# lthero-big/A-watermark-for-Diffusion-Models

Hardware: AMD Instinct MI355X
Metric: watermarked images/sec (embed+extract, 512x512 SD2.1) + lossless bit-accuracy (higher is better)
Workload: dtype f16; 1 GPU; e2e: gsw_embed -> 50-step DDIM sampling (CFG 7.5, 2B-row UNet) -> 50-step DDIM inversion -> fused last step + 256-bit vote; SD2.1-base-shaped UNet (865.9 M params, synthetic weights; convolutions on the hand-written MFMA implicit GEMM), image stages per image: VAE decode -> uint8 -> ToTensor -> VAE encode (timed; synthetic VAE, inversion consumes the latent); batch_per_gpu=64, global_batch=64, message_bits=256, ddim_steps=50, parallelism=dp1 (images sharded, UNet replicated, no data-path collective)

## Files before the change

a-watermark-for-diffusion-models_amd/_native.py:

```python
from __future__ import annotations

import ctypes as C
import os

_HERE = os.path.dirname(os.path.abspath(__file__))
LIB_PATH = os.environ.get("GSWM_LIB", os.path.join(_HERE, "libgswm.so"))

GSW_F32, GSW_F16, GSW_BF16, GSW_F64 = 0, 1, 2, 3
GSW_OK, GSW_ERR_BAD_ARG, GSW_ERR_UNSUPPORTED, GSW_ERR_RAGGED, GSW_ERR_HIP, GSW_WARN_NO_RECORDS = 0, 1, 2, 3, 4, 5
GSW_EMBED_EXACT_F64, GSW_EMBED_FAST_F32 = 0, 1
GSW_MM_GN_ONLY = 1
GSW_FLAG_SATURATED, GSW_FLAG_NAN = 1, 2
GSW_MSG_INLINE_MAX = 256
GSW_IMG_U8_HWC, GSW_IMG_F16_CHW, GSW_IMG_F32_CHW = 0, 1, 2
GSW_PW_BRIGHTNESS, GSW_PW_CONTRAST, GSW_PW_INVERT, GSW_PW_GRAY, GSW_PW_HFLIP, GSW_PW_VFLIP, GSW_PW_NOISE = range(7)
GSW_RESAMPLE_LANCZOS, GSW_RESAMPLE_BILINEAR = 1, 2
GSW_TRACE_SOFT, GSW_TRACE_HARD = 0, 1

_u8p = C.POINTER(C.c_uint8)


class GswMmExtras(C.Structure):
    _fields_ = [("colstats_dev", C.c_void_p), ("colstats_capacity", C.c_int64), ("rowstats_dev", C.c_void_p), ("rowstats_capacity", C.c_int64),
                ("workspace_dev", C.c_void_p), ("workspace_bytes", C.c_int64), ("max_splits", C.c_int),
                ("colstats_rows_per_block", C.c_int), ("colstats_blocks", C.c_int), ("rowstats_slots", C.c_int), ("splits", C.c_int), ("flags", C.c_int)]


_PROTOTYPES = {
    "gsw_version": (C.c_int, []),
    "gsw_build_flags": (C.c_int, []),
    "gsw_strerror": (C.c_char_p, [C.c_int]),
    "gsw_last_hip_error": (C.c_int, []),
    "gsw_keystream": (C.c_int, [C.c_char_p, C.c_char_p, C.c_void_p, C.c_size_t, C.c_void_p]),
    "gsw_embed": (C.c_int, [C.c_char_p, C.c_char_p, C.c_char_p, C.c_int, C.c_void_p, C.c_uint64, C.c_uint64, C.c_void_p,
                            C.c_int, C.c_int, C.c_int64, C.c_uint32, C.c_void_p]),
    "gsw_philox_uniform": (C.c_int, [C.c_uint64, C.c_uint64, C.c_void_p, C.c_int, C.c_int64, C.c_void_p]),
    "gsw_extract": (C.c_int, [C.c_void_p, C.c_int, C.c_char_p, C.c_char_p, C.c_int, C.c_void_p, C.c_void_p, C.c_void_p,
                              C.c_int, C.c_int64, C.c_void_p]),
    "gsw_bit_matches": (C.c_int, [C.c_void_p, C.c_int, C.c_char_p, C.c_int, C.c_void_p, C.c_int, C.c_void_p]),
    "gsw_ddim_step": (C.c_int, [C.c_void_p, C.c_void_p, C.c_void_p, C.c_float, C.c_float, C.c_int, C.c_int64, C.c_void_p]),
    "gsw_ddim_step_cfg": (C.c_int, [C.c_void_p, C.c_void_p, C.c_void_p, C.c_void_p, C.c_float, C.c_float, C.c_float,
                                    C.c_int, C.c_int64, C.c_void_p]),
    "gsw_dpm_step": (C.c_int, [C.c_void_p, C.c_void_p, C.c_void_p, C.c_void_p, C.c_void_p, C.c_void_p, C.c_float, C.c_float, C.c_float,
                               C.c_float, C.c_float, C.c_float, C.c_int, C.c_int64, C.c_void_p]),
    "gsw_ddim_step_extract": (C.c_int, [C.c_void_p, C.c_void_p, C.c_void_p, C.c_float, C.c_float, C.c_int, C.c_char_p,
                                        C.c_char_p, C.c_int, C.c_void_p, C.c_void_p, C.c_void_p, C.c_int, C.c_int64,
                                        C.c_void_p]),
    "gsw_groupnorm_silu": (C.c_int, [C.c_void_p, C.c_void_p, C.c_void_p, C.c_void_p, C.c_void_p, C.c_int, C.c_int, C.c_int, C.c_int,
                                     C.c_float, C.c_int, C.c_int, C.c_void_p]),
    "gsw_geglu": (C.c_int, [C.c_void_p, C.c_void_p, C.c_int64, C.c_int, C.c_int, C.c_void_p]),
    "gsw_conv_pf": (C.c_int, [C.c_void_p, C.c_void_p, C.c_void_p, C.c_void_p, C.c_int, C.c_void_p, C.c_void_p, C.c_int, C.c_int, C.c_int, C.c_int,
                              C.c_int, C.c_int, C.c_int, C.c_int, C.c_int, C.c_void_p]),
    "gsw_groupnorm_pf": (C.c_int, [C.c_void_p, C.c_void_p, C.c_void_p, C.c_void_p, C.c_void_p, C.c_int, C.c_int, C.c_int, C.c_int, C.c_int,
                                   C.c_float, C.c_int, C.c_int, C.c_int, C.c_void_p]),
    "gsw_add_layernorm": (C.c_int, [C.c_void_p, C.c_void_p, C.c_void_p, C.c_void_p, C.c_void_p, C.c_void_p, C.c_int64, C.c_int, C.c_float,
                                    C.c_int, C.c_void_p]),
    "gsw_groupnorm_pf2": (C.c_int, [C.c_void_p, C.c_void_p, C.c_int, C.c_void_p, C.c_void_p, C.c_void_p, C.c_void_p, C.c_int, C.c_int, C.c_int,
                                    C.c_int, C.c_int, C.c_float, C.c_int, C.c_int, C.c_int, C.c_void_p]),
    "gsw_conv3x3_res_pf": (C.c_int, [C.c_void_p, C.c_void_p, C.c_void_p, C.c_void_p, C.c_int, C.c_void_p, C.c_void_p, C.c_int, C.c_int, C.c_int, C.c_int,
                                     C.c_int, C.c_void_p, C.c_int, C.c_void_p, C.c_int, C.c_int, C.c_void_p]),
    "gsw_conv_up2x_pf": (C.c_int, [C.c_void_p, C.c_void_p, C.c_void_p, C.c_void_p, C.c_int, C.c_int, C.c_int, C.c_int, C.c_int, C.c_int, C.c_void_p]),
    "gsw_attention": (C.c_int, [C.c_void_p, C.c_void_p, C.c_void_p, C.c_void_p, C.c_int, C.c_int, C.c_int, C.c_int, C.c_int, C.c_int, C.c_int, C.c_int,
                                C.c_int, C.c_float, C.c_int, C.c_void_p]),
    "gsw_attention_ws": (C.c_int, [C.c_void_p, C.c_void_p, C.c_void_p, C.c_void_p, C.c_int, C.c_int, C.c_int, C.c_int, C.c_int, C.c_int, C.c_int, C.c_int,
                                   C.c_int, C.c_float, C.c_int, C.c_void_p, C.c_int64, C.c_void_p]),
    "gsw_xattn_fused": (C.c_int, [C.c_void_p, C.c_void_p, C.c_void_p, C.c_int64, C.c_void_p, C.c_int64, C.c_void_p, C.c_void_p, C.c_void_p, C.c_float, C.c_int, C.c_int,
                                  C.c_int, C.c_int, C.c_int, C.c_int, C.c_void_p]),
    "gsw_xattn_fused_pre": (C.c_int, [C.c_void_p, C.c_void_p, C.c_void_p, C.c_float, C.c_void_p, C.c_int64, C.c_void_p, C.c_int64, C.c_void_p, C.c_void_p, C.c_void_p,
                                      C.c_float, C.c_int, C.c_int, C.c_int, C.c_int, C.c_int, C.c_int, C.c_void_p]),
    "gsw_gn_colstats_pairs": (C.c_int, [C.c_void_p, C.c_int, C.c_int, C.c_int, C.c_void_p, C.c_int, C.c_int, C.c_int, C.c_int, C.c_void_p]),
    "gsw_gn_proj_tokens": (C.c_int, [C.c_void_p, C.c_void_p, C.c_void_p, C.c_void_p, C.c_float, C.c_int, C.c_void_p, C.c_void_p, C.c_void_p, C.c_float, C.c_int, C.c_int,
                                     C.c_int, C.c_int, C.c_int, C.c_void_p]),
    "gsw_mt19937_seed": (None, [C.c_uint32, C.c_void_p]),
    "gsw_mt19937_uniform": (C.c_int, [C.c_void_p, C.c_int, C.c_void_p, C.c_int64, C.c_void_p, C.c_void_p]),
    "gsw_lanczos_plan": (C.c_int, [C.c_int, C.c_int, C.c_void_p, C.c_void_p, C.c_int]),
    "gsw_resize_lanczos": (C.c_int, [C.c_void_p, C.c_int, C.c_int, C.c_int, C.c_void_p, C.c_int, C.c_int, C.c_int, C.c_void_p, C.c_void_p, C.c_void_p,
                                     C.c_int, C.c_void_p, C.c_void_p, C.c_int, C.c_void_p]),
    "gsw_tensor_to_image": (C.c_int, [C.c_void_p, C.c_int, C.c_int, C.c_int, C.c_int, C.c_int, C.c_void_p, C.c_void_p]),
    "gsw_jpeg_quant_tables": (C.c_int, [C.c_int, C.c_void_p, C.c_void_p]),
    "gsw_jpeg_workspace_bytes": (C.c_size_t, [C.c_int, C.c_int, C.c_int]),
    "gsw_jpeg_roundtrip": (C.c_int, [C.c_void_p, C.c_int, C.c_int, C.c_int, C.c_int, C.c_void_p, C.c_int, C.c_void_p, C.c_void_p]),
    "gsw_gaussian_blur_params": (C.c_int, [C.c_float, C.c_int, C.c_void_p, C.c_void_p, C.c_void_p]),
    "gsw_gaussian_blur": (C.c_int, [C.c_void_p, C.c_int, C.c_int, C.c_int, C.c_float, C.c_void_p, C.c_void_p, C.c_void_p]),
    "gsw_image_pointwise": (C.c_int, [C.c_void_p, C.c_int, C.c_int, C.c_int, C.c_int, C.c_float, C.c_uint64, C.c_uint64, C.c_void_p, C.c_int,
                                      C.c_void_p, C.c_void_p]),
    "gsw_resample_plan": (C.c_int, [C.c_int, C.c_int, C.c_int, C.c_void_p, C.c_void_p, C.c_int]),
    "gsw_affine_nearest": (C.c_int, [C.c_void_p, C.c_int, C.c_int, C.c_int, C.c_void_p, C.c_void_p, C.c_int, C.c_void_p]),
    "gsw_box_mask": (C.c_int, [C.c_void_p, C.c_int, C.c_int, C.c_int, C.c_void_p, C.c_int, C.c_void_p, C.c_int, C.c_void_p]),
    "gsw_crop_resize": (C.c_int, [C.c_void_p, C.c_int, C.c_int, C.c_int, C.c_void_p, C.c_int, C.c_int, C.c_void_p, C.c_int, C.c_int, C.c_int,
                                  C.c_void_p, C.c_void_p, C.c_void_p, C.c_int, C.c_void_p, C.c_void_p, C.c_int, C.c_void_p]),
    "gsw_gemm": (C.c_int, [C.c_void_p, C.c_void_p, C.c_void_p, C.c_void_p, C.c_void_p, C.c_int64, C.c_int, C.c_int, C.c_int, C.c_int, C.c_int,
                           C.c_int, C.c_void_p]),
    "gsw_gemm_qkv": (C.c_int, [C.c_void_p, C.c_void_p, C.c_void_p, C.c_void_p, C.c_void_p, C.c_int64, C.c_int, C.c_int, C.c_int, C.c_int, C.c_int, C.c_void_p]),
    "gsw_ln_rowstats_finish": (C.c_int, [C.c_void_p, C.c_int, C.c_int64, C.c_int, C.c_float, C.c_void_p, C.c_void_p]),
    "gsw_gemm_ln": (C.c_int, [C.c_void_p, C.c_void_p, C.c_void_p, C.c_void_p, C.c_void_p, C.c_void_p, C.c_int64, C.c_int, C.c_int, C.c_int, C.c_int, C.c_int, C.c_void_p]),
    "gsw_gemm_strided": (C.c_int, [C.c_void_p, C.c_int64, C.c_void_p, C.c_int64, C.c_void_p, C.c_void_p, C.c_int64, C.c_void_p, C.c_int64, C.c_int64,
                                   C.c_int, C.c_int, C.c_int, C.c_int, C.c_int, C.c_int, C.c_void_p]),
    "gsw_softmax_rows": (C.c_int, [C.c_void_p, C.c_int64, C.c_int, C.c_int64, C.c_float, C.c_int, C.c_void_p]),
    "gsw_mm_config": (C.c_int, [C.c_int, C.c_int]),
    "gsw_mm_get_config": (C.c_int, [C.POINTER(C.c_int), C.POINTER(C.c_int)]),
    "gsw_groupnorm_pf_cs": (C.c_int, [C.c_void_p, C.c_void_p, C.c_int, C.c_void_p, C.c_int, C.c_int, C.c_int, C.c_void_p, C.c_int, C.c_int, C.c_int,
                                      C.c_void_p, C.c_void_p, C.c_void_p, C.c_void_p, C.c_int, C.c_int, C.c_int, C.c_int, C.c_int, C.c_float, C.c_int, C.c_int,
                                      C.c_int, C.c_void_p]),
    "gsw_groupnorm_pf_fused": (C.c_int, [C.c_void_p, C.c_void_p, C.c_int, C.c_void_p, C.c_void_p, C.c_void_p, C.c_int, C.c_int, C.c_int, C.c_int, C.c_int, C.c_float,
                                         C.c_int, C.c_int, C.c_int, C.c_void_p]),
    "gsw_gather_rows": (C.c_int, [C.c_void_p, C.c_int64, C.c_int64, C.c_void_p, C.c_int, C.c_void_p, C.c_int64, C.c_int, C.c_int64, C.c_void_p]),
    "gsw_nchw_to_pf": (C.c_int, [C.c_void_p, C.c_void_p, C.c_int, C.c_int, C.c_int, C.c_int, C.c_int, C.c_int, C.c_void_p]),
    "gsw_conv3x3_pf_nchw": (C.c_int, [C.c_void_p, C.c_void_p, C.c_void_p, C.c_void_p, C.c_int, C.c_int, C.c_int, C.c_int, C.c_int, C.c_int, C.c_void_p]),
    "gsw_gemm_small_config": (C.c_int, [C.c_int64, C.c_int, C.c_int, C.c_int]),
    "gsw_gemm_small": (C.c_int, [C.c_void_p, C.c_int64, C.c_void_p, C.c_int64, C.c_void_p, C.c_void_p, C.c_int64, C.c_void_p, C.c_int64, C.c_int64, C.c_int, C.c_int,
                                 C.c_int, C.c_int, C.c_int, C.c_void_p, C.c_int, C.c_float, C.c_void_p, C.c_void_p, C.c_void_p, C.c_int64, C.POINTER(C.c_int), C.c_int,
                                 C.c_int, C.c_void_p]),
    "gsw_gemm_ex": (C.c_int, [C.c_void_p, C.c_int64, C.c_void_p, C.c_int64, C.c_void_p, C.c_void_p, C.c_int64, C.c_void_p, C.c_int64, C.c_int64, C.c_int, C.c_int,
                              C.c_int, C.c_int, C.c_int, C.c_int, C.c_void_p, C.c_void_p]),
    "gsw_gemm2_ex": (C.c_int, [C.c_void_p, C.c_int64, C.c_int, C.c_void_p, C.c_int64, C.c_int, C.c_void_p, C.c_int64, C.c_void_p, C.c_void_p, C.c_int64, C.c_void_p,
                               C.c_int64, C.c_int64, C.c_int, C.c_int, C.c_int, C.c_int, C.c_int, C.c_void_p, C.c_void_p]),
    "gsw_gemm_ln_ex": (C.c_int, [C.c_void_p, C.c_void_p, C.c_void_p, C.c_void_p, C.c_void_p, C.c_void_p, C.c_int64, C.c_int, C.c_int, C.c_int, C.c_int, C.c_int,
                                 C.c_void_p, C.c_void_p]),
    "gsw_conv_pf_ex": (C.c_int, [C.c_void_p, C.c_void_p, C.c_void_p, C.c_void_p, C.c_int, C.c_void_p, C.c_void_p, C.c_int, C.c_int, C.c_int, C.c_int,
                                 C.c_int, C.c_int, C.c_int, C.c_int, C.c_int, C.c_void_p, C.c_void_p]),
    "gsw_conv3x3_res_pf_ex": (C.c_int, [C.c_void_p, C.c_void_p, C.c_void_p, C.c_void_p, C.c_int, C.c_void_p, C.c_void_p, C.c_int, C.c_int, C.c_int, C.c_int,
                                        C.c_int, C.c_void_p, C.c_int, C.c_void_p, C.c_int, C.c_int, C.c_void_p, C.c_void_p]),
    "gsw_conv_up2x_pf_ex": (C.c_int, [C.c_void_p, C.c_void_p, C.c_void_p, C.c_void_p, C.c_int, C.c_int, C.c_int, C.c_int, C.c_int, C.c_int, C.c_void_p, C.c_void_p]),
    "gsw_trace_workspace_bytes": (C.c_size_t, [C.c_int, C.c_int64, C.c_int]),
    "gsw_trace_topk": (C.c_int, [C.c_void_p, C.c_int, C.c_int, C.c_int, C.c_int, C.c_void_p, C.c_int64, C.c_int, C.c_void_p, C.c_void_p, C.c_void_p, C.c_void_p]),
    "gsw_sign_pack": (C.c_int, [C.c_void_p, C.c_int, C.c_void_p, C.c_void_p, C.c_int, C.c_int64, C.c_void_p]),
    "gsw_trace_keyed_workspace_bytes": (C.c_size_t, [C.c_int, C.c_int64, C.c_int]),
    "gsw_trace_keyed_topk": (C.c_int, [C.c_void_p, C.c_int, C.c_int64, C.c_void_p, C.c_int64, C.c_int, C.c_int64, C.c_int, C.c_void_p, C.c_void_p, C.c_void_p, C.c_void_p]),
    "gsw_embed_l": (C.c_int, [C.c_char_p, C.c_char_p, C.c_char_p, C.c_int, C.c_void_p, C.c_uint64, C.c_uint64, C.c_void_p,
                              C.c_int, C.c_int, C.c_int64, C.c_uint32, C.c_int, C.c_void_p]),
    "gsw_extract_l": (C.c_int, [C.c_void_p, C.c_int, C.c_char_p, C.c_char_p, C.c_int, C.c_void_p, C.c_void_p, C.c_void_p,
                                C.c_int, C.c_int64, C.c_int, C.c_void_p]),
    "gsw_quant_pack": (C.c_int, [C.c_void_p, C.c_int, C.c_void_p, C.c_void_p, C.c_int, C.c_int64, C.c_int, C.c_void_p]),
}

_lib = None


class GswError(RuntimeError):
    def __init__(self, status: int, what: str):
        super().__init__(f"libgswm: {what} (status {status})")
        self.status = status


def lib() -> C.CDLL:
    global _lib
    if _lib is None:
        if not os.path.exists(LIB_PATH):
            raise ImportError(
                f"{LIB_PATH} is missing: the HIP library has not been built. Run __graft_entry__.build() "
                "(hipcc --offload-arch=gfx950). There is no CPU fallback for the watermark hot path.")
        l = C.CDLL(LIB_PATH)
        for name, (res, args) in _PROTOTYPES.items():
            fn = getattr(l, name)
            fn.restype = res
            fn.argtypes = args
        flags = l.gsw_build_flags()
        if flags != 0 and os.environ.get("GSWM_LIB") is None:
            raise ImportError(f"{LIB_PATH} was compiled with measurement switches (gsw_build_flags() = {flags:#x}): not a production build; rebuild it "
                              "(__graft_entry__.build()) or select the side build explicitly with GSWM_LIB")
        _lib = l
    return _lib


def exported_symbols():
    return sorted(_PROTOTYPES)


def check(status: int):
    if status == GSW_OK:
        return
    what = lib().gsw_strerror(status).decode()
    if status == GSW_ERR_RAGGED:
        raise IndexError("string index out of range")
    if status == GSW_ERR_BAD_ARG:
        raise ValueError(f"libgswm: {what}")
    if status == GSW_ERR_HIP:
        what += f" (hipError_t {lib().gsw_last_hip_error()})"
    raise GswError(status, what)
```

a-watermark-for-diffusion-models_amd/csrc/gswm_mm.hip:

```cpp
#include <hip/hip_runtime.h>
#include <hip/hip_fp16.h>
#include <hip/hip_bf16.h>
#include <stdint.h>
#include <stdlib.h>
#include <algorithm>
#include <atomic>
#include <type_traits>

#include "../../include/gswm.h"
#include "gswm_mm.h"
#include "gswm_mmtypes.h"
#include "gswm_ablate.inc"

static std::atomic<int> g_mm_tile_rows{getenv("GSW_MM_BM") ? atoi(getenv("GSW_MM_BM")) : 0};
static std::atomic<int> g_mm_split_mask{getenv("GSW_MM_SPLIT") ? atoi(getenv("GSW_MM_SPLIT")) : 10 };

namespace {

__device__ unsigned long long* g_mm_trace_buf;
template <typename F>
__device__ __forceinline__ mm_f4 mm_abl_touch(F a, F b, mm_f4 c) { c[0] = fmaf((float)a[0], (float)b[0], c[0]); return c; }
#define MM_BARRIER() do { __builtin_amdgcn_sched_barrier(0); __builtin_amdgcn_s_barrier(); __builtin_amdgcn_sched_barrier(0); } while (0)
#define MM_LDS_BARRIER() do { asm volatile("s_waitcnt lgkmcnt(0)" ::: "memory"); MM_BARRIER(); } while (0)

typedef float mm_f2 __attribute__((ext_vector_type(2)));
__device__ __forceinline__ uint32_t mm_lds_addr(const uint8_t* p) { return (uint32_t)(uintptr_t)(const __attribute__((address_space(3))) uint8_t*)p; }
__device__ __forceinline__ void mm_lds_read5_b64(uint32_t a, uint2 (&o)[5]) {
    uint64_t r0, r1, r2, r3, r4;
    asm volatile("ds_read_b64 %0, %5\n\tds_read_b64 %1, %5 offset:32\n\tds_read_b64 %2, %5 offset:64\n\tds_read_b64 %3, %5 offset:96\n\tds_read_b64 %4, %5 offset:128\n\t"
                 "s_waitcnt lgkmcnt(0)"
                 : "=&v"(r0), "=&v"(r1), "=&v"(r2), "=&v"(r3), "=&v"(r4) : "v"(a) : "memory");
    const uint64_t r[5] = {r0, r1, r2, r3, r4};
#pragma unroll
    for (int i = 0; i < 5; ++i) o[i] = make_uint2((uint32_t)r[i], (uint32_t)(r[i] >> 32));
}
template <uint32_t VOFF>
__device__ __forceinline__ void mm_lds_read_uv(uint32_t a, mm_f4 (&u)[5], mm_f4 (&v)[5]) {
    asm volatile("ds_read_b128 %0, %10\n\tds_read_b128 %1, %10 offset:64\n\tds_read_b128 %2, %10 offset:128\n\tds_read_b128 %3, %10 offset:192\n\tds_read_b128 %4, %10 offset:256\n\t"
                 "ds_read_b128 %5, %10 offset:%11\n\tds_read_b128 %6, %10 offset:%12\n\tds_read_b128 %7, %10 offset:%13\n\tds_read_b128 %8, %10 offset:%14\n\t"
                 "ds_read_b128 %9, %10 offset:%15\n\ts_waitcnt lgkmcnt(0)"
                 : "=&v"(u[0]), "=&v"(u[1]), "=&v"(u[2]), "=&v"(u[3]), "=&v"(u[4]), "=&v"(v[0]), "=&v"(v[1]), "=&v"(v[2]), "=&v"(v[3]), "=&v"(v[4])
                 : "v"(a), "n"(VOFF), "n"(VOFF + 64u), "n"(VOFF + 128u), "n"(VOFF + 192u), "n"(VOFF + 256u) : "memory");
}
template <uint32_t VOFF>
__device__ __forceinline__ void mm_lds_read_uv1(uint32_t a, mm_f4& u, mm_f4& v) {
    asm volatile("ds_read_b128 %0, %2\n\tds_read_b128 %1, %2 offset:%3\n\ts_waitcnt lgkmcnt(0)" : "=&v"(u), "=&v"(v) : "v"(a), "n"(VOFF) : "memory");
}
template <int MT>
__device__ __forceinline__ void mm_lds_read_rows(uint32_t a, mm_f2 (&r)[MT]) {
    if constexpr (MT == 8)
        asm volatile("ds_read_b64 %0, %8\n\tds_read_b64 %1, %8 offset:128\n\tds_read_b64 %2, %8 offset:256\n\tds_read_b64 %3, %8 offset:384\n\t"
                     "ds_read_b64 %4, %8 offset:512\n\tds_read_b64 %5, %8 offset:640\n\tds_read_b64 %6, %8 offset:768\n\tds_read_b64 %7, %8 offset:896\n\ts_waitcnt lgkmcnt(0)"
                     : "=&v"(r[0]), "=&v"(r[1]), "=&v"(r[2]), "=&v"(r[3]), "=&v"(r[4]), "=&v"(r[5]), "=&v"(r[6]), "=&v"(r[7]) : "v"(a) : "memory");
    else if constexpr (MT == 4)
        asm volatile("ds_read_b64 %0, %4\n\tds_read_b64 %1, %4 offset:128\n\tds_read_b64 %2, %4 offset:256\n\tds_read_b64 %3, %4 offset:384\n\ts_waitcnt lgkmcnt(0)"
                     : "=&v"(r[0]), "=&v"(r[1]), "=&v"(r[2]), "=&v"(r[3]) : "v"(a) : "memory");
    else
        asm volatile("ds_read_b64 %0, %2\n\tds_read_b64 %1, %2 offset:128\n\ts_waitcnt lgkmcnt(0)" : "=&v"(r[0]), "=&v"(r[1]) : "v"(a) : "memory");
}

__device__ __forceinline__ uint32_t mm_lane_now() {
    uint32_t l;
    asm volatile("v_mbcnt_lo_u32_b32 %0, -1, 0\n\tv_mbcnt_hi_u32_b32 %0, -1, %0" : "=v"(l));
    return l;
}
template <int CTRL, int ROW_MASK>
__device__ __forceinline__ float mm_dpp_add(float x) {
    return x + __int_as_float(__builtin_amdgcn_update_dpp(0, __float_as_int(x), CTRL, ROW_MASK, 0xf, false));
}

template <typename T, int EPI, bool SPLIT, int MT, bool LNF = false>
__global__ __launch_bounds__(SPLIT ? 768 : 512, SPLIT ? 1 : 2) void gsw_mm_kernel(const MMArgs p) {
    static_assert(!LNF || (!SPLIT && (EPI == 0 || EPI == 2 || EPI == 3)), "LayerNorm-folded epilogues: dense rows, GEGLU, transposed; 8-wave form");
    constexpr bool SWAP = EPI == 3;
    constexpr bool QKV = EPI == 5;
    constexpr bool PART = EPI == 4;
    static_assert(!PART || SPLIT, "split-K partial launches use the producer-wave variant");
    constexpr bool WIDE = MT == 8;
    constexpr int WM = WIDE ? 2 : 4;
    constexpr int NG = 8 / WM;
    constexpr int BM = WM * 16 * MT, BN = NG * 80;
    constexpr int NPR = MT / 2;
    static_assert(MT == 8 || MT == 4 || MT == 2, "wave tile of 128, 64 or 32 rows");
    static_assert(!WIDE || (!SPLIT && EPI != 3 && EPI != 4 && EPI != 5), "the wide tile: 8-wave form, dense rows / PF rows / GEGLU; no split-K, no transposed output, no fused q | k | v");
    constexpr int NPROD = SPLIT ? 4 : 8;
    constexpr int NPA = BM / 8 / NPROD;
    constexpr int NPW = BN / 8 / NPROD;
    constexpr int NEXTRA = BN / 8 - NPROD * NPW;
    constexpr int NDMA = NPA + NPW;
    constexpr uint32_t STAGE = (uint32_t)(BM + BN) * 128u;
    constexpr uint32_t RING = (WIDE ? 2u : 3u) * STAGE;
    constexpr int HC = 80;
    constexpr bool STG = !SPLIT && !SWAP && !QKV && (EPI == 2 || (EPI == 0 && (!LNF || WIDE)));
    constexpr uint32_t PARAM = RING;
    constexpr uint32_t PAR_V = WIDE ? 2048u : 1024u, PAR_ROWS = WIDE ? 4096u : 2048u;
    constexpr int NPCOL = WIDE ? 2 : 1;
    constexpr int NPAR = LNF ? 2 * NPCOL + (BM + 127) / 128 : 1;
    typedef typename MM<T>::frag frag;
    typedef unsigned int mm_u4 __attribute__((ext_vector_type(4)));
    extern __shared__ __attribute__((aligned(16))) uint8_t lds[];

    const uint32_t tid = threadIdx.x, lane = tid & 63u;
    const uint32_t wave = (uint32_t)__builtin_amdgcn_readfirstlane((int)(tid >> 6));
    const uint32_t grp = WIDE ? (wave >> 1) & 3u : (wave >> 2) & 1u, wm = WIDE ? wave & 1u : wave & 3u;
    const uint32_t pid = SPLIT ? (wave & 3u) : wave;
    const bool extra = pid < (uint32_t)NEXTRA;
    const bool stg = STG && p.P >= (WIDE ? 2 : 3) && (LNF || p.bias != nullptr);
    const bool stg7 = stg && wave == 7u;

    const uint32_t lane_rd0 = (lane & 15u) * 128u + ((((lane >> 4)) ^ ((lane >> 1) & 7u)) << 4);
    const uint32_t a_rd0 = wm * (16u * MT) * 128u + lane_rd0, a_rd1 = a_rd0 ^ 64u;
    const uint32_t w_rd0 = (uint32_t)BM * 128u + (grp * (uint32_t)HC) * 128u + lane_rd0, w_rd1 = w_rd0 ^ 64u;
    const uint32_t prow = lane >> 3;
    const uint32_t chunk8 = ((lane & 7u) ^ ((4u * (pid & 1u) + (lane >> 4)) & 7u)) * 8u;

    const uint32_t G = gridDim.x;
    const uint32_t slotx = (blockIdx.x & 7u) * (G >> 3) + (blockIdx.x >> 3);
    const uint32_t ntiles = (uint32_t)p.ntiles;
    const uint32_t nvirt = PART ? ntiles * (uint32_t)p.splits : ntiles;
    const uint32_t nt_mine = nvirt > slotx ? (nvirt - slotx + G - 1u) / G : 0u;
    if (nt_mine == 0u) return;
    const uint32_t part_split = PART ? slotx / ntiles : 0u;
    const int32_t k_lo = PART ? (int32_t)(((int64_t)part_split * p.P) / p.splits) : 0;
    const int32_t P_mine = PART ? (int32_t)(((int64_t)(part_split + 1u) * p.P) / p.splits) - k_lo : p.P;
    const T* Wbase = reinterpret_cast<const T*>(p.w);
    auto decode_tile = [&](uint32_t L, int32_t& tm, int32_t& tn) {
        const uint32_t tiles_m = ntiles / (uint32_t)p.tiles_n, pw = (uint32_t)p.panel;
        const uint32_t full = tiles_m * pw;
        const uint32_t pn = L / full, rem = L - pn * full;
        const uint32_t width = min(pw, (uint32_t)p.tiles_n - pn * pw);
        tm = (int32_t)(rem / width);
        tn = (int32_t)(pn * pw + rem - (rem / width) * width);
    };

    uint32_t pr_it = 0, pr_slot = 0;
    int32_t pr_seg = 0, pr_kc = 0, pr_kh = 0, pr_run = 0, a_step = 0, w_step = 0;
    int32_t pr_arow[NPA], pr_wrow[NPW + 1];
    const T* pa[NPA];
    const T* pw[NPW + 1];
    const bool compact = (p.flags & MM_FLAG_COMPACT) != 0;
    const int32_t HpWp = p.Hp * p.Wp;
    auto opaque = [&](int32_t v) -> int32_t { if constexpr (WIDE) asm volatile("" : "+s"(v)); return v; };
    auto udiv = [&](uint32_t m, uint32_t d, uint32_t mg) -> uint32_t {
        uint32_t q = __umulhi(m, mg);
        if (m - q * d >= d) ++q;
        return q;
    };
    auto pf_row = [&](int32_t m, int32_t& b, int32_t& yy, int32_t& xx) -> int32_t {
        if constexpr (WIDE) {
            const int32_t Wi = opaque(p.Wp - 2), HW = opaque((p.Hp - 2) * (p.Wp - 2));
            const uint32_t mg_hw = 0xFFFFFFFFu / (uint32_t)HW, mg_wi = 0xFFFFFFFFu / (uint32_t)Wi;
            b = (int32_t)udiv((uint32_t)m, (uint32_t)HW, mg_hw);
            const int32_t r = m - b * HW;
            yy = (int32_t)udiv((uint32_t)r, (uint32_t)Wi, mg_wi);
            xx = r - yy * Wi + 1;
            yy += 1;
            return b * HpWp + yy * p.Wp + xx;
        }
        const int32_t Wi = p.Wp - 2, HW = (p.Hp - 2) * Wi;
        b = m / HW;
        const int32_t r = m - b * HW;
        yy = r / Wi;
        xx = r - yy * Wi + 1;
        yy += 1;
        return b * HpWp + yy * p.Wp + xx;
    };
    auto setup_tile = [&](uint32_t it) {
        int32_t tm, tn;
        decode_tile(PART ? slotx % ntiles : it * G + slotx, tm, tn);
        const int32_t m0 = tm * BM, n0 = tn * BN;
#pragma unroll
        for (int i = 0; i < NPA; ++i) {
            const int32_t m = m0 + 8 * (int32_t)(pid + (uint32_t)NPROD * i) + (int32_t)prow;
            const int32_t mc = m < p.M ? m : p.M - 1;
            int32_t b_, y_, x_;
            pr_arow[i] = compact ? pf_row(mc, b_, y_, x_) : mc;
            if (compact && p.stride == 2) pr_arow[i] = b_ * (p.in_Hp * p.in_Wp) + 2 * (y_ - 1) * p.in_Wp + 2 * (x_ - 1);
        }
#pragma unroll
        for (int i = 0; i <= NPW; ++i) {
            const int32_t n = n0 + 8 * (int32_t)(pid + (uint32_t)NPROD * i) + (int32_t)prow;
            pr_wrow[i] = n < p.N ? n : p.N - 1;
        }
    };
    auto begin_run = [&]() {
        const MMSeg& s0 = p.seg[0]; const MMSeg& s1 = p.seg[1]; const MMSeg& s2 = p.seg[2];
        const int32_t s = pr_seg;
        const T* x = reinterpret_cast<const T*>(s == 0 ? s0.x : s == 1 ? s1.x : s2.x);
        const int32_t ld = s == 0 ? s0.ld : s == 1 ? s1.ld : s2.ld;
        const int32_t kb = s == 0 ? s0.kblocks : s == 1 ? s1.kblocks : s2.kblocks;
        const int32_t nt = s == 0 ? s0.ntaps : s == 1 ? s1.ntaps : s2.ntaps;
        const int32_t tw = s == 0 ? s0.tw : s == 1 ? s1.tw : s2.tw;
        const int32_t trow = s == 0 ? s0.tap_row : s == 1 ? s1.tap_row : s2.tap_row;
        const int32_t tbase = s == 0 ? s0.tap_base : s == 1 ? s1.tap_base : s2.tap_base;
        const int32_t wk0 = s == 0 ? s0.wk0 : s == 1 ? s1.wk0 : s2.wk0;
        const int32_t tapoff = tbase + pr_kh * trow;
        const int32_t wk = wk0 + pr_kh * tw * (kb * 64) + pr_kc * 64 + (int32_t)chunk8;
        if (nt == 1) { pr_run = kb; a_step = 64; w_step = 64; }
        else { pr_run = tw; a_step = ld; w_step = kb * 64; }
#pragma unroll
        for (int i = 0; i < NPA; ++i) pa[i] = x + ((int64_t)(pr_arow[i] + tapoff) * ld + pr_kc * 64 + (int32_t)chunk8);
#pragma unroll
        for (int i = 0; i <= NPW; ++i) pw[i] = Wbase + (pr_wrow[i] * p.ldw + wk);
    };
    auto end_run = [&]() {
        const MMSeg& s0 = p.seg[0]; const MMSeg& s1 = p.seg[1]; const MMSeg& s2 = p.seg[2];
        const int32_t s = pr_seg;
        const int32_t kb = s == 0 ? s0.kblocks : s == 1 ? s1.kblocks : s2.kblocks;
        const int32_t nt = s == 0 ? s0.ntaps : s == 1 ? s1.ntaps : s2.ntaps;
        const int32_t tw = s == 0 ? s0.tw : s == 1 ? s1.tw : s2.tw;
        bool seg_done = nt == 1;
        if (!seg_done && ++pr_kh * tw == nt) { pr_kh = 0; seg_done = ++pr_kc == kb; }
        if (seg_done) {
            pr_kc = 0; pr_kh = 0;
            if (++pr_seg == p.nseg) {
                pr_seg = 0;
                if (++pr_it == nt_mine) {
                    pr_run = 0x7FFFFFFF; a_step = 0; w_step = 0;
#pragma unroll
                    for (int i = 0; i < NPA; ++i) pa[i] = Wbase + chunk8;
#pragma unroll
                    for (int i = 0; i <= NPW; ++i) pw[i] = Wbase + chunk8;
                    return;
                }
                setup_tile(pr_it);
            }
        }
        begin_run();
    };
    auto dma_extra = [&]() {
        if (extra) {
            __builtin_amdgcn_global_load_lds((const __attribute__((address_space(1))) void*)pw[NPW],
                                             (__attribute__((address_space(3))) void*)(lds + pr_slot + (uint32_t)BM * 128u + (pid + (uint32_t)NPROD * NPW) * 1024u), 16, 0, 0);
            pw[NPW] += w_step;
        }
    };
    auto dma_piece_a = [&](int i) {
        __builtin_amdgcn_global_load_lds((const __attribute__((address_space(1))) void*)pa[i],
                                         (__attribute__((address_space(3))) void*)(lds + pr_slot + (pid + (uint32_t)NPROD * i) * 1024u), 16, 0, 0);
        pa[i] += a_step;
    };
    auto dma_piece_w = [&](int i) {
        __builtin_amdgcn_global_load_lds((const __attribute__((address_space(1))) void*)pw[i],
                                         (__attribute__((address_space(3))) void*)(lds + pr_slot + (uint32_t)BM * 128u + (pid + (uint32_t)NPROD * i) * 1024u), 16, 0, 0);
        pw[i] += w_step;
    };
    constexpr bool AFF = EPI == 0 || EPI == 2;
    uint32_t vo_a[4] = {0u, 0u, 0u, 0u}, vo_w = 0u, so_a = 0u, so_w = 0u, st_a = 0u, st_w = 0u, w_piece = 0u, a_piece = 0u;
    int32_t seg_rows = -1;
    bool pr_end = false;
    __amdgpu_buffer_rsrc_t rs_a = __builtin_amdgcn_make_buffer_rsrc(const_cast<void*>(p.w), 0, -1, 0x00020000);
    const __amdgpu_buffer_rsrc_t rs_w = __builtin_amdgcn_make_buffer_rsrc(const_cast<void*>(p.w), 0, -1, 0x00020000);
    uint32_t str_a8 = 128u * (uint32_t)p.seg[0].ld, str_w8 = 128u * (uint32_t)p.ldw;
    if constexpr (WIDE) asm volatile("" : "+s"(str_a8), "+s"(str_w8));
    int32_t tile_m8 = 0, tile_n8 = 0;
    auto setup_tile8 = [&](uint32_t it) {
        decode_tile(it * G + slotx, tile_m8, tile_n8);
        seg_rows = -1;
    };
    auto begin_run8 = [&]() {
        const MMSeg& s0 = p.seg[0]; const MMSeg& s1 = p.seg[1]; const MMSeg& s2 = p.seg[2];
        const int32_t sg = pr_seg;
        const T* x = reinterpret_cast<const T*>(sg == 0 ? s0.x : sg == 1 ? s1.x : s2.x);
        const int32_t ld = sg == 0 ? s0.ld : sg == 1 ? s1.ld : s2.ld;
        const int32_t kb = sg == 0 ? s0.kblocks : sg == 1 ? s1.kblocks : s2.kblocks;
        const int32_t nt = sg == 0 ? s0.ntaps : sg == 1 ? s1.ntaps : s2.ntaps;
        const int32_t tw = sg == 0 ? s0.tw : sg == 1 ? s1.tw : s2.tw;
        const int32_t trow = sg == 0 ? s0.tap_row : sg == 1 ? s1.tap_row : s2.tap_row;
        const int32_t tbase = sg == 0 ? s0.tap_base : sg == 1 ? s1.tap_base : s2.tap_base;
        const int32_t wk0 = sg == 0 ? s0.wk0 : sg == 1 ? s1.wk0 : s2.wk0;
        if (seg_rows != sg) {
            seg_rows = sg;
            const uint32_t l8 = mm_lane_now();

            const uint32_t prow = l8 >> 3;
            const uint32_t chunk8 = ((l8 & 7u) ^ ((4u * (pid & 1u) + (l8 >> 4)) & 7u)) * 8u;
            rs_a = __builtin_amdgcn_make_buffer_rsrc(const_cast<T*>(x + (int64_t)tbase * ld), 0, -1, 0x00020000);
            const int32_t m0 = tile_m8 * BM;
            if constexpr (AFF) {
                vo_a[0] = ((uint32_t)(m0 + 8 * (int32_t)pid + (int32_t)prow) * (uint32_t)ld + chunk8) * 2u;
            } else {
#pragma unroll
                for (int i = 0; i < NPA; ++i) {
                    const int32_t m = m0 + 8 * (int32_t)(pid + (uint32_t)NPROD * i) + (int32_t)prow;
                    const int32_t mc = m < p.M ? m : p.M - 1;
                    int32_t b_, y_, x_, row = mc;
                    if (compact) {
                        row = pf_row(mc, b_, y_, x_);
                        if (p.stride == 2) row = b_ * (p.in_Hp * p.in_Wp) + 2 * (y_ - 1) * p.in_Wp + 2 * (x_ - 1);
                    }
                    vo_a[i] = ((uint32_t)row * (uint32_t)ld + chunk8) * 2u;
                }
            }
        }
        so_a = (uint32_t)(pr_kh * trow * ld + pr_kc * 64) * 2u;
        so_w = (uint32_t)(tile_n8 * BN * p.ldw + wk0 + pr_kh * tw * (kb * 64) + pr_kc * 64) * 2u;
        if (nt == 1) { pr_run = kb; st_a = 128u; st_w = 128u; }
        else { pr_run = tw; st_a = (uint32_t)ld * 2u; st_w = (uint32_t)(kb * 64) * 2u; }
    };
    auto end_run8 = [&]() {
        const MMSeg& s0 = p.seg[0]; const MMSeg& s1 = p.seg[1]; const MMSeg& s2 = p.seg[2];
        const int32_t sg = pr_seg;
        const int32_t kb = sg == 0 ? s0.kblocks : sg == 1 ? s1.kblocks : s2.kblocks;
        const int32_t nt = sg == 0 ? s0.ntaps : sg == 1 ? s1.ntaps : s2.ntaps;
        const int32_t tw = sg == 0 ? s0.tw : sg == 1 ? s1.tw : s2.tw;
        bool seg_done = nt == 1;
        if (!seg_done && ++pr_kh * tw == nt) { pr_kh = 0; seg_done = ++pr_kc == kb; }
        if (seg_done) {
            pr_kc = 0; pr_kh = 0;
            if (++pr_seg == p.nseg) {
                pr_seg = 0;
                if (++pr_it == nt_mine) {
                    pr_run = 0x7FFFFFFF; st_a = 0u; st_w = 0u;
                    so_a = 0u; so_w = 0u;
                    return;
                }
                setup_tile8(pr_it);
            }
        }
        begin_run8();
    };
    auto dma_piece8 = [&](int j) {
        if (j < NPA) {
            if constexpr (AFF) {
                if (j == 0) a_piece = so_a;
                MM_ABL_DMA_A(__builtin_amdgcn_raw_ptr_buffer_load_lds(rs_a, (__attribute__((address_space(3))) void*)(lds + pr_slot + (pid + (uint32_t)NPROD * j) * 1024u), 16, (int)vo_a[0], (int)a_piece, 0, 0));
                a_piece += str_a8;
            } else {
                MM_ABL_DMA_A(__builtin_amdgcn_raw_ptr_buffer_load_lds(rs_a, (__attribute__((address_space(3))) void*)(lds + pr_slot + (pid + (uint32_t)NPROD * j) * 1024u), 16, (int)vo_a[j], (int)so_a, 0, 0));
            }
        } else {
            if (j == NPA) w_piece = so_w;
            MM_ABL_DMA_W(__builtin_amdgcn_raw_ptr_buffer_load_lds(rs_w, (__attribute__((address_space(3))) void*)(lds + pr_slot + (uint32_t)BM * 128u + (pid + (uint32_t)NPROD * (j - NPA)) * 1024u), 16,
                                                                  (int)vo_w, (int)w_piece, 0, 0));
            w_piece += str_w8;
        }
        if (j == NDMA - 1) {
            so_a += st_a; so_w += st_w;
            pr_slot = pr_slot + STAGE == RING ? 0u : pr_slot + STAGE;
            pr_end = --pr_run == 0;
        }
    };
    auto dma_h1 = [&]() {
#pragma unroll
        for (int i = 0; i < NPA / 2; ++i) dma_piece_a(i);
        dma_piece_w(0);
    };
    auto dma_h2 = [&]() {
#pragma unroll
        for (int i = NPA / 2; i < NPA; ++i) dma_piece_a(i);
        dma_piece_w(1);
        pr_slot = pr_slot + STAGE == RING ? 0u : pr_slot + STAGE;
    };
    if constexpr (SPLIT) {
        if (wave >= 8u) {
            int32_t pr_left = 0x7FFFFFFF;
            auto dma_stage = [&]() {
#pragma unroll
                for (int i = 0; i < NPA; ++i) MM_ABL_DMA_A(dma_piece_a(i));
#pragma unroll
                for (int i = 0; i < NPW; ++i) MM_ABL_DMA_W(dma_piece_w(i));
                pr_slot = pr_slot + STAGE == RING ? 0u : pr_slot + STAGE;
                if constexpr (PART) {
                    if (--pr_left == 0) {
                        pr_run = 0x7FFFFFFF; a_step = 0; w_step = 0;
#pragma unroll
                        for (int i = 0; i < NPA; ++i) pa[i] = Wbase + chunk8;
#pragma unroll
                        for (int i = 0; i <= NPW; ++i) pw[i] = Wbase + chunk8;
                        return;
                    }
                }
                if (--pr_run == 0) end_run();
            };
            constexpr int NWAIT = MM_ABL_NPA(NPA) + MM_ABL_NPW(NPW);
            setup_tile(0);
            if constexpr (PART) {
                const MMSeg& s0 = p.seg[0]; const MMSeg& s1 = p.seg[1];
                int32_t st = k_lo;
                const int32_t len0 = s0.kblocks * s0.ntaps, len1 = s1.kblocks * s1.ntaps;
                if (p.nseg > 1 && st >= len0) { st -= len0; pr_seg = 1; if (p.nseg > 2 && st >= len1) { st -= len1; pr_seg = 2; } }
                const int32_t nt = pr_seg == 0 ? s0.ntaps : 1, tw = pr_seg == 0 ? s0.tw : 1;
                int32_t skip = st;
                if (nt != 1) { pr_kc = st / nt; const int32_t r = st - pr_kc * nt; pr_kh = r / tw; skip = r - pr_kh * tw; }
                begin_run();
#pragma unroll
                for (int i = 0; i < NPA; ++i) pa[i] += (int64_t)skip * a_step;
#pragma unroll
                for (int i = 0; i <= NPW; ++i) pw[i] += (int64_t)skip * w_step;
                pr_run -= skip;
                pr_left = P_mine;
            } else {
                begin_run();
            }
            dma_stage();
            dma_stage();
            asm volatile("s_waitcnt vmcnt(%0)" :: "n"(NWAIT) : "memory");
            MM_BARRIER();
            const uint32_t total = nt_mine * (uint32_t)P_mine;
            MM_TRACE_DECL();
            for (uint32_t sidx = 0; sidx < total; ++sidx) {
                dma_stage();
                MM_STAMP(0);
                asm volatile("s_waitcnt vmcnt(%0)" :: "n"(NWAIT) : "memory");
                MM_STAMP(1);
                MM_BARRIER();
                MM_STAMP(2);
            }
            MM_TRACE_DUMP();
            asm volatile("s_waitcnt vmcnt(0)" ::: "memory");
            return;
        }
    } else if constexpr (WIDE) {
        {
            const uint32_t l8 = mm_lane_now();

            vo_w = (((8u * pid + (l8 >> 3)) * (uint32_t)p.ldw) + ((l8 & 7u) ^ ((4u * (pid & 1u) + (l8 >> 4)) & 7u)) * 8u) * 2u;
        }
        setup_tile8(0);
        begin_run8();
#pragma unroll
        for (int j = 0; j < NDMA; ++j) dma_piece8(j);
        if (pr_end) { end_run8(); pr_end = false; }
#pragma unroll
        for (int j = 0; j < NDMA; ++j) dma_piece8(j);
        __builtin_amdgcn_s_waitcnt(0x0F70);
    } else {
        static_assert(SPLIT || ((NPA == 4 || NPA == 2) && NPW == 2), "the half-stage split assumes 4 (2) + 2 (+1) pieces per wave");
        setup_tile(0);
        begin_run();
        for (int i = 0; i < 2; ++i) { dma_h1(); dma_extra(); dma_h2(); if (--pr_run == 0) end_run(); }
        dma_h1();
        asm volatile("s_waitcnt vmcnt(%0)" :: "n"(NDMA + NPA / 2 + 1) : "memory");
    }
    MM_BARRIER();

    const uint16_t* bias = reinterpret_cast<const uint16_t*>(p.bias);
    const uint16_t* rowbias = reinterpret_cast<const uint16_t*>(p.rowbias);
    const uint16_t* resid = reinterpret_cast<const uint16_t*>(p.resid);
    uint16_t* Y = reinterpret_cast<uint16_t*>(p.y);
    mm_f4 acc[5][MT];
#pragma unroll
    for (int a = 0; a < 5; ++a)
#pragma unroll
        for (int b = 0; b < MT; ++b) acc[a][b] = mm_f4{0.f, 0.f, 0.f, 0.f};
    uint32_t c_it = 0, rd_slot = 0;
    MM_TRACE_DECL();

    auto read_frags = [&](frag (&xf)[MT], frag (&wf)[5], uint32_t slot, uint32_t khalf) {
        const uint8_t* ap = lds + ((khalf ? a_rd1 : a_rd0) + slot);
        const uint8_t* wp = lds + ((khalf ? w_rd1 : w_rd0) + slot);
#pragma unroll
        for (int im = 0; im < MT; ++im) xf[im] = *reinterpret_cast<const frag*>(ap + im * 2048);
#pragma unroll
        for (int in = 0; in < 5; ++in) wf[in] = *reinterpret_cast<const frag*>(wp + in * 2048);
    };

    auto dma_params = [&]() {
        int32_t tm, tn;
        decode_tile(c_it * G + slotx, tm, tn);
        const int32_t m0 = tm * BM, n0 = tn * BN;
        const uint32_t lane_p = WIDE ? mm_lane_now() : (threadIdx.x & 63u);
        const uint32_t lane = lane_p;
        auto piece = [&](const void* base, uint32_t lane_bytes, uint32_t byte_off) {
            if constexpr (WIDE) {
                const __amdgpu_buffer_rsrc_t rs = __builtin_amdgcn_make_buffer_rsrc(const_cast<void*>(base), 0, -1, 0x00020000);
                __builtin_amdgcn_raw_ptr_buffer_load_lds(rs, (__attribute__((address_space(3))) void*)(lds + PARAM + byte_off), 16, (int)lane_bytes, 0, 0, 0);
            } else {
                __builtin_amdgcn_global_load_lds((const __attribute__((address_space(1))) void*)(reinterpret_cast<const uint8_t*>(base) + lane_bytes),
                                                 (__attribute__((address_space(3))) void*)(lds + PARAM + byte_off), 16, 0, 0);
            }
        };
        if constexpr (LNF) {
#pragma unroll
            for (int k = 0; k < NPCOL; ++k) {
                const uint32_t nc = (uint32_t)min(n0 + 256 * k + 4 * (int32_t)lane, p.N - 4) * 4u;
                piece(p.ln_u, nc, (uint32_t)k * 1024u);
                piece(p.ln_v, nc, PAR_V + (uint32_t)k * 1024u);
            }
#pragma unroll
            for (int k = 0; k < (BM + 127) / 128; ++k) piece(p.ln_stat, (uint32_t)min(m0 + 128 * k + 2 * (int32_t)lane, p.M - 2) * 8u, PAR_ROWS + (uint32_t)k * 1024u);
        } else {
            piece(p.bias, (uint32_t)min(n0 + 8 * (int32_t)lane, p.N - 8) * 2u, 0u);
        }
    };

    auto epilogue = [&]() {
        int32_t tile_m, tile_n;
        decode_tile(PART ? slotx % ntiles : c_it * G + slotx, tile_m, tile_n);
        const int32_t m0 = tile_m * BM, n0 = tile_n * BN;
        const uint32_t lane_e = WIDE ? mm_lane_now() : (threadIdx.x & 63u);

        const uint32_t lane = lane_e;
        const uint32_t q = lane >> 4, li = lane & 15u;
        uint32_t zero_hi = 0u;
        if constexpr (WIDE) asm volatile("v_mov_b32 %0, 0" : "=v"(zero_hi));
        auto zx = [&](uint32_t v) -> int64_t { return WIDE ? (int64_t)(((uint64_t)zero_hi << 32) | (uint64_t)v) : (int64_t)v; };
        MM_STAMP(13);
        auto out_row = [&](int32_t m, int32_t& img, bool& brd, bool& lv) -> int64_t {
            lv = m < p.M; brd = false; img = 0;
            int64_t orow_ = m;
            const int32_t mc = lv ? m : 0;
            if (p.mode == MM_MODE_PF || p.mode == MM_MODE_UP2X) {
                int32_t b, yy, xx;
                if (compact) {
                    orow_ = pf_row(mc, b, yy, xx);
                } else {
                    const int32_t d1 = opaque(HpWp), d2 = opaque(p.Wp);
                    b = mc / d1;
                    const int32_t r = mc - b * HpWp;
                    yy = r / d2; xx = r - yy * p.Wp;
                    brd = (yy == 0) | (yy == p.Hp - 1) | (xx == 0) | (xx == p.Wp - 1);
                }
                img = b;
                if (p.mode == MM_MODE_UP2X) {
                    const int32_t dy = (p.up - 1) >> 1, dx = (p.up - 1) & 1;
                    orow_ = ((int64_t)b * (2 * p.Hp - 2) + (2 * (yy - 1) + dy + 1)) * (2 * p.Wp - 2) + (2 * (xx - 1) + dx + 1);
                    lv = lv && !brd;
                }
            } else if (p.mode == MM_MODE_TOK2PF) {
                const int32_t d1 = opaque(p.S), d2 = opaque(p.Wimg);
                const int32_t b = mc / d1, ii = mc - b * p.S;
                const int32_t yy = ii / d2, xx = ii - yy * p.Wimg;
                img = b;
                orow_ = (int64_t)b * HpWp + (int64_t)(yy + 1) * p.Wp + (xx + 1);
            }
            return orow_;
        };
        if constexpr (WIDE && EPI == 1) {
            if (resid) {
                const __amdgpu_buffer_rsrc_t rs_r = __builtin_amdgcn_make_buffer_rsrc(const_cast<uint16_t*>(resid), 0, -1, 0x00020000);
#pragma unroll
                for (int k = 0; k < 4; ++k) {
                    const int32_t m = m0 + (int32_t)(wm * (16u * MT) + (uint32_t)k * 32u + (lane >> 1));
                    int32_t img_; bool brd_, lv_ = m < p.M;
                    int64_t row_ = m;
                    if constexpr (EPI == 1) row_ = out_row(m, img_, brd_, lv_);
                    const int64_t col_ = (int64_t)n0 + grp * (uint32_t)HC + (lane & 1u) * 64u;
                    if (lv_ && col_ < p.N)
                        __builtin_amdgcn_raw_ptr_buffer_load_lds(rs_r, (__attribute__((address_space(3))) void*)(lds + RING + 6144u), 4, (int)(uint32_t)((row_ * p.ldr + col_) * 2), 0, 0, 0);
                }
            }
        }
        const bool vtile = QKV && n0 >= p.n_rows;
        const bool transposed = SWAP || vtile;
        if constexpr (PART) {
            uint32_t sx = slotx * 8u + wave;
            asm volatile("" : "+s"(sx));
            float* slab = p.ws + (size_t)sx * (size_t)(5 * MT * 64 * 4);
            const uint32_t loff = lane * 4u;
#pragma unroll
            for (int in = 0; in < 5; ++in)
#pragma unroll
                for (int im = 0; im < MT; ++im)
                    if (m0 + (int32_t)(wm * (16u * MT)) + im * 16 < p.M)
                        *reinterpret_cast<mm_f4*>(slab + (uint32_t)((in * MT + im) * 256) + loff) = acc[in][im];
            ++c_it;
            return;
        }
        float ln_r[SWAP ? 4 * MT : MT], ln_n[SWAP ? 4 * MT : MT];
        mm_f4 ln_u4[5], ln_v4[5];
        if constexpr (LNF) {
            const float2* st = reinterpret_cast<const float2*>(p.ln_stat);
            if constexpr (!SWAP) {
                if constexpr (STG) {
                    if (!stg) {
                        MM_BARRIER();
                        if (wave == 7u) { dma_params(); asm volatile("s_waitcnt vmcnt(0)" ::: "memory"); }
                        MM_BARRIER();
                    }
                    if constexpr (!(WIDE && EPI == 0)) {
                        mm_f2 rw[MT];
                        mm_lds_read_rows<MT>(mm_lds_addr(lds + PARAM + PAR_ROWS) + (wm * (16u * MT) + li) * 8u, rw);
#pragma unroll
                        for (int im = 0; im < MT; ++im) { ln_r[im] = rw[im][0]; ln_n[im] = rw[im][1]; }
                    }
                    if constexpr (!WIDE) mm_lds_read_uv<PAR_V>(mm_lds_addr(lds + PARAM) + (grp * HC + q * 4u) * 4u, ln_u4, ln_v4);
                } else {
#pragma unroll
                for (int im = 0; im < MT; ++im) {
                    const int32_t m = m0 + (int32_t)(wm * (16u * MT) + (uint32_t)im * 16u + li);
                    const float2 v = st[m < p.M ? m : p.M - 1];
                    ln_r[im] = v.x; ln_n[im] = v.y;
                }
#pragma unroll
                for (int in = 0; in < 5; ++in) {
                    const int32_t nb = n0 + (int32_t)(grp * HC + (uint32_t)in * 16u + q * 4u);
                    const int32_t nc = nb < p.N ? nb : 0;
                    ln_u4[in] = *reinterpret_cast<const mm_f4*>(p.ln_u + nc);
                    ln_v4[in] = *reinterpret_cast<const mm_f4*>(p.ln_v + nc);
                }
                }
            } else {
#pragma unroll
                for (int im = 0; im < MT; ++im) {
                    const int32_t m = m0 + (int32_t)(wm * (16u * MT) + (uint32_t)im * 16u + q * 4u);
                    const int32_t mc = m + 3 < p.M ? m : 0;
                    const mm_f4 a = *reinterpret_cast<const mm_f4*>(st + mc), b = *reinterpret_cast<const mm_f4*>(st + mc + 2);
                    ln_r[4 * im] = a[0]; ln_n[4 * im] = a[1]; ln_r[4 * im + 1] = a[2]; ln_n[4 * im + 1] = a[3];
                    ln_r[4 * im + 2] = b[0]; ln_n[4 * im + 2] = b[1]; ln_r[4 * im + 3] = b[2]; ln_n[4 * im + 3] = b[3];
                }
#pragma unroll
                for (int in = 0; in < 5; ++in) {
                    const int32_t ncol = n0 + (int32_t)(grp * HC + (uint32_t)in * 16u + li);
                    const int32_t nc = ncol < p.N ? ncol : 0;
                    ln_u4[in] = mm_f4{p.ln_u[nc], 0.f, 0.f, 0.f};
                    ln_v4[in] = mm_f4{p.ln_v[nc], 0.f, 0.f, 0.f};
                }
            }
        }
        auto lnf_rows = [&](int pr) {
            if constexpr (LNF && WIDE && STG && EPI == 0) {
                mm_f2 rw[2];
                mm_lds_read_rows<2>(mm_lds_addr(lds + PARAM + PAR_ROWS) + (wm * (16u * MT) + (uint32_t)(2 * pr) * 16u + li) * 8u, rw);
                ln_r[2 * pr] = rw[0][0]; ln_n[2 * pr] = rw[0][1]; ln_r[2 * pr + 1] = rw[1][0]; ln_n[2 * pr + 1] = rw[1][1];
            }
        };
        auto lnf_cols = [&](int in) {
            if constexpr (LNF && WIDE && STG) mm_lds_read_uv1<PAR_V>(mm_lds_addr(lds + PARAM) + (grp * HC + (uint32_t)in * 16u + q * 4u) * 4u, ln_u4[in], ln_v4[in]);
        };
        auto vals4 = [&](int in, int im, const float (&b)[4], float (&o)[4]) {
            const mm_f4& a = acc[in][im];
            if constexpr (LNF) {
                if constexpr (!SWAP) {
#pragma unroll
                    for (int j = 0; j < 4; ++j) o[j] = fmaf(a[j], ln_r[im], fmaf(ln_n[im], ln_u4[in][j], ln_v4[in][j]));
                } else {
#pragma unroll
                    for (int j = 0; j < 4; ++j) o[j] = fmaf(a[j], ln_r[4 * im + j], fmaf(ln_n[4 * im + j], ln_u4[in][0], ln_v4[in][0]));
                }
            } else {
#pragma unroll
                for (int j = 0; j < 4; ++j) o[j] = a[j] + b[j];
            }
        };
        auto pack4 = [&](int in, int im, const float (&b)[4], uint32_t& lo, uint32_t& hi) {
            if constexpr (LNF) {
                float o[4];
                vals4(in, im, b, o);
                lo = MM<T>::cvt2(o[0], o[1]);
                hi = MM<T>::cvt2(o[2], o[3]);
            } else {
                const mm_f4& a = acc[in][im];
                lo = MM<T>::cvt2(a[0] + b[0], a[1] + b[1]);
                hi = MM<T>::cvt2(a[2] + b[2], a[3] + b[3]);
            }
        };
        uint2 bq_raw[5];
        if constexpr (STG && !LNF) {
#pragma unroll
            for (int in = 0; in < 5; ++in) bq_raw[in] = make_uint2(0, 0);
            if (bias) {
                if (!stg) {
                    MM_BARRIER();
                    if (wave == 7u) { dma_params(); asm volatile("s_waitcnt vmcnt(0)" ::: "memory"); }
                    MM_BARRIER();
                }
                mm_lds_read5_b64(mm_lds_addr(lds + PARAM) + (grp * HC + q * 4u) * 2u, bq_raw);
            }
        } else
#pragma unroll
        for (int in = 0; in < 5; ++in) {
            bq_raw[in] = make_uint2(0, 0);
            const int32_t nb = n0 + (int32_t)(grp * HC + (uint32_t)in * 16u + q * 4u);
            if (!LNF && !transposed && bias && nb < p.N) bq_raw[in] = *reinterpret_cast<const uint2*>(bias + nb);
        }
        auto bias4 = [&](int in, float (&bq)[4]) {
            bq[0] = MM<T>::up((uint16_t)bq_raw[in].x); bq[1] = MM<T>::up((uint16_t)(bq_raw[in].x >> 16));
            bq[2] = MM<T>::up((uint16_t)bq_raw[in].y); bq[3] = MM<T>::up((uint16_t)(bq_raw[in].y >> 16));
        };
        auto swap16 = [&](uint32_t& a, uint32_t& b) {
            const auto r = __builtin_amdgcn_permlane16_swap(a, b, false, false);
            a = r[0]; b = r[1];
        };
        auto swap32 = [&](uint32_t& a, uint32_t& b) {
            const auto r = __builtin_amdgcn_permlane32_swap(a, b, false, false);
            a = r[0]; b = r[1];
        };
        if (EPI == 0 || (QKV && !vtile)) {
            uint16_t* yrow[NPR];
            const uint16_t* rrow[NPR];
            bool live[NPR];
            const int32_t colb = n0 + (int32_t)(grp * HC + (q >> 1) * 8u);
            auto row_setup = [&](int pr) {
                const int32_t m = m0 + (int32_t)(wm * (16u * MT) + (uint32_t)(2 * pr + (int)(q & 1u)) * 16u + li);
                live[pr] = m < p.M;
                const int64_t mm = live[pr] ? m : 0;
                yrow[pr] = Y + mm * p.ldy + colb;
                rrow[pr] = resid ? resid + mm * p.ldr + colb : nullptr;
            };
            const bool rstat = EPI == 0 && p.rowstats != nullptr;
            float rs_s[NPR], rs_q[NPR];
#pragma unroll
            for (int pr = 0; pr < NPR; ++pr) { rs_s[pr] = __uint_as_float(zero_hi); rs_q[pr] = __uint_as_float(zero_hi); }
            constexpr int RSD = SPLIT ? 2 : (WIDE ? 2 : 5);
            uint4 rs[5][NPR];
            auto load_rs1 = [&](int in, int pr) {
                rs[in][pr] = make_uint4(zero_hi, zero_hi, zero_hi, zero_hi);
                if (colb + in * 16 < p.N) rs[in][pr] = *reinterpret_cast<const uint4*>(rrow[pr] + in * 16);
            };
            auto load_rs = [&](int in) {
#pragma unroll
                for (int pr = 0; pr < NPR; ++pr) load_rs1(in, pr);
            };
            auto block = [&](int in, int pr, const float (&bq)[4]) {
                uint32_t a0, a1, b0, b1;
                pack4(in, 2 * pr, bq, a0, a1);
                pack4(in, 2 * pr + 1, bq, b0, b1);
                swap16(a0, b0);
                swap16(a1, b1);
                uint32_t w4[4] = {a0, a1, b0, b1};
                if (resid) {
                    const uint32_t rsw[4] = {rs[in][pr].x, rs[in][pr].y, rs[in][pr].z, rs[in][pr].w};
#pragma unroll
                    for (int k = 0; k < 4; ++k) w4[k] = MM<T>::add2(w4[k], rsw[k]);
                }
                if constexpr (WIDE) { if (in == 0 && pr == 0) { MM_STAMP(7); if (!resid) __builtin_amdgcn_s_waitcnt(0x0F70); MM_STAMP(8); } }
                if (live[pr] && colb + in * 16 < p.N) {
                    *reinterpret_cast<uint4*>(yrow[pr] + in * 16) = make_uint4(w4[0], w4[1], w4[2], w4[3]);
                    if (rstat) {
#pragma unroll
                        for (int k = 0; k < 4; ++k) MM<T>::stat2(w4[k], rs_s[pr], rs_q[pr]);
                    }
                }
            };
            auto flush_stat = [&](int pr) {
                uint32_t a = __float_as_uint(rs_s[pr]), b = __float_as_uint(rs_q[pr]);
                swap32(a, b);
                const float t = __uint_as_float(a) + __uint_as_float(b);
                const int32_t m = m0 + (int32_t)(wm * (16u * MT) + (uint32_t)(2 * pr + (int)(q & 1u)) * 16u + li);
                if (m < p.M) p.rowstats[((int64_t)m * (NG * p.tiles_n) + NG * tile_n + (int32_t)grp) * 2 + zx(lane >> 5)] = t;
            };
            if constexpr (WIDE) {
                auto body = [&](auto res_tag, auto stat_tag) {
                    constexpr bool RES = decltype(res_tag)::value, STAT = decltype(stat_tag)::value;
                    constexpr int RD = LNF ? 10 : 8;
                    const uint32_t lrow = (q & 1u) * 16u + li, lcol = grp * (uint32_t)HC + (q >> 1) * 8u;
                    const uint32_t y_voff = (lrow * (uint32_t)p.ldy + lcol) * 2u;
                    const uint32_t y_s0 = (uint32_t)(((int64_t)(m0 + (int32_t)(wm * (16u * MT))) * p.ldy + n0) * 2);
                    mm_u4 rq[4 * 5];
                    const __amdgpu_buffer_rsrc_t rs_q = __builtin_amdgcn_make_buffer_rsrc(const_cast<uint16_t*>(RES ? resid : Y), 0, -1, 0x00020000);
                    uint32_t r_voff = 0u, r_s0 = 0u;
                    auto rq_issue = [&](int b) {
                        const int pr = b / 5, in = b % 5;
                        rq[b] = __builtin_amdgcn_raw_buffer_load_b128(rs_q, (int)r_voff, (int)(r_s0 + (uint32_t)(pr * 32) * (uint32_t)p.ldr * 2u + (uint32_t)(in * 32)), 0);
                    };
                    if constexpr (RES) {
                        r_voff = (lrow * (uint32_t)p.ldr + lcol) * 2u;
                        r_s0 = (uint32_t)(((int64_t)(m0 + (int32_t)(wm * (16u * MT))) * p.ldr + n0) * 2);
#pragma unroll
                        for (int b = 0; b < RD; ++b) rq_issue(b);
                    }
#pragma unroll
                    for (int pr = 0; pr < NPR; ++pr) {
                        lnf_rows(pr);
                        float ss = __uint_as_float(zero_hi), sq = __uint_as_float(zero_hi);
#pragma unroll
                        for (int in = 0; in < 5; ++in) {
                            const int b = pr * 5 + in;
                            float bq[4];
                            bias4(in, bq);
                            lnf_cols(in);
                            if constexpr (RES) { if (b + RD < 20) rq_issue(b + RD); }
                            uint32_t a0, a1, b0, b1;
                            pack4(in, 2 * pr, bq, a0, a1);
                            pack4(in, 2 * pr + 1, bq, b0, b1);
                            swap16(a0, b0);
                            swap16(a1, b1);
                            mm_u4 w4 = {a0, a1, b0, b1};
                            if constexpr (RES) {
#pragma unroll
                                for (int k = 0; k < 4; ++k) w4[k] = MM<T>::add2(w4[k], rq[b][k]);
                            }
                            if (b == 0) {
                                MM_STAMP(7);
                                if constexpr (!RES) __builtin_amdgcn_s_waitcnt(0x0F70);
                                MM_STAMP(8);
                            }
                            *reinterpret_cast<mm_u4*>(reinterpret_cast<uint8_t*>(Y) + (size_t)(y_s0 + (uint32_t)(pr * 32) * (uint32_t)p.ldy * 2u + (uint32_t)(in * 32)) + (size_t)y_voff) = w4;
                            if constexpr (STAT) {
#pragma unroll
                                for (int k = 0; k < 4; ++k) MM<T>::stat2(w4[k], ss, sq);
                            }
                            __builtin_amdgcn_sched_barrier(0);
                        }
                        if constexpr (STAT) {
                            uint32_t a = __float_as_uint(ss), bb = __float_as_uint(sq);
                            swap32(a, bb);
                            const float t = __uint_as_float(a) + __uint_as_float(bb);
                            const int32_t m = m0 + (int32_t)(wm * (16u * MT) + (uint32_t)(2 * pr + (int)(q & 1u)) * 16u + li);
                            p.rowstats[((int64_t)m * (NG * p.tiles_n) + NG * tile_n + (int32_t)grp) * 2 + zx(lane >> 5)] = t;
                        }
                        __builtin_amdgcn_sched_barrier(0);
                    }
                };
                if (resid) { if (rstat) body(std::true_type{}, std::true_type{}); else body(std::true_type{}, std::false_type{}); }
                else { if (rstat) body(std::false_type{}, std::true_type{}); else body(std::false_type{}, std::false_type{}); }
            } else {
#pragma unroll
                for (int pr = 0; pr < NPR; ++pr) row_setup(pr);
                if (resid) {
#pragma unroll
                    for (int in = 0; in < RSD; ++in) load_rs(in);
                }
#pragma unroll
                for (int in = 0; in < 5; ++in) {
                    float bq[4];
                    bias4(in, bq);
                    if (resid && in + RSD < 5) load_rs(in + RSD);
#pragma unroll
                    for (int pr = 0; pr < NPR; ++pr) block(in, pr, bq);
                }
                if (rstat) {
#pragma unroll
                    for (int pr = 0; pr < NPR; ++pr) flush_stat(pr);
                }
            }
        } else if (EPI == 1) {
            using orow_t = std::conditional_t<WIDE, int32_t, int64_t>;
            orow_t orow[NPR];
            int32_t img_b[NPR];
            bool live[NPR], border[NPR];
#pragma unroll
            for (int pr = 0; pr < NPR; ++pr) {
                const int32_t m = m0 + (int32_t)(wm * (16u * MT) + (uint32_t)(2 * pr + (int)(q & 1u)) * 16u + li);
                orow[pr] = (orow_t)out_row(m, img_b[pr], border[pr], live[pr]);
            }
            const bool cstat = p.colstats != nullptr;
            MM_STAMP(14);
            constexpr int PD = WIDE ? 6 : 1;
            uint4 prev[PD + 1];
            auto fetch = [&](int in, int pr, int sl) {
                const int64_t col = (int64_t)n0 + grp * (uint32_t)HC + (uint32_t)in * 16u + (q >> 1) * 8u;
                const bool okl = live[pr] && col < p.N && !border[pr];
                if (resid) prev[sl] = *reinterpret_cast<const uint4*>(resid + (okl ? (int64_t)orow[pr] * p.ldr + col : (int64_t)0));
                else prev[sl] = *reinterpret_cast<const uint4*>(rowbias + (okl ? (int64_t)img_b[pr] * p.ldrb + col : (int64_t)0));
            };
            if constexpr (WIDE) {
                if (rowbias || resid) {
#pragma unroll
                    for (int j0 = 0; j0 < PD; ++j0) fetch(j0 / NPR, j0 % NPR, j0);
                }
            }
#pragma unroll
            for (int in = 0; in < 5; ++in) {
                float bq[4];
                bias4(in, bq);
                const int64_t col = (int64_t)n0 + grp * (uint32_t)HC + (uint32_t)in * 16u + (q >> 1) * 8u;
                float cs_s[4] = {0.f, 0.f, 0.f, 0.f}, cs_q[4] = {0.f, 0.f, 0.f, 0.f};
#pragma unroll
                for (int pr = 0; pr < NPR; ++pr) {
                    constexpr int NB = 5 * NPR;
                    const int j = in * NPR + pr;
                    if constexpr (WIDE) { if ((rowbias || resid) && j + PD < NB) fetch((j + PD) / NPR, (j + PD) % NPR, (j + PD) % (PD + 1)); }
                    uint32_t a0, a1, b0, b1;
                    pack4(in, 2 * pr, bq, a0, a1);
                    pack4(in, 2 * pr + 1, bq, b0, b1);
                    swap16(a0, b0);
                    swap16(a1, b1);
                    if constexpr (WIDE) { if (j == 0 && !(rowbias || resid)) __builtin_amdgcn_s_waitcnt(0x0F70); }
                    if constexpr (WIDE) {
                        uint32_t w4[4] = {a0, a1, b0, b1};
                        if (rowbias || resid) {
                            uint4 rb = make_uint4(0, 0, 0, 0), rs = make_uint4(0, 0, 0, 0);
                            if (resid) { rs = prev[j % (PD + 1)]; if (rowbias) rb = *reinterpret_cast<const uint4*>(rowbias + (int64_t)img_b[pr] * p.ldrb + (col < p.N ? col : 0)); }
                            else rb = prev[j % (PD + 1)];
                            const uint32_t rbw[4] = {rb.x, rb.y, rb.z, rb.w}, rsw[4] = {rs.x, rs.y, rs.z, rs.w};
#pragma unroll
                            for (int k = 0; k < 4; ++k) {
                                if (rowbias) w4[k] = MM<T>::add2(w4[k], rbw[k]);
                                if (resid) w4[k] = MM<T>::add2(w4[k], rsw[k]);
                            }
                        }
                        if (border[pr]) { w4[0] = w4[1] = w4[2] = w4[3] = 0u; }
                        if (live[pr] && col < p.N) {
                            *reinterpret_cast<uint4*>(Y + (int64_t)orow[pr] * p.ldy + col) = make_uint4(w4[0], w4[1], w4[2], w4[3]);
                            if (cstat && !border[pr]) {
#pragma unroll
                                for (int k = 0; k < 4; ++k) MM<T>::stat2(w4[k], cs_s[k], cs_q[k]);
                            }
                        }
                        continue;
                    }
                    if (!live[pr] || col >= p.N) continue;
                    uint32_t w4[4] = {a0, a1, b0, b1};
                    if (border[pr]) { w4[0] = w4[1] = w4[2] = w4[3] = 0u; }
                    else if (rowbias || resid) {
                        uint4 rb = make_uint4(0, 0, 0, 0), rs = make_uint4(0, 0, 0, 0);
                        if (rowbias) rb = *reinterpret_cast<const uint4*>(rowbias + (int64_t)img_b[pr] * p.ldrb + col);
                        if (resid) rs = *reinterpret_cast<const uint4*>(resid + (int64_t)orow[pr] * p.ldr + col);
                        const uint32_t rbw[4] = {rb.x, rb.y, rb.z, rb.w}, rsw[4] = {rs.x, rs.y, rs.z, rs.w};
#pragma unroll
                        for (int k = 0; k < 4; ++k) {
                            if (rowbias) w4[k] = MM<T>::add2(w4[k], rbw[k]);
                            if (resid) w4[k] = MM<T>::add2(w4[k], rsw[k]);
                        }
                    }
                    *reinterpret_cast<uint4*>(Y + (int64_t)orow[pr] * p.ldy + col) = make_uint4(w4[0], w4[1], w4[2], w4[3]);
                    if (cstat && !border[pr]) {
#pragma unroll
                        for (int k = 0; k < 4; ++k) MM<T>::stat2(w4[k], cs_s[k], cs_q[k]);
                    }
                }
                if (cstat) {
                    float rec[4];
#pragma unroll
                    for (int k = 0; k < 4; ++k) {
                        uint32_t a = __float_as_uint(cs_s[k]), b = __float_as_uint(cs_q[k]);
                        swap16(a, b);
                        float t = __uint_as_float(a) + __uint_as_float(b);
                        t = mm_dpp_add<0x111, 0xf>(t);
                        t = mm_dpp_add<0x112, 0xf>(t);
                        t = mm_dpp_add<0x114, 0xf>(t);
                        t = mm_dpp_add<0x118, 0xf>(t);
                        rec[k] = t;
                    }
                    if (li == 15u && col < p.N) {
                        float* dst = p.colstats + (((int64_t)tile_m * WM + wm) * 2 + (q & 1u)) * (int64_t)(p.N >> 1) + (col >> 1);
                        *reinterpret_cast<mm_f4*>(dst) = mm_f4{rec[0], rec[1], rec[2], rec[3]};
                    }
                }
                MM_STAMP(8 + in);
            }
            if constexpr (WIDE) {
                if (rowbias || resid) {
#pragma unroll
                    for (int k = 0; k <= PD; ++k) asm volatile("" :: "v"(prev[k].x));
                }
            }
        } else if (EPI == 2) {
            const uint32_t qv = q & 1u;
            uint32_t D[5][NPR][2];
            auto gate_block = [&](int in) {
                float bq[4];
                bias4(in, bq);
                lnf_cols(in);
                uint32_t Wv[MT];
#pragma unroll
                for (int im = 0; im < MT; ++im) {
                    uint32_t A, Bp;
                    pack4(in, im, bq, A, Bp);
                    swap32(A, Bp);
                    const uint32_t G = MM<T>::cvt2(mm_gelu(MM<T>::up_lo(Bp)), mm_gelu(MM<T>::up_hi(Bp)));
                    Wv[im] = MM<T>::mul2(A, G);
                }
#pragma unroll
                for (int pr = 0; pr < NPR; ++pr) {
                    uint32_t a = Wv[2 * pr], b = Wv[2 * pr + 1];
                    swap32(a, b);
                    D[in][pr][0] = a;
                    D[in][pr][1] = b;
                }
            };
            const int64_t obase = (int64_t)tile_n * (BN / 2) + grp * 40u;
            auto store_pair = [&](int ip) {
#pragma unroll
                for (int pr = 0; pr < NPR; ++pr) {
                    uint32_t a0 = D[2 * ip][pr][0], a1 = D[2 * ip][pr][1], b0 = D[2 * ip + 1][pr][0], b1 = D[2 * ip + 1][pr][1];
                    swap16(a0, b0);
                    swap16(a1, b1);
                    const int32_t m = m0 + (int32_t)(wm * (16u * MT) + (uint32_t)(2 * pr + (int)(q >> 1)) * 16u + li);
                    if (m < p.M)
                        *reinterpret_cast<uint4*>(Y + (int64_t)m * p.ldy + obase + zx((uint32_t)(2 * ip + (int)(q & 1u)) * 8u)) = make_uint4(a0, a1, b0, b1);
                }
            };
            auto store_last = [&]() {
#pragma unroll
                for (int pr = 0; pr < NPR; ++pr) {
                    const int32_t m = m0 + (int32_t)(wm * (16u * MT) + (uint32_t)(2 * pr + (int)(lane >> 5)) * 16u + li);
                    if (m < p.M)
                        *reinterpret_cast<uint2*>(Y + (int64_t)m * p.ldy + obase + zx(32u + qv * 4u)) = make_uint2(D[4][pr][0], D[4][pr][1]);
                }
            };
            if constexpr (WIDE) {
                gate_block(0); gate_block(1);
                MM_STAMP(7);
                __builtin_amdgcn_s_waitcnt(0x0F70);
                MM_STAMP(8);
                store_pair(0);
                __builtin_amdgcn_sched_barrier(0);
                gate_block(2); gate_block(3); store_pair(1);
                __builtin_amdgcn_sched_barrier(0);
                gate_block(4); store_last();
            } else {
#pragma unroll
                for (int in = 0; in < 5; ++in) gate_block(in);
                store_pair(0); store_pair(1);
                store_last();
            }
        } else {
            const int32_t nbase = QKV ? p.n_rows : 0, Nt = p.N - nbase;
            uint16_t* Yt = QKV ? reinterpret_cast<uint16_t*>(p.y2) : Y;
#pragma unroll
            for (int in = 0; in < 5; ++in) {
                const int32_t ncol = n0 + (int32_t)(grp * HC + (uint32_t)in * 16u + li);
                const int32_t nrow = ncol - nbase;
                const bool nok = ncol < p.N;
                const float bv = !LNF && bias && nok ? MM<T>::up(bias[ncol]) : 0.f;
                const float bq[4] = {bv, bv, bv, bv};
#pragma unroll
                for (int pr = 0; pr < NPR; ++pr) {
                    uint32_t a0, a1, b0, b1;
                    pack4(in, 2 * pr, bq, a0, a1);
                    pack4(in, 2 * pr + 1, bq, b0, b1);
                    swap16(a0, b0);
                    swap16(a1, b1);
                    const int32_t m = m0 + (int32_t)(wm * (16u * MT) + (uint32_t)(2 * pr + (int)(q & 1u)) * 16u + (q >> 1) * 8u);
                    if (m >= p.M || !nok) continue;
                    const int32_t b = m / p.S, sidx = m - b * p.S;
                    *reinterpret_cast<uint4*>(Yt + ((int64_t)b * Nt + nrow) * p.S + sidx) = make_uint4(a0, a1, b0, b1);
                }
            }
        }
#pragma unroll
        for (int a = 0; a < 5; ++a)
#pragma unroll
            for (int b = 0; b < MT; ++b) acc[a][b] = mm_f4{0.f, 0.f, 0.f, 0.f};
        ++c_it;
    };

    auto mfma20 = [&](auto swap_tag, frag (&xc)[MT], frag (&wc)[5]) {
        constexpr bool SW = decltype(swap_tag)::value;
#pragma unroll
        for (int in = 0; in < 5; ++in)
#pragma unroll
            for (int im = 0; im < MT; ++im)
                acc[in][im] = SW ? MM_ABL_MMA(xc[im], wc[in], acc[in][im]) : MM_ABL_MMA(wc[in], xc[im], acc[in][im]);
    };
    auto pin_order = [&]() {
        constexpr int NM = 5 * MT, NR = MT + 5;
        if constexpr (SPLIT) {
            constexpr int per = MT == 4 ? 2 : 1;
#pragma unroll
            for (int i = 0; i < NR; ++i) {
                __builtin_amdgcn_sched_group_barrier(0x008, per, 0);
                __builtin_amdgcn_sched_group_barrier(0x100, 1, 0);
            }
            __builtin_amdgcn_sched_group_barrier(0x008, NM - per * NR, 0);
        } else {
            constexpr int NV = NPA / 2 + 1;
            constexpr int per = MT == 4 ? 3 : 1;
#pragma unroll
            for (int i = 0; i < NV; ++i) {
                __builtin_amdgcn_sched_group_barrier(0x008, per, 0);
                __builtin_amdgcn_sched_group_barrier(0x020, 1, 0);
            }
#pragma unroll
            for (int i = 0; i < NR; ++i) {
                __builtin_amdgcn_sched_group_barrier(0x008, 1, 0);
                __builtin_amdgcn_sched_group_barrier(0x100, 1, 0);
            }
            __builtin_amdgcn_sched_group_barrier(0x008, NM - per * NV - NR, 0);
        }
    };
    auto step = [&](auto swap_tag, frag (&xX)[MT], frag (&wX)[5], frag (&xY)[MT], frag (&wY)[5], const int32_t step_i) {
        const uint32_t nx_slot = rd_slot + STAGE == RING ? 0u : rd_slot + STAGE;
        MM_STAMP(0);
        if constexpr (!SPLIT) { dma_extra(); dma_h2(); }
        MM_ABL_READ(read_frags(xY, wY, rd_slot, 1u));
        mfma20(swap_tag, xX, wX);
        pin_order();
        if constexpr (!SPLIT) { if (--pr_run == 0) end_run(); }
        MM_STAMP(1);
        if constexpr (STG) {
            if (stg7 && step_i == 1) asm volatile("s_waitcnt vmcnt(%0)" :: "n"(NDMA + NPAR) : "memory");
            else asm volatile("s_waitcnt vmcnt(%0)" :: "n"(NDMA) : "memory");
        } else if constexpr (!SPLIT) asm volatile("s_waitcnt vmcnt(%0)" :: "n"(NDMA) : "memory");
        MM_STAMP(2);
        asm volatile("s_waitcnt lgkmcnt(0)" ::: "memory");
        MM_BARRIER();
        MM_STAMP(3);
        if constexpr (STG) {
            if (stg7 && step_i == 0) dma_params();
        }
        if constexpr (!SPLIT) dma_h1();
        MM_ABL_READ(read_frags(xX, wX, nx_slot, 0u));
        mfma20(swap_tag, xY, wY);
        pin_order();
        MM_STAMP(4);
        __builtin_amdgcn_sched_barrier(0);
        MM_STAMP(5);
        rd_slot = nx_slot;
    };

    if constexpr (WIDE) {
        auto rd_at = [&](uint32_t base, int blk) -> frag { return *reinterpret_cast<const frag*>(lds + base + blk * 2048); };
        frag wA[5], wB[5], xr[4];
        auto seg = [&](auto odd_tag, auto im0_tag, auto im1_tag, auto dma_tag, frag (&wc)[5], frag (&wn)[5], const uint32_t slot_c, const uint32_t slot_n) {
            constexpr bool ODD = decltype(odd_tag)::value;
            constexpr int IM0 = decltype(im0_tag)::value, IM1 = decltype(im1_tag)::value, DMA = decltype(dma_tag)::value;
            constexpr uint32_t kh_c = ODD ? 1u : 0u, kh_n = ODD ? 0u : 1u;
            uint32_t lrd = lane_rd0;
            asm volatile("" : "+v"(lrd));
            const uint32_t a_c = (lrd ^ (kh_c * 64u)) + (wm * (16u * MT) * 128u + slot_c);
            const uint32_t a_n = (lrd ^ (kh_n * 64u)) + (wm * (16u * MT) * 128u + slot_n);
            const uint32_t w_n = (lrd ^ (kh_n * 64u)) + ((uint32_t)BM * 128u + grp * (uint32_t)HC * 128u + slot_n);
#pragma unroll
            for (int im = IM0; im < IM1; ++im) {
                if (im + 3 < 8) { MM_ABL_READ(xr[(im + 3) & 3] = rd_at(a_c, im + 3)); }
                else if (DMA != 2) { MM_ABL_READ(xr[(im + 3) & 3] = rd_at(a_n, im - 5)); }
                if (DMA != 2 && im == 5) { MM_ABL_READ(wn[0] = rd_at(w_n, 0)); MM_ABL_READ(wn[1] = rd_at(w_n, 1)); MM_ABL_READ(wn[2] = rd_at(w_n, 2)); }
                if (DMA != 2 && im == 6) { MM_ABL_READ(wn[3] = rd_at(w_n, 3)); MM_ABL_READ(wn[4] = rd_at(w_n, 4)); }
                if (DMA == 2 && ODD && im >= 5) { dma_piece8(3 * (im - 5)); dma_piece8(3 * (im - 5) + 1); dma_piece8(3 * (im - 5) + 2); }
                if (DMA == 1 && ODD && im >= 5) dma_piece8(im - 5);
                if (DMA == 1 && !ODD && im < 6) dma_piece8(3 + im);
#pragma unroll
                for (int in = 0; in < 5; ++in) acc[in][im] = MM_ABL_MMA(wc[in], xr[im & 3], acc[in][im]);
                __builtin_amdgcn_sched_barrier(0);
            }
        };
        auto run_end = [&]() { if (pr_end) { end_run8(); pr_end = false; } };
        using I0 = std::integral_constant<int, 0>; using I1 = std::integral_constant<int, 1>; using I2 = std::integral_constant<int, 2>;
        using I5 = std::integral_constant<int, 5>; using I8 = std::integral_constant<int, 8>;
        for (uint32_t it = 0; it < nt_mine; ++it) {
            uint32_t nx_slot = rd_slot + STAGE == RING ? 0u : rd_slot + STAGE;
            MM_STAMP(6);
            {
                uint32_t lrd = lane_rd0;
                asm volatile("" : "+v"(lrd));
                const uint32_t a0_ = lrd + (wm * (16u * MT) * 128u + rd_slot), w0_ = lrd + ((uint32_t)BM * 128u + grp * (uint32_t)HC * 128u + rd_slot);
#pragma unroll
                for (int in = 0; in < 5; ++in) { MM_ABL_READ(wA[in] = rd_at(w0_, in)); }
#pragma unroll
                for (int im = 0; im < 3; ++im) { MM_ABL_READ(xr[im] = rd_at(a0_, im)); }
            }
            seg(std::false_type{}, I0{}, I8{}, I0{}, wA, wB, rd_slot, rd_slot);
            seg(std::true_type{}, I0{}, I5{}, I0{}, wB, wA, rd_slot, nx_slot);
            MM_STAMP(0);
            asm volatile("s_waitcnt lgkmcnt(0)" ::: "memory");
            MM_BARRIER();
            MM_STAMP(1);
            run_end();
            if constexpr (STG) { if (stg7) dma_params(); }
            for (int32_t i = 1; i < P_mine; ++i) {
                seg(std::true_type{}, I5{}, I8{}, I1{}, wB, wA, rd_slot, nx_slot);
                rd_slot = nx_slot;
                nx_slot = rd_slot + STAGE == RING ? 0u : rd_slot + STAGE;
                seg(std::false_type{}, I0{}, I8{}, I1{}, wA, wB, rd_slot, rd_slot);
                seg(std::true_type{}, I0{}, I5{}, I0{}, wB, wA, rd_slot, nx_slot);
                MM_STAMP(2);
                asm volatile("s_waitcnt vmcnt(0)" ::: "memory");
                MM_STAMP(3);
                asm volatile("s_waitcnt lgkmcnt(0)" ::: "memory");
                MM_BARRIER();
                MM_STAMP(4);
                run_end();
            }
            seg(std::true_type{}, I5{}, I8{}, I2{}, wB, wA, rd_slot, nx_slot);
            MM_STAMP(5);
            rd_slot = nx_slot;
            epilogue();
        }
        MM_STAMP(6);
        MM_TRACE_DUMP();
        asm volatile("s_waitcnt vmcnt(0)" ::: "memory");
        return;
    }
    frag xa[MT], wa[5], xb[MT], wb[5];
    read_frags(xa, wa, 0u, 0u);
    asm volatile("s_waitcnt lgkmcnt(0)" ::: "memory");
    for (uint32_t it = 0; it < nt_mine; ++it) {
        if constexpr (QKV) {
            int32_t tm_, tn_;
            decode_tile(it * G + slotx, tm_, tn_);
            if (tn_ * BN >= p.n_rows) { for (int32_t i = 0; i < P_mine; ++i) step(std::true_type{}, xa, wa, xb, wb, i); }
            else { for (int32_t i = 0; i < P_mine; ++i) step(std::false_type{}, xa, wa, xb, wb, i); }
        } else {
            for (int32_t i = 0; i < P_mine; ++i) step(std::integral_constant<bool, SWAP>{}, xa, wa, xb, wb, i);
        }
        epilogue();
        MM_STAMP(6);
    }
    MM_TRACE_DUMP();
    asm volatile("s_waitcnt vmcnt(0)" ::: "memory");
}


template <typename T>
__global__ __launch_bounds__(256) void gsw_mm_reduce_kernel(const MMArgs p, const int MT) {
    const int32_t BM = 64 * MT, upt = 8 * 5 * MT * 64;
    const int64_t total = (int64_t)p.ntiles * upt;
    const size_t split_stride = (size_t)total * 4;
    const uint16_t* bias = reinterpret_cast<const uint16_t*>(p.bias);
    const uint16_t* rowbias = reinterpret_cast<const uint16_t*>(p.rowbias);
    const uint16_t* resid = reinterpret_cast<const uint16_t*>(p.resid);
    uint16_t* Y = reinterpret_cast<uint16_t*>(p.y);
    const bool compact = (p.flags & MM_FLAG_COMPACT) != 0;
    const int32_t HpWp = p.Hp * p.Wp;
    const uint32_t tiles_m = (uint32_t)p.ntiles / (uint32_t)p.tiles_n;
    for (int64_t u = (int64_t)blockIdx.x * 256 + threadIdx.x; u < total; u += (int64_t)gridDim.x * 256) {
        const uint32_t lane = (uint32_t)u & 63u;
        uint32_t r = (uint32_t)(u >> 6);
        const uint32_t accidx = r % (uint32_t)(5 * MT); r /= (uint32_t)(5 * MT);
        const uint32_t wave = r & 7u, L = r >> 3;
        const uint32_t in = accidx / (uint32_t)MT, im = accidx - in * (uint32_t)MT;
        const uint32_t wm = wave & 3u, grp = wave >> 2, q = lane >> 4, li = lane & 15u;
        const uint32_t pw = (uint32_t)p.panel, full = tiles_m * pw, pn = L / full, rem = L - pn * full;
        const uint32_t width = min(pw, (uint32_t)p.tiles_n - pn * pw);
        const int32_t tile_m = (int32_t)(rem / width), tile_n = (int32_t)(pn * pw + rem - (rem / width) * width);
        const int32_t m = tile_m * BM + (int32_t)(wm * (uint32_t)(16 * MT) + im * 16u + li);
        const int32_t n = tile_n * 160 + (int32_t)(grp * 80u + in * 16u + q * 4u);
        const bool geglu = p.mode == MM_MODE_GEGLU;
        if (m >= p.M || n >= p.N || (geglu && q >= 2u)) continue;
        mm_f4 a = mm_f4{0.f, 0.f, 0.f, 0.f}, g = mm_f4{0.f, 0.f, 0.f, 0.f};
        const float* src = p.ws + (size_t)u * 4;
        int s = 0;
        for (; s + 8 <= p.splits; s += 8) {
            mm_f4 t[8], tg[8];
#pragma unroll
            for (int j = 0; j < 8; ++j) t[j] = *reinterpret_cast<const mm_f4*>(src + (size_t)(s + j) * split_stride);
            if (geglu) {
#pragma unroll
                for (int j = 0; j < 8; ++j) tg[j] = *reinterpret_cast<const mm_f4*>(src + (size_t)(s + j) * split_stride + 32 * 4);
            }
#pragma unroll
            for (int j = 0; j < 8; ++j) a += t[j];
            if (geglu) {
#pragma unroll
                for (int j = 0; j < 8; ++j) g += tg[j];
            }
        }
        for (; s + 2 <= p.splits; s += 2) {
            const mm_f4 t0 = *reinterpret_cast<const mm_f4*>(src + (size_t)s * split_stride), t1 = *reinterpret_cast<const mm_f4*>(src + (size_t)(s + 1) * split_stride);
            mm_f4 g0 = mm_f4{0.f, 0.f, 0.f, 0.f}, g1 = g0;
            if (geglu) { g0 = *reinterpret_cast<const mm_f4*>(src + (size_t)s * split_stride + 32 * 4); g1 = *reinterpret_cast<const mm_f4*>(src + (size_t)(s + 1) * split_stride + 32 * 4); }
            a += t0; a += t1;
            if (geglu) { g += g0; g += g1; }
        }
        for (; s < p.splits; ++s) {
            a += *reinterpret_cast<const mm_f4*>(src + (size_t)s * split_stride);
            if (geglu) g += *reinterpret_cast<const mm_f4*>(src + (size_t)s * split_stride + 32 * 4);
        }
        float b4[4] = {0.f, 0.f, 0.f, 0.f};
        if (bias) { for (int j = 0; j < 4; ++j) b4[j] = MM<T>::up(bias[n + j]); }
        uint16_t h[4];
        for (int j = 0; j < 4; ++j) h[j] = MM<T>::cvt(a[j] + b4[j]);
        if (geglu) {
            for (int j = 0; j < 4; ++j) {
                const float gb = bias ? MM<T>::up(bias[n + 8 + j]) : 0.f;
                const float gg = MM<T>::up(MM<T>::cvt(g[j] + gb));
                const float ge = MM<T>::up(MM<T>::cvt(mm_gelu(gg)));
                h[j] = MM<T>::cvt(MM<T>::up(h[j]) * ge);
            }
            const int64_t ocol = (int64_t)tile_n * 80 + grp * 40u + in * 8u + q * 4u;
            *reinterpret_cast<uint2*>(Y + (int64_t)m * p.ldy + ocol) = make_uint2((uint32_t)h[0] | ((uint32_t)h[1] << 16), (uint32_t)h[2] | ((uint32_t)h[3] << 16));
            continue;
        }
        if (p.mode == MM_MODE_TRANS || (p.mode == MM_MODE_QKV && n >= p.n_rows)) {
            const int32_t nbase = p.mode == MM_MODE_QKV ? p.n_rows : 0;
            uint16_t* Yt = p.mode == MM_MODE_QKV ? reinterpret_cast<uint16_t*>(p.y2) : Y;
            const int32_t b = m / p.S, sidx = m - b * p.S;
            for (int j = 0; j < 4; ++j) Yt[((int64_t)b * (p.N - nbase) + (n - nbase) + j) * p.S + sidx] = h[j];
            continue;
        }
        int64_t orow = m;
        int32_t img = 0;
        bool border = false;
        if (p.mode == MM_MODE_PF || p.mode == MM_MODE_UP2X) {
            int32_t b, yy, xx;
            if (compact) {
                const int32_t Wi = p.Wp - 2, HW = (p.Hp - 2) * Wi;
                b = m / HW;
                const int32_t rr = m - b * HW;
                yy = rr / Wi; xx = rr - yy * Wi + 1; yy += 1;
                orow = (int64_t)b * HpWp + yy * p.Wp + xx;
            } else {
                b = m / HpWp;
                const int32_t rr = m - b * HpWp;
                yy = rr / p.Wp; xx = rr - yy * p.Wp;
                border = (yy == 0) | (yy == p.Hp - 1) | (xx == 0) | (xx == p.Wp - 1);
            }
            img = b;
            if (p.mode == MM_MODE_UP2X) {
                if (border) continue;
                const int32_t dy = (p.up - 1) >> 1, dx = (p.up - 1) & 1;
                orow = ((int64_t)b * (2 * p.Hp - 2) + (2 * (yy - 1) + dy + 1)) * (2 * p.Wp - 2) + (2 * (xx - 1) + dx + 1);
            }
        } else if (p.mode == MM_MODE_TOK2PF) {
            const int32_t b = m / p.S, ii = m - b * p.S;
            const int32_t yy = ii / p.Wimg, xx = ii - yy * p.Wimg;
            img = b;
            orow = (int64_t)b * HpWp + (int64_t)(yy + 1) * p.Wp + (xx + 1);
        }
        if (border) { h[0] = h[1] = h[2] = h[3] = 0; }
        else if (rowbias || resid) {
            for (int j = 0; j < 4; ++j) {
                float f = MM<T>::up(h[j]);
                if (p.mode == MM_MODE_DENSE && !rowbias) f += MM<T>::up(resid[orow * p.ldr + n + j]);
                else f = f + (rowbias ? MM<T>::up(rowbias[(int64_t)img * p.ldrb + n + j]) : 0.f) + (resid ? MM<T>::up(resid[orow * p.ldr + n + j]) : 0.f);
                h[j] = MM<T>::cvt(f);
            }
        }
        *reinterpret_cast<uint2*>(Y + orow * p.ldy + n) = make_uint2((uint32_t)h[0] | ((uint32_t)h[1] << 16), (uint32_t)h[2] | ((uint32_t)h[3] << 16));
    }
}

template <typename T, int EPI, bool SPLIT, int MT, bool LNF = false>
int mm_launch_k(const MMArgs& a, uint32_t grid, hipStream_t st) {
    static bool attr_done = false;
    constexpr bool wide = MT == 8;
    constexpr size_t ldsb = wide ? 2u * 576u * 128u + 6144u + 256u
                                 : 3u * (size_t)(64 * MT + 160) * 128u + (!SPLIT && (EPI == 2 || (EPI == 0 && !LNF)) ? 4096u : 0u);
    if (!attr_done) {
        hipError_t e = hipFuncSetAttribute((const void*)gsw_mm_kernel<T, EPI, SPLIT, MT, LNF>, hipFuncAttributeMaxDynamicSharedMemorySize, 160 * 1024);
        if (e != hipSuccess) return (int)e;
        attr_done = true;
    }
    hipLaunchKernelGGL((gsw_mm_kernel<T, EPI, SPLIT, MT, LNF>), dim3(grid), dim3(SPLIT ? 768 : 512), ldsb, st, a);
    return (int)hipGetLastError();
}
template <typename T, int EPI>
int mm_launch_t(const MMArgs& a, uint32_t grid, int mt, hipStream_t st) {
    if constexpr (EPI == 5) return mt == 4 ? mm_launch_k<T, 5, false, 4>(a, grid, st) : mm_launch_k<T, 5, false, 2>(a, grid, st);
    else {
    if (a.ln_stat) {
        if constexpr (EPI == 0 || EPI == 2) { if (mt == 8) return mm_launch_k<T, EPI, false, 8, true>(a, grid, st); }
        if constexpr (EPI == 0 || EPI == 2 || EPI == 3)
            return mt == 4 ? mm_launch_k<T, EPI, false, 4, true>(a, grid, st) : mm_launch_k<T, EPI, false, 2, true>(a, grid, st);
        else return (int)hipErrorInvalidValue;
    }
    if constexpr (EPI == 0 || EPI == 1 || EPI == 2) { if (mt == 8) return mm_launch_k<T, EPI, false, 8>(a, grid, st); }
    const bool split = (g_mm_split_mask.load(std::memory_order_relaxed) >> EPI) & 1;
    if constexpr (EPI == 0) { if (mt == 4) return mm_launch_k<T, EPI, false, 4>(a, grid, st); }
    else { if (mt == 4) return split ? mm_launch_k<T, EPI, true, 4>(a, grid, st) : mm_launch_k<T, EPI, false, 4>(a, grid, st); }
    return split ? mm_launch_k<T, EPI, true, 2>(a, grid, st) : mm_launch_k<T, EPI, false, 2>(a, grid, st);
    }
}
template <typename T>
int mm_launch_splitk(const MMArgs& a, uint32_t grid, int mt, hipStream_t st) {
    if (mt != 2 && mt != 4) return (int)hipErrorInvalidValue;
    const int e = mt == 4 ? mm_launch_k<T, 4, true, 4>(a, grid, st) : mm_launch_k<T, 4, true, 2>(a, grid, st);
    if (e != 0) return e;
    const int64_t units = (int64_t)a.ntiles * 8 * 5 * mt * 64;
    hipLaunchKernelGGL((gsw_mm_reduce_kernel<T>), dim3((uint32_t)std::min<int64_t>((units + 255) / 256, 2048)), dim3(256), 0, st, a, mt);
    return (int)hipGetLastError();
}
template <typename T>
int mm_launch_e(const MMArgs& a, int epi, uint32_t grid, int mt, hipStream_t st) {
    switch (epi) {
        case 0: return mm_launch_t<T, 0>(a, grid, mt, st);
        case 1: return mm_launch_t<T, 1>(a, grid, mt, st);
        case 2: return mm_launch_t<T, 2>(a, grid, mt, st);
        case 5: return mm_launch_t<T, 5>(a, grid, mt, st);
        default: return mm_launch_t<T, 3>(a, grid, mt, st);
    }
}

}

extern __attribute__((visibility("hidden"))) thread_local int g_last_hip_error;


void gsw_mm_no_extras(GswMmExtras* ex) {
    ex->colstats_dev = nullptr; ex->colstats_capacity = 0;
    ex->rowstats_dev = nullptr; ex->rowstats_capacity = 0;
    ex->workspace_dev = nullptr; ex->workspace_bytes = 0; ex->max_splits = 0;
    ex->colstats_rows_per_block = 0; ex->colstats_blocks = 0; ex->rowstats_slots = 0; ex->splits = 1; ex->flags = 0;
}

int gsw_build_flags(void) { return GSW_MM_BUILD_FLAGS; }

int gsw_mm_config(int tile_rows, int split_mask) {
    if (tile_rows != 0 && tile_rows != 128 && tile_rows != 256 && tile_rows != 512 && tile_rows != -1) return GSW_ERR_BAD_ARG;
    if (split_mask < -1 || split_mask > 15) return GSW_ERR_BAD_ARG;
    if (tile_rows != -1) g_mm_tile_rows.store(tile_rows, std::memory_order_relaxed);
    if (split_mask != -1) g_mm_split_mask.store(split_mask, std::memory_order_relaxed);
    return GSW_OK;
}

int gsw_mm_get_config(int* tile_rows, int* split_mask) {
    if (tile_rows) *tile_rows = g_mm_tile_rows.load(std::memory_order_relaxed);
    if (split_mask) *split_mask = g_mm_split_mask.load(std::memory_order_relaxed);
    return GSW_OK;
}

static int mm_cus() {
    static const int cus = [] {
        const char* e = getenv("GSW_MM_CUS");
        if (!e || !*e) return 256;
        int n = atoi(e);
        if (n <= 0) {
            int dev = 0;
            hipDeviceProp_t pr;
            n = (hipGetDevice(&dev) == hipSuccess && hipGetDeviceProperties(&pr, dev) == hipSuccess) ? pr.multiProcessorCount : 256;
        }
        return n >= 8 ? n / 8 * 8 : 256;
    }();
    return cus;
}
struct MMPlan { int bm; int splits; double t_us; };
static inline double mm_stage_us(int bm, double W, int64_t CU) {
    const double half = 0.5 * (double)CU;
    const double over = W > half ? (W - half) / half : 0.0;
    return bm == 128 ? 0.56 + 0.11 * over : 0.79 + 0.02 * std::min(1.0, W / half) + 0.32 * over;
}
static MMPlan mm_plan(int64_t M, int64_t tiles_n, int32_t P, bool can_split, int max_splits) {
    const int bm_env = g_mm_tile_rows.load(std::memory_order_relaxed);
    const int64_t CU = mm_cus();
    const int64_t nt256 = ((M + 255) / 256) * tiles_n, nt128 = ((M + 127) / 128) * tiles_n;
    auto t_unsplit = [&](int bm) {
        const int64_t nt = bm == 256 ? nt256 : nt128, rounds = (nt + CU - 1) / CU;
        return 2.5 + mm_stage_us(bm, rounds == 1 ? (double)nt : (double)CU, CU) * (double)P * (double)rounds;
    };
    int BM;
    if (bm_env == 128 || bm_env == 256) BM = bm_env;
    else if (M <= 128) BM = 256;
    else if (P >= 40 && nt256 <= CU) BM = t_unsplit(128) < t_unsplit(256) ? 128 : 256;
    else BM = nt256 < (P >= 64 ? CU / 2 : CU) ? 128 : 256;
    MMPlan pl{BM, 1, t_unsplit(BM)};
    if (!can_split) return pl;
    if (max_splits > 1) {
        const int bm_s = bm_env == 256 && M > 128 ? 256 : 128;
        const int64_t nt_f = ((M + bm_s - 1) / bm_s) * tiles_n;
        const int sp = (int)std::min<int64_t>(std::min<int64_t>(max_splits, P), CU / std::max<int64_t>(nt_f, 1));
        if (sp >= 2) { pl.bm = bm_s; pl.splits = sp; }
        return pl;
    }
    if (P < 8) return pl;
    double best = pl.t_us / 1.05;
    for (int bm_c = 128; bm_c <= 256; bm_c += 128) {
        if (bm_c == 256 && (M <= 128 || bm_env == 128)) continue;
        if (bm_c == 128 && bm_env == 256) continue;
        const int64_t nt_c = bm_c == 256 ? nt256 : nt128;
        if (nt_c > CU / 2) continue;
        for (int s_ = 2; s_ <= 32 && s_ * nt_c <= CU && 2 * s_ <= P; ++s_) {
            const double t = 12.5 + mm_stage_us(bm_c, (double)(s_ * nt_c), CU) * (double)((P + s_ - 1) / s_) + 0.014 * (double)(s_ * nt_c * (bm_c / 128));
            if (t < best) { best = t; pl.bm = bm_c; pl.splits = s_; pl.t_us = t; }
        }
    }
    return pl;
}

double gsw_mm_predict_us(int64_t M, int N, int P, const GswMmExtras* ex) {
    const bool have_ws = ex && ex->workspace_bytes > 0 && ex->workspace_dev;
    const int max_splits = ex ? ex->max_splits : 0;
    const MMPlan pl = mm_plan(M, ((int64_t)N + 159) / 160, P, have_ws && max_splits != 1, max_splits);
    const int64_t need = (int64_t)pl.splits * (((M + pl.bm - 1) / pl.bm) * (((int64_t)N + 159) / 160)) * 8 * 5 * (pl.bm / 64) * 64 * 16;
    if (pl.splits >= 2 && need > (ex ? ex->workspace_bytes : 0)) return mm_plan(M, ((int64_t)N + 159) / 160, P, false, 1).t_us;
    return pl.t_us;
}

int gsw_mm_launch(MMArgs& a, int dtype, void* stream, GswMmExtras* ex) {
    GswMmExtras none;
    if (!ex) { gsw_mm_no_extras(&none); ex = &none; }
    else { ex->colstats_rows_per_block = 0; ex->colstats_blocks = 0; ex->rowstats_slots = 0; ex->splits = 1; }
    if (dtype != GSW_F16 && dtype != GSW_BF16) return GSW_ERR_BAD_ARG;
    if (ex->colstats_capacity < 0 || ex->rowstats_capacity < 0 || ex->workspace_bytes < 0 || ex->max_splits < 0 || ex->max_splits > 64
        || ((uintptr_t)ex->colstats_dev & 15) || ((uintptr_t)ex->rowstats_dev & 7) || ((uintptr_t)ex->workspace_dev & 15)
        || (ex->flags & ~GSW_MM_GN_ONLY)) return GSW_ERR_BAD_ARG;
    void* const ws_dev = ex->workspace_bytes > 0 ? ex->workspace_dev : nullptr;
    const int64_t ws_bytes = ws_dev ? ex->workspace_bytes : 0;
    const int max_splits = ex->max_splits;
    if (a.N % 8 || (a.mode == MM_MODE_GEGLU && a.N % 160) || a.M <= 0 || a.P <= 0) return GSW_ERR_UNSUPPORTED;
    if (a.mode == MM_MODE_QKV && (a.n_rows <= 0 || a.n_rows % 160 || a.n_rows >= a.N || !a.y2)) return GSW_ERR_UNSUPPORTED;
    constexpr int BN = 160;
    const int64_t tiles_n = (a.N + BN - 1) / BN;
    {
        static const int panel_env = getenv("GSW_MM_PANEL") ? atoi(getenv("GSW_MM_PANEL")) : 0;
        a.panel = 8;
        if (tiles_n > 8 && tiles_n <= 32 && tiles_n * BN * (int64_t)a.P * 64 * 2 <= (2 << 20)) a.panel = (int32_t)tiles_n;
        if (panel_env > 0) a.panel = panel_env;
    }
    const MMPlan plan = mm_plan(a.M, tiles_n, a.P, ws_dev && max_splits != 1 && !a.ln_stat, max_splits);
    const int BM = plan.splits >= 2 ? mm_plan(a.M, tiles_n, a.P, false, 1).bm : plan.bm;
    hipStream_t st = (hipStream_t)stream;
    a.splits = 1; a.ws = nullptr;
    if ((a.mode == MM_MODE_DENSE || a.mode == MM_MODE_GEGLU) && ((uintptr_t)a.bias & 15u)) return GSW_ERR_BAD_ARG;
    float* const cs_req = ex->colstats_capacity > 0 ? ex->colstats_dev : nullptr;
    const int64_t cs_cap = cs_req ? ex->colstats_capacity : 0;
    float* const rs_req = ex->rowstats_capacity > 0 ? ex->rowstats_dev : nullptr;
    const int64_t rs_cap = rs_req ? ex->rowstats_capacity : 0;
    a.colstats = nullptr;
    a.rowstats = nullptr;
    if (a.ln_stat && (a.mode != MM_MODE_DENSE && a.mode != MM_MODE_GEGLU && a.mode != MM_MODE_TRANS)) return GSW_ERR_UNSUPPORTED;
    if (a.ln_stat && a.rowbias) return GSW_ERR_UNSUPPORTED;
    if (plan.splits >= 2) {
        const int bm_s = plan.bm, splits = plan.splits;
        const int64_t nt = (((int64_t)a.M + bm_s - 1) / bm_s) * tiles_n;
        const int64_t need = (int64_t)splits * nt * 8 * 5 * (bm_s / 64) * 64 * 16;
        if (need <= ws_bytes) {
            a.tiles_n = (int32_t)tiles_n;
            a.ntiles = (int32_t)nt;
            a.splits = splits; a.ws = (float*)ws_dev;
            ex->splits = splits;
            const uint32_t grid = (uint32_t)((nt * splits + 7) / 8 * 8);
            const int e = dtype == GSW_F16 ? mm_launch_splitk<_Float16>(a, grid, bm_s / 64, st) : mm_launch_splitk<__bf16>(a, grid, bm_s / 64, st);
            if (e != 0) { g_last_hip_error = e; return GSW_ERR_HIP; }
            return GSW_OK;
        }
    }
    bool wide = false;
    {
        static const int wide_mask = getenv("GSW_MM_WIDE") ? atoi(getenv("GSW_MM_WIDE")) : 7;
        const int epi_k = a.mode == MM_MODE_GEGLU ? 2 : (a.mode == MM_MODE_DENSE && !a.rowbias) ? 0 : 1;
        const int wide_env = (wide_mask >> epi_k) & 1;
        const int bm_cfg = g_mm_tile_rows.load(std::memory_order_relaxed);
        const bool mode_ok = a.mode == MM_MODE_DENSE || a.mode == MM_MODE_PF || a.mode == MM_MODE_TOK2PF || a.mode == MM_MODE_UP2X || a.mode == MM_MODE_GEGLU;
        const int64_t tn_w = (a.N + 319) / 320, tm_w = ((int64_t)a.M + 255) / 256;
        int64_t rows_in = a.M;
        if (a.mode == MM_MODE_PF || a.mode == MM_MODE_UP2X) {
            const int64_t per_img = (a.flags & MM_FLAG_COMPACT) ? (int64_t)std::max(1, (a.Hp - 2) * (a.Wp - 2)) : (int64_t)a.Hp * a.Wp;
            rows_in = ((int64_t)a.M / per_img + 1) * (int64_t)a.in_Hp * a.in_Wp + 2 * (int64_t)a.in_Wp + 4;
        }
        int64_t ld_max = 0;
        for (int i = 0; i < a.nseg; ++i) ld_max = std::max<int64_t>(ld_max, a.seg[i].ld);
        int64_t rows_out = a.M;
        if (a.mode == MM_MODE_PF || a.mode == MM_MODE_TOK2PF) rows_out = ((int64_t)a.M / std::max<int64_t>(1, (a.mode == MM_MODE_TOK2PF ? a.S : ((a.flags & MM_FLAG_COMPACT) ? (int64_t)(a.Hp - 2) * (a.Wp - 2) : (int64_t)a.Hp * a.Wp))) + 1) * (int64_t)a.Hp * a.Wp;
        if (a.mode == MM_MODE_UP2X) rows_out = rows_in * 4 + 8;
        const bool res_ok = !a.resid || rows_out * (int64_t)a.ldr * 2 < ((int64_t)1 << 32) - (1 << 20);
        const bool y_ok = !(a.mode == MM_MODE_DENSE && !a.rowbias) || (int64_t)a.M * a.ldy * 2 < ((int64_t)1 << 32) - (1 << 20);
        const bool legal = mode_ok && res_ok && y_ok && a.N >= 320 && a.N % 320 == 0 && (!(a.mode == MM_MODE_GEGLU || (a.mode == MM_MODE_DENSE && !a.rowbias)) || a.M % 256 == 0) && rows_in * ld_max * 2 < ((int64_t)1 << 32) - (1 << 20) && (int64_t)a.N * a.ldw * 2 < ((int64_t)1 << 32) - (1 << 20);
        static const int pmin_dense = getenv("GSW_MM_WIDE_PMIN") ? atoi(getenv("GSW_MM_WIDE_PMIN")) : 5;
        static const int pmin_pf = getenv("GSW_MM_WIDE_PMIN_PF") ? atoi(getenv("GSW_MM_WIDE_PMIN_PF")) : 64;
        static const int pmin_res = getenv("GSW_MM_WIDE_PMIN_RES") ? atoi(getenv("GSW_MM_WIDE_PMIN_RES")) : 8;
        const int p_min = epi_k == 1 ? pmin_pf : (a.resid ? std::max(pmin_dense, pmin_res) : pmin_dense);
        const int64_t cus = mm_cus();
        const int64_t t_w = tm_w * tn_w, t_n = (((int64_t)a.M + 255) / 256) * tiles_n;
        const double cost_w = 1.77 * (double)((t_w + cus - 1) / cus), cost_n = (double)((t_n + cus - 1) / cus);
        const bool fits = t_w >= cus && cost_w <= 0.995 * cost_n && a.P >= p_min && a.M >= 2048;
        const bool aff_multi = epi_k != 1 && a.nseg > 1;
        if (aff_multi && legal && bm_cfg == 512) return GSW_ERR_UNSUPPORTED;
        wide = legal && !aff_multi && (bm_cfg == 512 || (bm_cfg == 0 && wide_env != 0 && fits));
    }
    const int BMt = wide ? 256 : BM, BNt = wide ? 320 : BN;
    const int64_t tiles_nt = (a.N + BNt - 1) / BNt;
    const int64_t tiles_m = ((int64_t)a.M + BMt - 1) / BMt;
    if (tiles_m * tiles_nt > 0x7FFFFFFF) return GSW_ERR_UNSUPPORTED;
    a.tiles_n = (int32_t)tiles_nt;
    a.ntiles = (int32_t)(tiles_m * tiles_nt);
    if (wide) {
        a.panel = 4;
        if (tiles_nt > 4 && tiles_nt <= 16 && tiles_nt * 320 * (int64_t)a.P * 64 * 2 <= (2 << 20)) a.panel = (int32_t)tiles_nt;
    }
    const uint32_t grid = (uint32_t)std::min<int64_t>(mm_cus(), (a.ntiles + 7) / 8 * 8);
    const int ngrp = wide ? 4 : 2, wmv = wide ? 2 : 4;
    if (rs_req && a.mode == MM_MODE_DENSE && !a.rowbias && !a.ln_stat && (int64_t)a.M * ngrp * tiles_nt * 2 <= rs_cap) {
        a.rowstats = rs_req;
        ex->rowstats_slots = (int)(ngrp * tiles_nt);
    }
    if (cs_req && (a.mode == MM_MODE_TOK2PF || ((a.mode == MM_MODE_PF || a.mode == MM_MODE_UP2X) && (a.flags & MM_FLAG_COMPACT)))
        && tiles_m * wmv * (int64_t)a.N <= cs_cap) {
        a.colstats = cs_req;
        ex->colstats_rows_per_block = BMt / wmv; ex->colstats_blocks = (int)(tiles_m * wmv);
    }
    const int epi = a.mode == MM_MODE_QKV ? 5 : a.mode == MM_MODE_TRANS ? 3 : a.mode == MM_MODE_GEGLU ? 2 : (a.mode == MM_MODE_DENSE && !a.rowbias) ? 0 : 1;
    const int e = dtype == GSW_F16 ? mm_launch_e<_Float16>(a, epi, grid, wide ? 8 : BM / 64, st) : mm_launch_e<__bf16>(a, epi, grid, wide ? 8 : BM / 64, st);
    if (e != 0) { g_last_hip_error = e; return GSW_ERR_HIP; }
    return GSW_OK;
}

int gsw_gemm_strided(const void* x_dev, int64_t ldx, const void* w_dev, int64_t ldw, const void* bias_dev, const void* resid_dev, int64_t ldr,
                     void* y_dev, int64_t ldy, int64_t M, int K, int N, int mode, int S, int Wimg, int dtype, void* stream) {
    return gsw_gemm_ex(x_dev, ldx, w_dev, ldw, bias_dev, resid_dev, ldr, y_dev, ldy, M, K, N, mode, S, Wimg, dtype, nullptr, stream);
}

static int mm_gemm_dense(const void* x0_dev, int64_t ld0, int K0, const void* x1_dev, int64_t ld1, int K1, const void* w_dev, int64_t ldw, const void* bias_dev,
                         const void* resid_dev, int64_t ldr, void* y_dev, int64_t ldy, int64_t M, int N, int mode, int S, int Wimg, int dtype, GswMmExtras* ex, void* stream) {
    const bool two = x1_dev != nullptr;
    const int64_t K = (int64_t)K0 + K1;
    if (!x0_dev || !w_dev || !y_dev || M <= 0 || K0 <= 0 || (two && K1 <= 0) || N <= 0) return GSW_ERR_BAD_ARG;
    if (mode != GSW_GEMM_PLAIN && mode != GSW_GEMM_GEGLU && mode != GSW_GEMM_TRANS && mode != GSW_GEMM_TOK2PF) return GSW_ERR_BAD_ARG;
    if (two && mode != GSW_GEMM_PLAIN && mode != GSW_GEMM_TOK2PF) return GSW_ERR_UNSUPPORTED;
    if (K0 % 64 || K1 % 64 || N % 8 || (mode == GSW_GEMM_GEGLU && N % 160) || M > 0x7FFFFF00 || ld0 < K0 || ldw < K || (ld0 & 7) || (ldw & 7) || (ldy & 7) || (ldr & 7)
        || M * ld0 >= ((int64_t)1 << 40) || (int64_t)N * ldw >= ((int64_t)1 << 31) || ld0 >= ((int64_t)1 << 31) || ldy >= ((int64_t)1 << 31) || ldr >= ((int64_t)1 << 31))
        return GSW_ERR_UNSUPPORTED;
    if (two && (ld1 < K1 || (ld1 & 7) || M * ld1 >= ((int64_t)1 << 40) || ld1 >= ((int64_t)1 << 31))) return GSW_ERR_UNSUPPORTED;
    if (mode == GSW_GEMM_GEGLU && resid_dev) return GSW_ERR_UNSUPPORTED;
    if ((mode == GSW_GEMM_PLAIN || mode == GSW_GEMM_GEGLU) && ((uintptr_t)bias_dev & 15u)) return GSW_ERR_BAD_ARG;
    if (mode == GSW_GEMM_TRANS && (resid_dev || S <= 0 || (S & 7) || M % S)) return GSW_ERR_UNSUPPORTED;
    if (mode == GSW_GEMM_TOK2PF && (S <= 0 || Wimg <= 0 || S % Wimg || M % S)) return GSW_ERR_BAD_ARG;
    const int64_t ncols = mode == GSW_GEMM_GEGLU ? N / 2 : N;
    if (mode != GSW_GEMM_TRANS && (ldy < ncols || (resid_dev && ldr < ncols))) return GSW_ERR_BAD_ARG;
    MMArgs a;
    for (int i = 0; i < 3; ++i) a.seg[i] = MMSeg{x0_dev, (int32_t)ld0, K0 / 64, 1, 1, 0, 0, 0};
    a.nseg = 1;
    if (two) { a.seg[1] = MMSeg{x1_dev, (int32_t)ld1, K1 / 64, 1, 1, 0, 0, K0}; a.nseg = 2; }
    a.P = (int32_t)(K / 64);
    a.w = w_dev; a.ldw = (int32_t)ldw;
    a.M = (int32_t)M; a.N = N;
    a.bias = bias_dev; a.rowbias = nullptr; a.resid = resid_dev; a.y = y_dev; a.colstats = nullptr; a.y2 = nullptr; a.n_rows = 0;
    a.ln_stat = nullptr; a.ln_u = nullptr; a.ln_v = nullptr;
    a.ldy = (int32_t)ldy; a.ldr = (int32_t)ldr; a.ldrb = N;
    a.Hp = 1; a.Wp = 1; a.in_Hp = 1; a.in_Wp = 1; a.stride = 1; a.S = S > 0 ? S : 1; a.Wimg = Wimg > 0 ? Wimg : 1; a.up = 0; a.flags = MM_FLAG_NONE;
    a.mode = MM_MODE_DENSE;
    if (mode == GSW_GEMM_GEGLU) a.mode = MM_MODE_GEGLU;
    else if (mode == GSW_GEMM_TRANS) a.mode = MM_MODE_TRANS;
    else if (mode == GSW_GEMM_TOK2PF) { a.mode = MM_MODE_TOK2PF; a.Wp = Wimg + 2; a.Hp = S / Wimg + 2; }
    return gsw_mm_launch(a, dtype, stream, ex);
}

int gsw_gemm_ex(const void* x_dev, int64_t ldx, const void* w_dev, int64_t ldw, const void* bias_dev, const void* resid_dev, int64_t ldr, void* y_dev, int64_t ldy,
                int64_t M, int K, int N, int mode, int S, int Wimg, int dtype, GswMmExtras* ex, void* stream) {
    return mm_gemm_dense(x_dev, ldx, K, nullptr, 0, 0, w_dev, ldw, bias_dev, resid_dev, ldr, y_dev, ldy, M, N, mode, S, Wimg, dtype, ex, stream);
}

int gsw_gemm2_ex(const void* x0_dev, int64_t ld0, int K0, const void* x1_dev, int64_t ld1, int K1, const void* w_dev, int64_t ldw, const void* bias_dev,
                 const void* resid_dev, int64_t ldr, void* y_dev, int64_t ldy, int64_t M, int N, int mode, int S, int Wimg, int dtype, GswMmExtras* ex, void* stream) {
    if (!x1_dev) return GSW_ERR_BAD_ARG;
    return mm_gemm_dense(x0_dev, ld0, K0, x1_dev, ld1, K1, w_dev, ldw, bias_dev, resid_dev, ldr, y_dev, ldy, M, N, mode, S, Wimg, dtype, ex, stream);
}

int gsw_gemm_qkv(const void* x_dev, const void* w_dev, const void* bias_dev, void* rows_dev, void* trans_dev, int64_t M, int K, int N_rows, int N,
                 int S, int dtype, void* stream) {
    if (!x_dev || !w_dev || !rows_dev || !trans_dev || M <= 0 || K <= 0 || N <= 0 || N_rows <= 0 || N_rows >= N || S <= 0) return GSW_ERR_BAD_ARG;
    if (K % 64 || N % 8 || N_rows % 160 || (S & 7) || M % S || M > 0x7FFFFF00 || M * (int64_t)K >= ((int64_t)1 << 40) || (int64_t)N * K >= ((int64_t)1 << 31)) return GSW_ERR_UNSUPPORTED;
    MMArgs a;
    for (int i = 0; i < 3; ++i) a.seg[i] = MMSeg{x_dev, K, K / 64, 1, 1, 0, 0, 0};
    a.nseg = 1; a.P = K / 64;
    a.w = w_dev; a.ldw = K;
    a.M = (int32_t)M; a.N = N;
    a.bias = bias_dev; a.rowbias = nullptr; a.resid = nullptr; a.y = rows_dev; a.colstats = nullptr; a.y2 = trans_dev; a.n_rows = N_rows;
    a.ln_stat = nullptr; a.ln_u = nullptr; a.ln_v = nullptr;
    a.ldy = N_rows; a.ldr = N_rows; a.ldrb = N;
    a.Hp = 1; a.Wp = 1; a.in_Hp = 1; a.in_Wp = 1; a.stride = 1; a.S = S; a.Wimg = 1; a.up = 0; a.flags = MM_FLAG_NONE;
    a.mode = MM_MODE_QKV;
    return gsw_mm_launch(a, dtype, stream, nullptr);
}

__global__ __launch_bounds__(256) void gsw_ln_rowstats_finish_kernel(const float2* __restrict__ rec, int32_t slots, int64_t M, float inv_c, float eps, float2* __restrict__ out) {
    const int64_t m = (int64_t)blockIdx.x * 256 + threadIdx.x;
    if (m >= M) return;
    float s = 0.f, q = 0.f;
    for (int32_t k = 0; k < slots; ++k) { const float2 v = rec[m * slots + k]; s += v.x; q += v.y; }
    const float mean = s * inv_c;
    const float var = fmaxf(q * inv_c - mean * mean, 0.f);
    const float rstd = rsqrtf(var + eps);
    out[m] = make_float2(rstd, -rstd * mean);
}

int gsw_ln_rowstats_finish(const float* records_dev, int slots, int64_t M, int C, float eps, float* stat_dev, void* stream) {
    if (!records_dev || !stat_dev || slots <= 0 || M <= 0 || C <= 0) return GSW_ERR_BAD_ARG;
    hipLaunchKernelGGL(gsw_ln_rowstats_finish_kernel, dim3((uint32_t)((M + 255) / 256)), dim3(256), 0, (hipStream_t)stream, reinterpret_cast<const float2*>(records_dev), slots, M,
                       1.0f / (float)C, eps, reinterpret_cast<float2*>(stat_dev));
    hipError_t e = hipGetLastError();
    if (e != hipSuccess) { g_last_hip_error = (int)e; return GSW_ERR_HIP; }
    return GSW_OK;
}

int gsw_gemm_ln(const void* x_dev, const float* ln_stat_dev, const void* w_dev, const float* u_dev, const float* v_dev, void* y_dev, int64_t M, int K, int N,
                int mode, int S, int dtype, void* stream) {
    return gsw_gemm_ln_ex(x_dev, ln_stat_dev, w_dev, u_dev, v_dev, y_dev, M, K, N, mode, S, dtype, nullptr, stream);
}

int gsw_gemm_ln_ex(const void* x_dev, const float* ln_stat_dev, const void* w_dev, const float* u_dev, const float* v_dev, void* y_dev, int64_t M, int K, int N,
                   int mode, int S, int dtype, GswMmExtras* ex, void* stream) {
    if (!x_dev || !ln_stat_dev || !w_dev || !u_dev || !v_dev || !y_dev || M <= 0 || K <= 0 || N <= 0) return GSW_ERR_BAD_ARG;
    if (mode != GSW_GEMM_PLAIN && mode != GSW_GEMM_GEGLU && mode != GSW_GEMM_TRANS) return GSW_ERR_BAD_ARG;
    if (K % 64 || N % 8 || (mode == GSW_GEMM_GEGLU && N % 160) || (M & 7) || M > 0x7FFFFF00 || M * (int64_t)K >= ((int64_t)1 << 40) || (int64_t)N * K >= ((int64_t)1 << 31)) return GSW_ERR_UNSUPPORTED;
    if (mode == GSW_GEMM_TRANS && (S <= 0 || (S & 7) || M % S)) return GSW_ERR_UNSUPPORTED;
    if (((uintptr_t)u_dev | (uintptr_t)v_dev | (uintptr_t)ln_stat_dev) & 15) return GSW_ERR_BAD_ARG;
    MMArgs a;
    for (int i = 0; i < 3; ++i) a.seg[i] = MMSeg{x_dev, K, K / 64, 1, 1, 0, 0, 0};
    a.nseg = 1; a.P = K / 64;
    a.w = w_dev; a.ldw = K;
    a.M = (int32_t)M; a.N = N;
    a.bias = nullptr; a.rowbias = nullptr; a.resid = nullptr; a.y = y_dev; a.colstats = nullptr; a.y2 = nullptr; a.n_rows = 0;
    a.ln_stat = ln_stat_dev; a.ln_u = u_dev; a.ln_v = v_dev;
    const int ncols = mode == GSW_GEMM_GEGLU ? N / 2 : N;
    a.ldy = ncols; a.ldr = ncols; a.ldrb = N;
    a.Hp = 1; a.Wp = 1; a.in_Hp = 1; a.in_Wp = 1; a.stride = 1; a.S = S > 0 ? S : 1; a.Wimg = 1; a.up = 0; a.flags = MM_FLAG_NONE;
    a.mode = mode == GSW_GEMM_GEGLU ? MM_MODE_GEGLU : mode == GSW_GEMM_TRANS ? MM_MODE_TRANS : MM_MODE_DENSE;
    return gsw_mm_launch(a, dtype, stream, ex);
}

int gsw_gemm(const void* x_dev, const void* w_dev, const void* bias_dev, const void* resid_dev, void* y_dev, int64_t M, int K, int N,
             int mode, int S, int Wimg, int dtype, void* stream) {
    return gsw_gemm_strided(x_dev, K, w_dev, K, bias_dev, resid_dev, N, y_dev, mode == GSW_GEMM_GEGLU ? N / 2 : N, M, K, N, mode, S, Wimg, dtype, stream);
}
```

a-watermark-for-diffusion-models_amd/graph.py:

```python
from __future__ import annotations

import os
import warnings
from collections import OrderedDict
from typing import Dict, Optional, Tuple

import torch


def _env_mode() -> str:
    return os.environ.get("GSW_GRAPH", "auto").lower()


AUTO_MAX_ROWS = 32
CHECK_EVERY = 32
_WEIGHTS_EPOCH = [0]


def weights_changed() -> None:
    _WEIGHTS_EPOCH[0] += 1

MAX_ENTRIES = 8


def _switches():
    from . import pf, unet as U, xattn as X, _native as N
    import ctypes as C
    tr, sm = C.c_int(0), C.c_int(0)
    N.lib().gsw_mm_get_config(C.byref(tr), C.byref(sm))
    return (U.FUSED_KERNELS, U.USE_PF, U.UPSAMPLE_SUBPIXEL, U.CACHE_CONTEXT_KV, U.FUSED_QK, U.FUSED_QKV, U.OWN_ATTENTION, U.OWN_GEMM, U.TEMB_TABLE,
            U.CONV_OUT_DIRECT_MAX_PIXELS, U.CFG_SHARED_PREFIX, pf.FUSE_GN_STATS, pf.GN_FUSED_MAX_WGS, pf.GN_FUSED_MAX_PIXELS, pf.FOLD_LN, pf.FOLD_LN_MIN_ROWS, pf.SPLITK_MAX,
            pf.SPLITK_BYTES, pf.SMALL_GEMM_MAX_ROWS, pf.ATTN_KEY_SPLIT, U.FOLD_FF_OUT, X.ENABLED, X.PRE_ENABLED, X.GNPROJ_ENABLED,
            tr.value, sm.value)


class _Entry:
    __slots__ = ("graph", "x_s", "t_s", "ctx_s", "out", "ctx_id", "replays", "ws")


def _ctx_identity(ctx: torch.Tensor):
    base = ctx._base if ctx._base is not None else ctx
    return (base, ctx._version, ctx.storage_offset(), tuple(ctx.shape), tuple(ctx.stride()))


def _same_ctx(a, b) -> bool:
    return a[0] is b[0] and a[1:] == b[1:]


class GraphedEpsModel:

    def __init__(self, model, mode: Optional[str] = None, max_rows: int = AUTO_MAX_ROWS, clone_output: bool = True):
        self.model = model
        m = (mode or _env_mode()).lower()
        self.mode = {"1": "always", "0": "never", "on": "always", "off": "never"}.get(m, m)
        if self.mode not in ("auto", "always", "never"):
            raise ValueError(f"GSW_GRAPH / mode must be auto | always | never (got {m!r})")
        self.max_rows = max_rows
        self.clone_output = clone_output
        self.capture_fallbacks: Dict[str, int] = {}
        self._entries: "OrderedDict[Tuple, _Entry]" = OrderedDict()
        self._weights_key = None
        self._epoch = _WEIGHTS_EPOCH[0]
        if hasattr(model, "register_load_state_dict_post_hook"):
            model.register_load_state_dict_post_hook(lambda _m, _keys: weights_changed())
        self._failed: Dict[Tuple, str] = {}
        self.stats = {"captures": 0, "replays": 0, "eager": 0, "context_refreshes": 0}

    def __getattr__(self, name):
        return getattr(self.__dict__["model"], name)

    def _wants_graph(self, x: torch.Tensor) -> bool:
        if self.mode == "never" or not x.is_cuda:
            return False
        if torch.cuda.is_current_stream_capturing():
            return False
        return self.mode == "always" or x.shape[0] <= self.max_rows

    def _params_key(self):
        return tuple((p.data_ptr(), p._version) for p in self.model.parameters())

    def reset(self):
        self._entries.clear()
        self._failed.clear()

    def _capture(self, key, x, t, ctx, kw) -> Optional[_Entry]:
        e = _Entry()
        e.x_s = torch.empty_like(x, memory_format=torch.contiguous_format).copy_(x)
        e.t_s = torch.empty_like(t).copy_(t)
        e.ctx_s = torch.empty(ctx.shape, dtype=ctx.dtype, device=ctx.device).copy_(ctx)
        e.ctx_id, e.replays = _ctx_identity(ctx), 0
        from . import pf
        e.ws = torch.empty(pf.SPLITK_BYTES, dtype=torch.uint8, device=x.device)
        from . import unet as U
        fb_before = dict(U.FALLBACKS)
        try:
            side = torch.cuda.Stream(device=x.device)
            side.wait_stream(torch.cuda.current_stream(x.device))
            with torch.cuda.stream(side), torch.no_grad(), pf.splitk_workspace(e.ws):
                self.model(e.x_s, e.t_s, e.ctx_s, **kw)
                self.model(e.x_s, e.t_s, e.ctx_s, **kw)
            torch.cuda.current_stream(x.device).wait_stream(side)
            g = torch.cuda.CUDAGraph()
            with torch.no_grad(), pf.splitk_workspace(e.ws), torch.cuda.graph(g):
                e.out = self.model(e.x_s, e.t_s, e.ctx_s, **kw)
            e.graph = g
            for k_, v_ in U.FALLBACKS.items():
                if v_ != fb_before.get(k_, 0):
                    self.capture_fallbacks[k_] = self.capture_fallbacks.get(k_, 0) + 1
        except Exception as exc:
            self._failed[key] = f"{type(exc).__name__}: {exc}"
            warnings.warn(f"gswm graph: capture of the eps model for {key} failed ({self._failed[key]}); running it eagerly", RuntimeWarning, stacklevel=3)
            return None
        self.stats["captures"] += 1
        return e

    @torch.no_grad()
    def __call__(self, x: torch.Tensor, t: torch.Tensor, ctx: torch.Tensor, cfg_dup: bool = False) -> torch.Tensor:
        kw = {"cfg_dup": True} if cfg_dup else {}
        if not self._wants_graph(ctx if cfg_dup else x):
            self.stats["eager"] += 1
            return self.model(x, t, ctx, **kw)
        if not torch.is_tensor(t):
            t = torch.as_tensor(t, device=x.device)
        key = (tuple(x.shape), x.dtype, str(x.device), tuple(t.shape), t.dtype, tuple(ctx.shape), ctx.dtype, bool(cfg_dup), _switches())
        if key in self._failed:
            self.stats["eager"] += 1
            return self.model(x, t, ctx, **kw)
        e = self._entries.get(key)
        cid = _ctx_identity(ctx)
        if e is None or not _same_ctx(cid, e.ctx_id) or e.replays % CHECK_EVERY == 0 or self._epoch != _WEIGHTS_EPOCH[0]:
            self._epoch = _WEIGHTS_EPOCH[0]
            wk = self._params_key()
            if wk != self._weights_key:
                self._entries.clear()
                self._weights_key = wk
                e = None
        if e is None:
            e = self._capture(key, x, t, ctx, kw)
            if e is None:
                self.stats["eager"] += 1
                return self.model(x, t, ctx, **kw)
            self._entries[key] = e
            while len(self._entries) > MAX_ENTRIES:
                self._entries.popitem(last=False)
        elif not _same_ctx(cid, e.ctx_id):
            e.ctx_s.copy_(ctx)
            e.ctx_id = cid
            self.model.prepare_context(e.ctx_s)
            self.stats["context_refreshes"] += 1
        e.x_s.copy_(x)
        e.t_s.copy_(t)
        e.graph.replay()
        e.replays += 1
        self.stats["replays"] += 1
        self._entries.move_to_end(key)
        return e.out.clone() if self.clone_output else e.out


def graphed(model, mode: Optional[str] = None, clone_output: bool = True):
    return model if isinstance(model, GraphedEpsModel) else GraphedEpsModel(model, mode, clone_output=clone_output)
```

a-watermark-for-diffusion-models_amd/vae.py:

```python
from __future__ import annotations

import os
import warnings
from typing import Sequence

import torch
import torch.nn as nn
import torch.nn.functional as F

from . import checkpoint, pf

SCALING_FACTOR = 0.18215

USE_PF = True
FALLBACKS = {}


STRICT = os.environ.get("GSW_STRICT_KERNELS", "1") != "0"


def _fell_off(what: str, x: torch.Tensor) -> None:
    if USE_PF and pf.half_gpu(x):
        why = f"{what}: input {tuple(x.shape)} {x.dtype} is off the padded-flat path (fp16 / bf16; H, W multiples of 8; mid-block tokens % 8; channel counts multiples of 64)"
        if STRICT:
            raise RuntimeError("gswm vae (strict kernels): " + why + " -- pass --strict_kernels 0 to allow the library kernels")
        if why not in FALLBACKS:
            warnings.warn("gswm vae: " + why + " -- running the plain torch modules", RuntimeWarning, stacklevel=3)
        FALLBACKS[why] = FALLBACKS.get(why, 0) + 1


def _pw(conv: nn.Conv2d, cin_pad: int = 0, cout_pad: int = 0):

    def build():
        w, b = conv.weight.detach(), conv.bias.detach()
        if cin_pad and w.shape[1] < cin_pad:
            w = torch.cat([w, w.new_zeros(w.shape[0], cin_pad - w.shape[1], *w.shape[2:])], dim=1)
        if cout_pad and w.shape[0] < cout_pad:
            w = torch.cat([w, w.new_zeros(cout_pad - w.shape[0], *w.shape[1:])], dim=0)
            b = torch.cat([b, b.new_zeros(cout_pad - b.shape[0])])
        return pf.pack_conv_weight(w), b.contiguous()

    return pf.cached(conv, "_gsw_packed", (conv.weight, conv.bias), build)


def _pw_out_folded(conv_out: nn.Conv2d, post: nn.Conv2d):

    def build():
        wp = post.weight.detach().float()[:, :, 0, 0]
        w = torch.einsum("oc,cikl->oikl", wp, conv_out.weight.detach().float())
        b = wp @ conv_out.bias.detach().float() + post.bias.detach().float()
        w = torch.cat([w, w.new_zeros(64 - w.shape[0], *w.shape[1:])], dim=0).to(conv_out.weight.dtype)
        b = torch.cat([b, b.new_zeros(64 - b.shape[0])]).to(conv_out.weight.dtype)
        return pf.pack_conv_weight(w), b.contiguous()

    return pf.cached(conv_out, "_gsw_folded", (conv_out.weight, conv_out.bias, post.weight, post.bias), build)


def _pw_in_folded(conv_in: nn.Conv2d, pre: nn.Conv2d):

    def build():
        wi = conv_in.weight.detach().float()
        wp, bp = pre.weight.detach().float()[:, :, 0, 0], pre.bias.detach().float()
        w = torch.einsum("oikl,ic->ockl", wi, wp)
        w1 = torch.einsum("oikl,i->okl", wi, bp)[:, None]
        w = torch.cat([w, w1, w.new_zeros(w.shape[0], 64 - w.shape[1] - 1, *w.shape[2:])], dim=1).to(conv_in.weight.dtype)
        return pf.pack_conv_weight(w), conv_in.bias.detach().contiguous()

    return pf.cached(conv_in, "_gsw_folded", (conv_in.weight, conv_in.bias, pre.weight, pre.bias), build)


def _pf_ok(x: torch.Tensor) -> bool:
    return USE_PF and pf.half_gpu(x) and x.shape[-1] % 8 == 0 and x.shape[-2] % 8 == 0


def _convs_fit_pf(module: nn.Module) -> bool:
    ok = getattr(module, "_gsw_pf_ok", None)
    if ok is None:
        ok = all((n == "conv_in" or m.in_channels % 64 == 0) and (n == "conv_out" or m.out_channels % 64 == 0)
                 for n, m in module.named_modules() if isinstance(m, nn.Conv2d))
        module._gsw_pf_ok = ok
    return ok


def _to_pf64(x: torch.Tensor, ones_channel: bool = False):
    B, C, H, W = x.shape
    p = pf.PF.zeros(B, H, W, 64, x.dtype, x.device)
    p.interior[..., :C].copy_(x.permute(0, 2, 3, 1))
    if ones_channel:
        p.interior[..., C].fill_(1.0)
    return p


class VaeResnet(nn.Module):
    def __init__(self, cin, cout, groups=32, eps=1e-6):
        super().__init__()
        self.norm1 = nn.GroupNorm(groups, cin, eps=eps)
        self.conv1 = nn.Conv2d(cin, cout, 3, padding=1)
        self.norm2 = nn.GroupNorm(groups, cout, eps=eps)
        self.conv2 = nn.Conv2d(cout, cout, 3, padding=1)
        self.conv_shortcut = nn.Conv2d(cin, cout, 1) if cin != cout else None

    def forward(self, x):
        h = self.conv1(F.silu(self.norm1(x)))
        h = self.conv2(F.silu(self.norm2(h)))
        return (x if self.conv_shortcut is None else self.conv_shortcut(x)) + h

    def forward_pf(self, x):
        h = pf.conv_pf(pf.gn_pf(x, self.norm1), *_pw(self.conv1))
        h = pf.gn_pf(h, self.norm2)
        sc = x if self.conv_shortcut is None else pf.conv_pf(x, *_pw(self.conv_shortcut), ksize=1)
        return pf.conv_pf(h, *_pw(self.conv2), resid=sc)


class VaeAttention(nn.Module):
    def __init__(self, ch, groups=32, eps=1e-6):
        super().__init__()
        self.group_norm = nn.GroupNorm(groups, ch, eps=eps)
        self.to_q = nn.Linear(ch, ch)
        self.to_k = nn.Linear(ch, ch)
        self.to_v = nn.Linear(ch, ch)
        self.to_out = nn.ModuleList([nn.Linear(ch, ch)])

    def forward(self, x):
        b, c, h, w = x.shape
        y = self.group_norm(x).reshape(b, c, h * w).transpose(1, 2)
        q, k, v = self.to_q(y)[:, None], self.to_k(y)[:, None], self.to_v(y)[:, None]
        o = F.scaled_dot_product_attention(q, k, v)[:, 0]
        return x + self.to_out[0](o).transpose(1, 2).reshape(b, c, h, w)

    def forward_pf(self, x):
        y = pf.gn_pf(x, self.group_norm, act=False, tokens=True)
        C, S = x.C, x.H * x.W
        if C % 64 or S % 8:
            raise RuntimeError(f"VaeAttention: {C} channels x {S} tokens is off the hand-written path (channels % 64, tokens % 8)")
        wqk, bqk = pf.cached(self, "_gsw_wqk", (self.to_q.weight, self.to_k.weight, self.to_q.bias, self.to_k.bias),
                          lambda: (torch.cat([self.to_q.weight.detach(), self.to_k.weight.detach()]).contiguous(),
                                   torch.cat([self.to_q.bias.detach(), self.to_k.bias.detach()]).contiguous()))
        qk = pf.gemm(y, wqk, bqk)
        vt = pf.gemm(y, self.to_v.weight.detach(), self.to_v.bias.detach(), mode="trans", tokens=S)
        o = pf.attention_single_head(qk[..., :C], qk[..., C:], vt)
        pf.gemm(o, self.to_out[0].weight.detach(), self.to_out[0].bias.detach(), resid=x.rows, mode="tok2pf", tokens=S, width=x.W, out=x.rows, stats_for=x)
        return x


class VaeMid(nn.Module):
    def __init__(self, ch):
        super().__init__()
        self.resnets = nn.ModuleList([VaeResnet(ch, ch), VaeResnet(ch, ch)])
        self.attentions = nn.ModuleList([VaeAttention(ch)])

    def forward(self, x):
        return self.resnets[1](self.attentions[0](self.resnets[0](x)))

    def forward_pf(self, x):
        return self.resnets[1].forward_pf(self.attentions[0].forward_pf(self.resnets[0].forward_pf(x)))


class _Down(nn.Module):
    def __init__(self, ch):
        super().__init__()
        self.conv = nn.Conv2d(ch, ch, 3, stride=2, padding=0)

    def forward(self, x):
        return self.conv(F.pad(x, (0, 1, 0, 1)))

    def forward_pf(self, x):
        return pf.conv_pf(x, *_pw(self.conv), stride=2, pad_after_only=True)


class _Up(nn.Module):
    def __init__(self, ch):
        super().__init__()
        self.conv = nn.Conv2d(ch, ch, 3, padding=1)

    def forward(self, x):
        return self.conv(F.interpolate(x, scale_factor=2.0, mode="nearest"))

    def forward_pf(self, x):
        if pf.conv_up2x_fusable(x, self.conv.out_channels):
            w4 = pf.cached(self, "_gsw_up4", (self.conv.weight,), lambda: pf.pack_upsample_weight(self.conv.weight))
            return pf.conv_up2x_pf(x, w4, self.conv.bias)
        up = pf.PF.zeros(x.B, 2 * x.H, 2 * x.W, x.C, x.buf.dtype, x.buf.device)
        xi, g = x.interior, up.grid
        for dy in (0, 1):
            for dx in (0, 1):
                g[:, 1 + dy:1 + dy + 2 * x.H:2, 1 + dx:1 + dx + 2 * x.W:2, :].copy_(xi)
        return pf.conv_pf(up, *_pw(self.conv))


class _EncBlock(nn.Module):
    def __init__(self, cin, cout, down):
        super().__init__()
        self.resnets = nn.ModuleList([VaeResnet(cin, cout), VaeResnet(cout, cout)])
        self.downsamplers = nn.ModuleList([_Down(cout)]) if down else None

    def forward(self, x):
        for r in self.resnets:
            x = r(x)
        return x if self.downsamplers is None else self.downsamplers[0](x)

    def forward_pf(self, x):
        for r in self.resnets:
            x = r.forward_pf(x)
        return x if self.downsamplers is None else self.downsamplers[0].forward_pf(x)


class _DecBlock(nn.Module):
    def __init__(self, cin, cout, up):
        super().__init__()
        self.resnets = nn.ModuleList([VaeResnet(cin if i == 0 else cout, cout) for i in range(3)])
        self.upsamplers = nn.ModuleList([_Up(cout)]) if up else None

    def forward(self, x):
        for r in self.resnets:
            x = r(x)
        return x if self.upsamplers is None else self.upsamplers[0](x)

    def forward_pf(self, x):
        for r in self.resnets:
            x = r.forward_pf(x)
        return x if self.upsamplers is None else self.upsamplers[0].forward_pf(x)


class Encoder(nn.Module):
    def __init__(self, chs: Sequence[int], latent=4):
        super().__init__()
        self.conv_in = nn.Conv2d(3, chs[0], 3, padding=1)
        self.down_blocks = nn.ModuleList([_EncBlock(chs[max(i - 1, 0)], c, i < len(chs) - 1) for i, c in enumerate(chs)])
        self.mid_block = VaeMid(chs[-1])
        self.conv_norm_out = nn.GroupNorm(32, chs[-1], eps=1e-6)
        self.conv_out = nn.Conv2d(chs[-1], 2 * latent, 3, padding=1)

    def forward(self, x, post: nn.Conv2d = None):
        if _pf_ok(x) and self._pf_shapes_ok() and self._pf_tokens_ok(x):
            return self.forward_pf(x, post)
        _fell_off("Encoder", x)
        x = self.conv_in(x)
        for b in self.down_blocks:
            x = b(x)
        x = self.conv_out(F.silu(self.conv_norm_out(self.mid_block(x))))
        return x if post is None else post(x)

    def _pf_shapes_ok(self):
        return _convs_fit_pf(self)

    def _pf_tokens_ok(self, x):
        f = 1 << (len(self.down_blocks) - 1)
        return ((x.shape[-2] // f) * (x.shape[-1] // f)) % 8 == 0

    def forward_pf(self, x, post: nn.Conv2d = None):
        h = pf.conv_pf(_to_pf64(x), *_pw(self.conv_in, cin_pad=64))
        for b in self.down_blocks:
            h = b.forward_pf(h)
        h = pf.gn_pf(self.mid_block.forward_pf(h), self.conv_norm_out)
        y = pf.conv_pf(h, *(_pw(self.conv_out, cout_pad=64) if post is None else _pw_out_folded(self.conv_out, post)))
        return y.interior[..., : self.conv_out.out_channels].permute(0, 3, 1, 2).contiguous()


class Decoder(nn.Module):
    def __init__(self, chs: Sequence[int], latent=4):
        super().__init__()
        rev = list(reversed(chs))
        self.conv_in = nn.Conv2d(latent, rev[0], 3, padding=1)
        self.mid_block = VaeMid(rev[0])
        self.up_blocks = nn.ModuleList([_DecBlock(rev[max(i - 1, 0)], c, i < len(rev) - 1) for i, c in enumerate(rev)])
        self.conv_norm_out = nn.GroupNorm(32, rev[-1], eps=1e-6)
        self.conv_out = nn.Conv2d(rev[-1], 3, 3, padding=1)

    def forward(self, z, pre: nn.Conv2d = None):
        if _pf_ok(z) and self._pf_shapes_ok():
            return self.forward_pf(z, pre)
        _fell_off("Decoder", z)
        x = self.mid_block(self.conv_in(z if pre is None else pre(z)))
        for b in self.up_blocks:
            x = b(x)
        return self.conv_out(F.silu(self.conv_norm_out(x)))

    def _pf_shapes_ok(self):
        return _convs_fit_pf(self)

    def forward_pf(self, z, pre: nn.Conv2d = None):
        h0 = pf.conv_pf(_to_pf64(z), *_pw(self.conv_in, cin_pad=64)) if pre is None else pf.conv_pf(_to_pf64(z, ones_channel=True), *_pw_in_folded(self.conv_in, pre))
        h = self.mid_block.forward_pf(h0)
        for b in self.up_blocks:
            h = b.forward_pf(h)
        y = pf.conv_pf(pf.gn_pf(h, self.conv_norm_out), *_pw(self.conv_out, cout_pad=64))
        return y.interior[..., : self.conv_out.out_channels].permute(0, 3, 1, 2).contiguous()


class AutoencoderKL(nn.Module):
    def __init__(self, block_out_channels: Sequence[int] = (128, 256, 512, 512), latent_channels: int = 4):
        super().__init__()
        self.encoder = Encoder(block_out_channels, latent_channels)
        self.decoder = Decoder(block_out_channels, latent_channels)
        self.quant_conv = nn.Conv2d(2 * latent_channels, 2 * latent_channels, 1)
        self.post_quant_conv = nn.Conv2d(latent_channels, latent_channels, 1)
        self.latent_channels = latent_channels

    def encode_mean(self, x: torch.Tensor) -> torch.Tensor:
        return self.encoder(x, post=self.quant_conv)[:, : self.latent_channels]

    def decode(self, z: torch.Tensor) -> torch.Tensor:
        return self.decoder(z, pre=self.post_quant_conv)


@torch.no_grad()
def img_to_latents(x: torch.Tensor, vae: AutoencoderKL) -> torch.Tensor:
    return (vae.encode_mean(2.0 * x - 1.0) * SCALING_FACTOR).contiguous()


@torch.no_grad()
def normalised_img_to_latents(xn: torch.Tensor, vae: AutoencoderKL) -> torch.Tensor:
    return (vae.encode_mean(xn) * SCALING_FACTOR).contiguous()


@torch.no_grad()
def latents_to_img(latents: torch.Tensor, vae: AutoencoderKL) -> torch.Tensor:
    return (vae.decode(latents / SCALING_FACTOR) / 2 + 0.5).clamp(0, 1)


def synthetic_init_(model: nn.Module, seed: int = 0) -> nn.Module:
    g = torch.Generator().manual_seed(seed)
    with torch.no_grad():
        for name, p in model.named_parameters():
            if p.dim() >= 2:
                std = (1.0 / p[0].numel()) ** 0.5
                if name.endswith(("conv2.weight", "to_out.0.weight")):
                    std *= 0.3
                p.copy_(torch.randn(p.shape, generator=g) * std)
            else:
                p.fill_(1.0 if name.endswith("weight") and "norm" in name else 0.0)
    return model


def load_diffusers_state_dict(model: nn.Module, weight_dir: str) -> nn.Module:
    sd = checkpoint.load_component_state_dict(weight_dir, "vae")
    ren = {"query": "to_q", "key": "to_k", "value": "to_v", "proj_attn": "to_out.0"}
    fixed = {}
    for k, v in sd.items():
        for old, new in ren.items():
            k = k.replace(f"attentions.0.{old}.", f"attentions.0.{new}.")
        if k.endswith(("to_q.weight", "to_k.weight", "to_v.weight", "to_out.0.weight")) and v.dim() == 4:
            v = v[:, :, 0, 0]
        fixed[k] = v
    missing, unexpected = model.load_state_dict(fixed, strict=False)
    if missing or unexpected:
        raise RuntimeError(f"VAE state dict mismatch: missing {missing[:5]}, unexpected {unexpected[:5]}")
    return model
```

include/gswm.h:

```cpp
#ifndef GSWM_H
#define GSWM_H

#include <stddef.h>
#include <stdint.h>

#ifdef __cplusplus
extern "C" {
#endif

#if defined(__GNUC__)
#pragma GCC visibility push(default)
#endif

#define GSW_VERSION 500

#define GSW_MSG_INLINE_MAX 256

typedef enum gsw_dtype {
    GSW_F32 = 0,
    GSW_F16 = 1,
    GSW_BF16 = 2,
    GSW_F64 = 3
} gsw_dtype;

typedef enum gsw_status {
    GSW_OK = 0,
    GSW_ERR_BAD_ARG = 1,
    GSW_ERR_UNSUPPORTED = 2,
    GSW_ERR_RAGGED = 3,
    GSW_ERR_HIP = 4,
    GSW_WARN_NO_RECORDS = 5
} gsw_status;

#define GSW_EMBED_EXACT_F64 0u
#define GSW_EMBED_FAST_F32 1u

#define GSW_FLAG_SATURATED 1u
#define GSW_FLAG_NAN 2u

int gsw_version(void);
int gsw_build_flags(void);
const char* gsw_strerror(int status);
int gsw_last_hip_error(void);

int gsw_keystream(const uint8_t key[32], const uint8_t nonce16[16], uint8_t* out_dev, size_t nbytes, void* stream);

int gsw_embed(const uint8_t key[32], const uint8_t nonce16[16], const uint8_t* msg, int msg_bytes,
              const double* u_dev, uint64_t seed, uint64_t image_index0, void* out_dev, int out_dtype, int B,
              int64_t n_elems, uint32_t flags, void* stream);

int gsw_philox_uniform(uint64_t seed, uint64_t image_index0, double* u_dev, int B, int64_t n_elems, void* stream);

int gsw_extract(const void* z_dev, int z_dtype, const uint8_t key[32], const uint8_t nonce16[16], int msg_bits,
                uint8_t* bits_dev, uint32_t* counts_dev, uint32_t* flags_dev, int B, int64_t n_elems, void* stream);

int gsw_bit_matches(const uint8_t* bits_dev, int msg_bits, const uint8_t* ref_msg, int ref_bits,
                    uint32_t* matches_dev, int B, void* stream);

int gsw_ddim_step(const void* x_dev, const void* model_out_dev, void* out_dev, float a, float b, int dtype,
                  int64_t n, void* stream);

int gsw_ddim_step_cfg(const void* x_dev, const void* e_uncond_dev, const void* e_text_dev, void* out_dev, float a,
                      float b, float guidance, int dtype, int64_t n, void* stream);

int gsw_dpm_step(const void* x_dev, const void* e_uncond_dev, const void* e_text_dev ,
                 const void* m_prev_dev , void* x_out_dev, void* m_out_dev, float P, float Q, float A,
                 float B, float C, float guidance, int dtype, int64_t n, void* stream);

int gsw_ddim_step_extract(const void* x_dev, const void* model_out_dev, void* z_out_dev, float a, float b, int dtype,
                          const uint8_t key[32], const uint8_t nonce16[16], int msg_bits, uint8_t* bits_dev,
                          uint32_t* counts_dev, uint32_t* flags_dev, int B, int64_t n_elems, void* stream);

int gsw_groupnorm_silu(const void* x_dev, const void* pre_bias_dev, const void* gamma_dev, const void* beta_dev, void* out_dev, int B, int C,
                       int HW, int groups, float eps, int act, int dtype, void* stream);
int gsw_geglu(const void* in_dev, void* out_dev, int64_t rows, int inner, int dtype, void* stream);

int gsw_conv_pf(const void* x_dev, const void* w_dev, const void* bias_dev, const void* rowbias_dev, int ld_rowbias, const void* resid_dev, void* y_dev,
                int B, int H, int W, int C, int N, int ksize, int stride, int ldx, int dtype, void* stream);

int gsw_groupnorm_pf(const void* x_dev, const void* gamma_dev, const void* beta_dev, void* out_dev, float* workspace_dev, int B, int H, int W,
                     int C, int groups, float eps, int act, int out_tokens, int dtype, void* stream);

int gsw_groupnorm_pf2(const void* x_dev, const void* x2_dev, int Ca, const void* gamma_dev, const void* beta_dev, void* out_dev, float* workspace_dev,
                      int B, int H, int W, int C, int groups, float eps, int act, int out_tokens, int dtype, void* stream);

#define GSW_MM_GN_ONLY 1
typedef struct GswMmExtras {
    float* colstats_dev;
    int64_t colstats_capacity;
    float* rowstats_dev;
    int64_t rowstats_capacity;
    void* workspace_dev;
    int64_t workspace_bytes;
    int max_splits;
    int colstats_rows_per_block, colstats_blocks, rowstats_slots, splits;
    int flags;
} GswMmExtras;

int gsw_gemm_ex(const void* x_dev, int64_t ldx, const void* w_dev, int64_t ldw, const void* bias_dev, const void* resid_dev, int64_t ldr, void* y_dev, int64_t ldy,
                int64_t M, int K, int N, int mode, int S, int Wimg, int dtype, GswMmExtras* ex, void* stream);
int gsw_gemm2_ex(const void* x0_dev, int64_t ld0, int K0, const void* x1_dev, int64_t ld1, int K1, const void* w_dev, int64_t ldw, const void* bias_dev,
                 const void* resid_dev, int64_t ldr, void* y_dev, int64_t ldy, int64_t M, int N, int mode, int S, int Wimg, int dtype, GswMmExtras* ex, void* stream);
int gsw_gemm_ln_ex(const void* x_dev, const float* ln_stat_dev, const void* w_dev, const float* u_dev, const float* v_dev, void* y_dev, int64_t M, int K, int N,
                   int mode, int S, int dtype, GswMmExtras* ex, void* stream);
int gsw_conv_pf_ex(const void* x_dev, const void* w_dev, const void* bias_dev, const void* rowbias_dev, int ld_rowbias, const void* resid_dev, void* y_dev,
                   int B, int H, int W, int C, int N, int ksize, int stride, int ldx, int dtype, GswMmExtras* ex, void* stream);
int gsw_conv3x3_res_pf_ex(const void* x_dev, const void* w_dev, const void* bias_dev, const void* rowbias_dev, int ld_rowbias, const void* resid_dev, void* y_dev,
                          int B, int H, int W, int C, int N, const void* x1_dev, int C1, const void* x2_dev, int C2, int dtype, GswMmExtras* ex, void* stream);
int gsw_conv_up2x_pf_ex(const void* x_dev, const void* w4_dev, const void* bias_dev, void* y_dev, int B, int H, int W, int C, int N, int dtype, GswMmExtras* ex,
                        void* stream);

int gsw_groupnorm_pf_cs(const void* x_dev, const void* x2_dev, int Ca, const float* cs1_dev, int cs1_rows, int cs1_npar, int cs1_blocks,
                        const float* cs2_dev, int cs2_rows, int cs2_npar, int cs2_blocks, const void* gamma_dev, const void* beta_dev, void* out_dev,
                        float* workspace_dev, int B, int H, int W, int C, int groups, float eps, int act, int out_tokens, int dtype, void* stream);

int gsw_conv3x3_res_pf(const void* x_dev, const void* w_dev, const void* bias_dev, const void* rowbias_dev, int ld_rowbias, const void* resid_dev, void* y_dev,
                       int B, int H, int W, int C, int N, const void* x1_dev, int C1, const void* x2_dev, int C2, int dtype, void* stream);

int gsw_add_layernorm(const void* x_dev, const void* delta_dev, const void* gamma_dev, const void* beta_dev, void* xnew_dev, void* y_dev,
                      int64_t rows, int C, float eps, int dtype, void* stream);


#define GSW_GEMM_PLAIN 0
#define GSW_GEMM_GEGLU 1
#define GSW_GEMM_TRANS 2
#define GSW_GEMM_TOK2PF 3
int gsw_gemm(const void* x_dev, const void* w_dev, const void* bias_dev, const void* resid_dev, void* y_dev, int64_t M, int K, int N,
             int mode, int S, int Wimg, int dtype, void* stream);
int gsw_gemm_qkv(const void* x_dev, const void* w_dev, const void* bias_dev, void* rows_dev, void* trans_dev, int64_t M, int K, int N_rows, int N,
                 int S, int dtype, void* stream);

int gsw_ln_rowstats_finish(const float* records_dev, int slots, int64_t M, int C, float eps, float* stat_dev, void* stream);
int gsw_gemm_ln(const void* x_dev, const float* ln_stat_dev, const void* w_dev, const float* u_dev, const float* v_dev, void* y_dev, int64_t M, int K, int N,
                int mode, int S, int dtype, void* stream);

int gsw_gemm_strided(const void* x_dev, int64_t ldx, const void* w_dev, int64_t ldw, const void* bias_dev, const void* resid_dev, int64_t ldr,
                     void* y_dev, int64_t ldy, int64_t M, int K, int N, int mode, int S, int Wimg, int dtype, void* stream);

int gsw_mm_config(int tile_rows, int split_mask);
int gsw_mm_get_config(int* tile_rows, int* split_mask);

int gsw_softmax_rows(void* x_dev, int64_t rows, int cols, int64_t ld, float scale, int dtype, void* stream);

int gsw_groupnorm_pf_fused(const void* x_dev, const void* x2_dev, int Ca, const void* gamma_dev, const void* beta_dev, void* out_dev, int B, int H, int W,
                           int C, int groups, float eps, int act, int out_tokens, int dtype, void* stream);
int gsw_gather_rows(const void* table_dev, int64_t ld_bytes, int64_t nrows, const int64_t* index_dev, int index_stride, void* out_dev, int64_t out_ld_bytes,
                    int B, int64_t row_bytes, void* stream);
int gsw_nchw_to_pf(const void* x_dev, void* y_dev, int B, int Cin, int H, int W, int Cp, int dtype, void* stream);
int gsw_conv3x3_pf_nchw(const void* x_dev, const void* w_dev, const void* bias_dev, void* y_dev, int B, int H, int W, int C, int Nout, int dtype, void* stream);

int gsw_gemm_small_config(int64_t M, int K, int N, int mode);
int gsw_gemm_small(const void* x_dev, int64_t ldx, const void* w_dev, int64_t ldw, const void* bias_dev, const void* resid_dev, int64_t ldr, void* y_dev, int64_t ldy,
                   int64_t M, int K, int N, int mode, int S, int Wimg, const float* ln_records_dev, int ln_slots, float ln_eps, const float* ln_u_dev,
                   const float* ln_v_dev, float* rowstats_dev, int64_t rowstats_capacity, int* rowstats_slots, int config, int dtype, void* stream);

int gsw_conv_up2x_pf(const void* x_dev, const void* w4_dev, const void* bias_dev, void* y_dev, int B, int H, int W, int C, int N, int dtype,
                     void* stream);

int gsw_attention(const void* q_dev, const void* k_dev, const void* vt_dev, void* out_dev, int B, int H, int head_dim, int Sq, int Sk,
                  int Sk_valid, int ldq, int ldk, int ldo, float scale, int dtype, void* stream);
int gsw_attention_ws(const void* q_dev, const void* k_dev, const void* vt_dev, void* out_dev, int B, int H, int head_dim, int Sq, int Sk,
                     int Sk_valid, int ldq, int ldk, int ldo, float scale, int dtype, void* workspace_dev, int64_t workspace_bytes, void* stream);
int gsw_xattn_fused(const void* x_dev, const float* ln_stat_dev, const void* blob_dev, int64_t blob_stride_bytes, const float* v_dev, int64_t v_stride_floats,
                    const int32_t* ctx_index_dev, void* out_dev, float* out_stat_dev, float out_eps, int x_images, int out_images, int tokens, int C, int heads,
                    int dtype, void* stream);
int gsw_xattn_fused_pre(const void* resid_dev, const void* o_dev, const void* w_frag_dev, float ln_eps, const void* blob_dev, int64_t blob_stride_bytes,
                        const float* v_dev, int64_t v_stride_floats, const int32_t* ctx_index_dev, void* out_dev, float* out_stat_dev, float out_eps, int x_images,
                        int out_images, int tokens, int C, int heads, int dtype, void* stream);

int gsw_gn_colstats_pairs(const float* cs_dev, int cs_rows, int cs_npar, int cs_blocks, float* pairsum_dev, int B, int H, int W, int C, void* stream);
int gsw_gn_proj_tokens(const void* x_pf_dev, const float* pairsum_dev, const void* gamma_dev, const void* beta_dev, float gn_eps, int groups, const void* w_frag_dev,
                       void* out_dev, float* out_stat_dev, float out_eps, int B, int H, int W, int C, int dtype, void* stream);

void gsw_mt19937_seed(uint32_t seed, uint32_t key[624]);
int gsw_mt19937_uniform(const uint32_t key[624], int pos, double* u_dev, int64_t n, uint32_t* state_out_dev, void* stream);

typedef enum gsw_image_mode {
    GSW_IMG_U8_HWC = 0,
    GSW_IMG_F16_CHW = 1,
    GSW_IMG_F32_CHW = 2
} gsw_image_mode;

int gsw_lanczos_plan(int in_size, int out_size, int32_t* bounds, int32_t* kk, int kk_capacity);

int gsw_resize_lanczos(const uint8_t* in_dev, int B, int Hin, int Win, void* out_dev, int Hout, int Wout, int out_mode, uint8_t* tmp_dev,
                       const int32_t* hbounds_dev, const int32_t* hkk_dev, int hksize, const int32_t* vbounds_dev, const int32_t* vkk_dev,
                       int vksize, void* stream);

int gsw_tensor_to_image(const void* in_dev, int dtype, int B, int H, int W, int denormalise, uint8_t* out_dev, void* stream);

int gsw_jpeg_quant_tables(int quality, uint8_t luma[64], uint8_t chroma[64]);
size_t gsw_jpeg_workspace_bytes(int B, int H, int W);
int gsw_jpeg_roundtrip(const uint8_t* rgb_dev, int B, int H, int W, int quality, void* out_dev, int out_mode, uint8_t* workspace_dev,
                       void* stream);

int gsw_gaussian_blur_params(float radius, int passes, int* box_radius, uint32_t* ww, uint32_t* fw);
int gsw_gaussian_blur(const uint8_t* rgb_dev, int B, int H, int W, float radius, uint8_t* out_dev, uint8_t* tmp_dev, void* stream);

typedef enum gsw_pointwise_op {
    GSW_PW_BRIGHTNESS = 0,
    GSW_PW_CONTRAST = 1,
    GSW_PW_INVERT = 2,
    GSW_PW_GRAY = 3,
    GSW_PW_HFLIP = 4,
    GSW_PW_VFLIP = 5,
    GSW_PW_NOISE = 6
} gsw_pointwise_op;
int gsw_image_pointwise(const uint8_t* rgb_dev, int B, int H, int W, int op, float strength, uint64_t seed, uint64_t image_index0,
                        void* out_dev, int out_mode, uint64_t* workspace_dev, void* stream);


typedef enum gsw_resample_filter {
    GSW_RESAMPLE_LANCZOS = 1,
    GSW_RESAMPLE_BILINEAR = 2
} gsw_resample_filter;

int gsw_resample_plan(int filter, int in_size, int out_size, int32_t* bounds, int32_t* kk, int kk_capacity);

int gsw_affine_nearest(const uint8_t* in_dev, int B, int H, int W, const int32_t* coeffs_dev, void* out_dev, int out_mode, void* stream);

int gsw_box_mask(const uint8_t* in_dev, int B, int H, int W, const int32_t* boxes_dev, int keep_inside, void* out_dev, int out_mode, void* stream);

int gsw_crop_resize(const uint8_t* in_dev, int B, int H, int W, const int32_t* origins_dev, int crop_h, int crop_w, void* out_dev, int Hout,
                    int Wout, int out_mode, uint8_t* tmp_dev, const int32_t* hbounds_dev, const int32_t* hkk_dev, int hksize,
                    const int32_t* vbounds_dev, const int32_t* vkk_dev, int vksize, void* stream);

#define GSW_TRACE_SOFT 0
#define GSW_TRACE_HARD 1
size_t gsw_trace_workspace_bytes(int B, int64_t n_users, int k);
int gsw_trace_topk(const uint32_t* counts_dev, int B, int msg_bits, int copies, int mode, const uint8_t* registry_dev, int64_t n_users, int k,
                   int32_t* idx_dev, int32_t* score_dev, void* workspace_dev, void* stream);

int gsw_sign_pack(const void* z_dev, int z_dtype, uint8_t* signs_dev, uint32_t* flags_dev, int B, int64_t n_elems, void* stream);

size_t gsw_trace_keyed_workspace_bytes(int B, int64_t n_records, int k);
int gsw_trace_keyed_topk(const uint8_t* signs_dev, int B, int64_t n_bits, const uint8_t* records_dev, int64_t record_stride, int msg_bytes,
                         int64_t n_records, int k, int32_t* idx_dev, int32_t* score_dev, void* workspace_dev, void* stream);

int gsw_embed_l(const uint8_t key[32], const uint8_t nonce16[16], const uint8_t* msg, int msg_bytes, const double* u_dev, uint64_t seed,
                uint64_t image_index0, void* out_dev, int out_dtype, int B, int64_t n_elems, uint32_t flags, int l, void* stream);
int gsw_extract_l(const void* z_dev, int z_dtype, const uint8_t key[32], const uint8_t nonce16[16], int msg_bits, uint8_t* bits_dev,
                  uint32_t* counts_dev, uint32_t* flags_dev, int B, int64_t n_elems, int l, void* stream);
int gsw_quant_pack(const void* z_dev, int z_dtype, uint8_t* packed_dev, uint32_t* flags_dev, int B, int64_t n_elems, int l, void* stream);

#if defined(__GNUC__)
#pragma GCC visibility pop
#endif

#ifdef __cplusplus
}
#endif
#endif
```

Baseline: 7.963 images/s.

## Add 128-column tile variant for PF-row conv GEMM epilogue with auto selection

Templates the MFMA GEMM kernel on the number of 16-column cells per wave group, adding a 128-column tile (NCB=4) for the PF-row epilogue. The tile width is chosen per launch by whichever of 128 or 160 pads N less, so convolutions with N=128, 256 or 512 channels stop wasting MMA work on padding columns. Planning, panel sizing and the wide-tile checks are refactored into helpers, and a policy query API plus a config knob are exposed. The VAE conv1 call also switches to gn_only. The narrower tile lowers arithmetic intensity per tile and changes the scheduling-barrier ratios, which could hurt MFMA overlap.

```diff
diff --git a/a-watermark-for-diffusion-models_amd/_native.py b/a-watermark-for-diffusion-models_amd/_native.py
--- a/a-watermark-for-diffusion-models_amd/_native.py
+++ b/a-watermark-for-diffusion-models_amd/_native.py
@@ -10,6 +10,7 @@
 GSW_OK, GSW_ERR_BAD_ARG, GSW_ERR_UNSUPPORTED, GSW_ERR_RAGGED, GSW_ERR_HIP, GSW_WARN_NO_RECORDS = 0, 1, 2, 3, 4, 5
 GSW_EMBED_EXACT_F64, GSW_EMBED_FAST_F32 = 0, 1
 GSW_MM_GN_ONLY = 1
+GSW_MM_POLICY_CONV, GSW_MM_POLICY_QKV = 4, 5
 GSW_FLAG_SATURATED, GSW_FLAG_NAN = 1, 2
 GSW_MSG_INLINE_MAX = 256
 GSW_IMG_U8_HWC, GSW_IMG_F16_CHW, GSW_IMG_F32_CHW = 0, 1, 2
@@ -99,6 +100,8 @@
     "gsw_softmax_rows": (C.c_int, [C.c_void_p, C.c_int64, C.c_int, C.c_int64, C.c_float, C.c_int, C.c_void_p]),
     "gsw_mm_config": (C.c_int, [C.c_int, C.c_int]),
     "gsw_mm_get_config": (C.c_int, [C.POINTER(C.c_int), C.POINTER(C.c_int)]),
+    "gsw_mm_config_cols": (C.c_int, [C.c_int]),
+    "gsw_mm_tile_policy": (C.c_int, [C.c_int, C.c_int64, C.c_int, C.c_int, C.POINTER(C.c_int), C.POINTER(C.c_int), C.POINTER(C.c_int)]),
     "gsw_groupnorm_pf_cs": (C.c_int, [C.c_void_p, C.c_void_p, C.c_int, C.c_void_p, C.c_int, C.c_int, C.c_int, C.c_void_p, C.c_int, C.c_int, C.c_int,
                                       C.c_void_p, C.c_void_p, C.c_void_p, C.c_void_p, C.c_int, C.c_int, C.c_int, C.c_int, C.c_int, C.c_float, C.c_int, C.c_int,
                                       C.c_int, C.c_void_p]),
diff --git a/a-watermark-for-diffusion-models_amd/csrc/gswm_mm.hip b/a-watermark-for-diffusion-models_amd/csrc/gswm_mm.hip
--- a/a-watermark-for-diffusion-models_amd/csrc/gswm_mm.hip
+++ b/a-watermark-for-diffusion-models_amd/csrc/gswm_mm.hip
@@ -13,6 +13,7 @@
 #include "gswm_ablate.inc"
 
 static std::atomic<int> g_mm_tile_rows{getenv("GSW_MM_BM") ? atoi(getenv("GSW_MM_BM")) : 0};
+static std::atomic<int> g_mm_tile_cols{getenv("GSW_MM_BN") ? atoi(getenv("GSW_MM_BN")) : 0};
 static std::atomic<int> g_mm_split_mask{getenv("GSW_MM_SPLIT") ? atoi(getenv("GSW_MM_SPLIT")) : 10 };
 
 namespace {
@@ -69,7 +70,7 @@
     return x + __int_as_float(__builtin_amdgcn_update_dpp(0, __float_as_int(x), CTRL, ROW_MASK, 0xf, false));
 }
 
-template <typename T, int EPI, bool SPLIT, int MT, bool LNF = false>
+template <typename T, int EPI, bool SPLIT, int MT, bool LNF = false, int NCB = 5>
 __global__ __launch_bounds__(SPLIT ? 768 : 512, SPLIT ? 1 : 2) void gsw_mm_kernel(const MMArgs p) {
     static_assert(!LNF || (!SPLIT && (EPI == 0 || EPI == 2 || EPI == 3)), "LayerNorm-folded epilogues: dense rows, GEGLU, transposed; 8-wave form");
     constexpr bool SWAP = EPI == 3;
@@ -79,7 +80,9 @@
     constexpr bool WIDE = MT == 8;
     constexpr int WM = WIDE ? 2 : 4;
     constexpr int NG = 8 / WM;
-    constexpr int BM = WM * 16 * MT, BN = NG * 80;
+    constexpr int HC = 16 * NCB;
+    constexpr int BM = WM * 16 * MT, BN = NG * HC;
+    static_assert(NCB == 5 || (NCB == 4 && EPI == 1 && MT != 8 && !LNF), "128-column tiles: the PF-row epilogue on the 256- and 128-row tiles only (the staged-parameter helpers read five cells)");
     constexpr int NPR = MT / 2;
     static_assert(MT == 8 || MT == 4 || MT == 2, "wave tile of 128, 64 or 32 rows");
     static_assert(!WIDE || (!SPLIT && EPI != 3 && EPI != 4 && EPI != 5), "the wide tile: 8-wave form, dense rows / PF rows / GEGLU; no split-K, no transposed output, no fused q | k | v");
@@ -90,7 +93,6 @@
     constexpr int NDMA = NPA + NPW;
     constexpr uint32_t STAGE = (uint32_t)(BM + BN) * 128u;
     constexpr uint32_t RING = (WIDE ? 2u : 3u) * STAGE;
-    constexpr int HC = 80;
     constexpr bool STG = !SPLIT && !SWAP && !QKV && (EPI == 2 || (EPI == 0 && (!LNF || WIDE)));
     constexpr uint32_t PARAM = RING;
     constexpr uint32_t PAR_V = WIDE ? 2048u : 1024u, PAR_ROWS = WIDE ? 4096u : 2048u;
@@ -439,21 +441,21 @@
     const uint16_t* rowbias = reinterpret_cast<const uint16_t*>(p.rowbias);
     const uint16_t* resid = reinterpret_cast<const uint16_t*>(p.resid);
     uint16_t* Y = reinterpret_cast<uint16_t*>(p.y);
-    mm_f4 acc[5][MT];
-#pragma unroll
-    for (int a = 0; a < 5; ++a)
+    mm_f4 acc[NCB][MT];
+#pragma unroll
+    for (int a = 0; a < NCB; ++a)
 #pragma unroll
         for (int b = 0; b < MT; ++b) acc[a][b] = mm_f4{0.f, 0.f, 0.f, 0.f};
     uint32_t c_it = 0, rd_slot = 0;
     MM_TRACE_DECL();
 
-    auto read_frags = [&](frag (&xf)[MT], frag (&wf)[5], uint32_t slot, uint32_t khalf) {
+    auto read_frags = [&](frag (&xf)[MT], frag (&wf)[NCB], uint32_t slot, uint32_t khalf) {
         const uint8_t* ap = lds + ((khalf ? a_rd1 : a_rd0) + slot);
         const uint8_t* wp = lds + ((khalf ? w_rd1 : w_rd0) + slot);
 #pragma unroll
         for (int im = 0; im < MT; ++im) xf[im] = *reinterpret_cast<const frag*>(ap + im * 2048);
 #pragma unroll
-        for (int in = 0; in < 5; ++in) wf[in] = *reinterpret_cast<const frag*>(wp + in * 2048);
+        for (int in = 0; in < NCB; ++in) wf[in] = *reinterpret_cast<const frag*>(wp + in * 2048);
     };
 
     auto dma_params = [&]() {
@@ -547,10 +549,10 @@
         if constexpr (PART) {
             uint32_t sx = slotx * 8u + wave;
             asm volatile("" : "+s"(sx));
-            float* slab = p.ws + (size_t)sx * (size_t)(5 * MT * 64 * 4);
+            float* slab = p.ws + (size_t)sx * (size_t)(NCB * MT * 64 * 4);
             const uint32_t loff = lane * 4u;
 #pragma unroll
-            for (int in = 0; in < 5; ++in)
+            for (int in = 0; in < NCB; ++in)
 #pragma unroll
                 for (int im = 0; im < MT; ++im)
                     if (m0 + (int32_t)(wm * (16u * MT)) + im * 16 < p.M)
@@ -584,7 +586,7 @@
                     ln_r[im] = v.x; ln_n[im] = v.y;
                 }
 #pragma unroll
-                for (int in = 0; in < 5; ++in) {
+                for (int in = 0; in < NCB; ++in) {
                     const int32_t nb = n0 + (int32_t)(grp * HC + (uint32_t)in * 16u + q * 4u);
                     const int32_t nc = nb < p.N ? nb : 0;
                     ln_u4[in] = *reinterpret_cast<const mm_f4*>(p.ln_u + nc);
@@ -601,7 +603,7 @@
                     ln_r[4 * im + 2] = b[0]; ln_n[4 * im + 2] = b[1]; ln_r[4 * im + 3] = b[2]; ln_n[4 * im + 3] = b[3];
                 }
 #pragma unroll
-                for (int in = 0; in < 5; ++in) {
+                for (int in = 0; in < NCB; ++in) {
                     const int32_t ncol = n0 + (int32_t)(grp * HC + (uint32_t)in * 16u + li);
                     const int32_t nc = ncol < p.N ? ncol : 0;
                     ln_u4[in] = mm_f4{p.ln_u[nc], 0.f, 0.f, 0.f};
@@ -660,7 +662,7 @@
             }
         } else
 #pragma unroll
-        for (int in = 0; in < 5; ++in) {
+        for (int in = 0; in < NCB; ++in) {
             bq_raw[in] = make_uint2(0, 0);
             const int32_t nb = n0 + (int32_t)(grp * HC + (uint32_t)in * 16u + q * 4u);
             if (!LNF && !transposed && bias && nb < p.N) bq_raw[in] = *reinterpret_cast<const uint2*>(bias + nb);
@@ -693,7 +695,7 @@
             float rs_s[NPR], rs_q[NPR];
 #pragma unroll
             for (int pr = 0; pr < NPR; ++pr) { rs_s[pr] = __uint_as_float(zero_hi); rs_q[pr] = __uint_as_float(zero_hi); }
-            constexpr int RSD = SPLIT ? 2 : (WIDE ? 2 : 5);
+            constexpr int RSD = SPLIT ? 2 : (WIDE ? 2 : NCB);
             uint4 rs[5][NPR];
             auto load_rs1 = [&](int in, int pr) {
                 rs[in][pr] = make_uint4(zero_hi, zero_hi, zero_hi, zero_hi);
@@ -804,10 +806,10 @@
                     for (int in = 0; in < RSD; ++in) load_rs(in);
                 }
 #pragma unroll
-                for (int in = 0; in < 5; ++in) {
+                for (int in = 0; in < NCB; ++in) {
                     float bq[4];
                     bias4(in, bq);
-                    if (resid && in + RSD < 5) load_rs(in + RSD);
+                    if (resid && in + RSD < NCB) load_rs(in + RSD);
 #pragma unroll
                     for (int pr = 0; pr < NPR; ++pr) block(in, pr, bq);
                 }
@@ -843,14 +845,14 @@
                 }
             }
 #pragma unroll
-            for (int in = 0; in < 5; ++in) {
+            for (int in = 0; in < NCB; ++in) {
                 float bq[4];
                 bias4(in, bq);
                 const int64_t col = (int64_t)n0 + grp * (uint32_t)HC + (uint32_t)in * 16u + (q >> 1) * 8u;
                 float cs_s[4] = {0.f, 0.f, 0.f, 0.f}, cs_q[4] = {0.f, 0.f, 0.f, 0.f};
 #pragma unroll
                 for (int pr = 0; pr < NPR; ++pr) {
-                    constexpr int NB = 5 * NPR;
+                    constexpr int NB = NCB * NPR;
                     const int j = in * NPR + pr;
                     if constexpr (WIDE) { if ((rowbias || resid) && j + PD < NB) fetch((j + PD) / NPR, (j + PD) % NPR, (j + PD) % (PD + 1)); }
                     uint32_t a0, a1, b0, b1;
@@ -984,7 +986,7 @@
                 gate_block(4); store_last();
             } else {
 #pragma unroll
-                for (int in = 0; in < 5; ++in) gate_block(in);
+                for (int in = 0; in < NCB; ++in) gate_block(in);
                 store_pair(0); store_pair(1);
                 store_last();
             }
@@ -992,7 +994,7 @@
             const int32_t nbase = QKV ? p.n_rows : 0, Nt = p.N - nbase;
             uint16_t* Yt = QKV ? reinterpret_cast<uint16_t*>(p.y2) : Y;
 #pragma unroll
-            for (int in = 0; in < 5; ++in) {
+            for (int in = 0; in < NCB; ++in) {
                 const int32_t ncol = n0 + (int32_t)(grp * HC + (uint32_t)in * 16u + li);
                 const int32_t nrow = ncol - nbase;
                 const bool nok = ncol < p.N;
@@ -1013,22 +1015,22 @@
             }
         }
 #pragma unroll
-        for (int a = 0; a < 5; ++a)
+        for (int a = 0; a < NCB; ++a)
 #pragma unroll
             for (int b = 0; b < MT; ++b) acc[a][b] = mm_f4{0.f, 0.f, 0.f, 0.f};
         ++c_it;
     };
 
-    auto mfma20 = [&](auto swap_tag, frag (&xc)[MT], frag (&wc)[5]) {
+    auto mfma20 = [&](auto swap_tag, frag (&xc)[MT], frag (&wc)[NCB]) {
         constexpr bool SW = decltype(swap_tag)::value;
 #pragma unroll
-        for (int in = 0; in < 5; ++in)
+        for (int in = 0; in < NCB; ++in)
 #pragma unroll
             for (int im = 0; im < MT; ++im)
                 acc[in][im] = SW ? MM_ABL_MMA(xc[im], wc[in], acc[in][im]) : MM_ABL_MMA(wc[in], xc[im], acc[in][im]);
     };
     auto pin_order = [&]() {
-        constexpr int NM = 5 * MT, NR = MT + 5;
+        constexpr int NM = NCB * MT, NR = MT + NCB;
         if constexpr (SPLIT) {
             constexpr int per = MT == 4 ? 2 : 1;
 #pragma unroll
@@ -1036,10 +1038,10 @@
                 __builtin_amdgcn_sched_group_barrier(0x008, per, 0);
                 __builtin_amdgcn_sched_group_barrier(0x100, 1, 0);
             }
-            __builtin_amdgcn_sched_group_barrier(0x008, NM - per * NR, 0);
+            if constexpr (NM - per * NR > 0) __builtin_amdgcn_sched_group_barrier(0x008, NM - per * NR, 0);
         } else {
             constexpr int NV = NPA / 2 + 1;
-            constexpr int per = MT == 4 ? 3 : 1;
+            constexpr int per = MT == 4 ? (NCB == 5 ? 3 : 2) : 1;
 #pragma unroll
             for (int i = 0; i < NV; ++i) {
                 __builtin_amdgcn_sched_group_barrier(0x008, per, 0);
@@ -1050,10 +1052,11 @@
                 __builtin_amdgcn_sched_group_barrier(0x008, 1, 0);
                 __builtin_amdgcn_sched_group_barrier(0x100, 1, 0);
             }
-            __builtin_amdgcn_sched_group_barrier(0x008, NM - per * NV - NR, 0);
-        }
-    };
-    auto step = [&](auto swap_tag, frag (&xX)[MT], frag (&wX)[5], frag (&xY)[MT], frag (&wY)[5], const int32_t step_i) {
+            static_assert(NM - per * NV - NR >= 0, "a phase has an MFMA for every DMA piece and fragment read");
+            if constexpr (NM - per * NV - NR > 0) __builtin_amdgcn_sched_group_barrier(0x008, NM - per * NV - NR, 0);
+        }
+    };
+    auto step = [&](auto swap_tag, frag (&xX)[MT], frag (&wX)[NCB], frag (&xY)[MT], frag (&wY)[NCB], const int32_t step_i) {
         const uint32_t nx_slot = rd_slot + STAGE == RING ? 0u : rd_slot + STAGE;
         MM_STAMP(0);
         if constexpr (!SPLIT) { dma_extra(); dma_h2(); }
@@ -1156,7 +1159,7 @@
         asm volatile("s_waitcnt vmcnt(0)" ::: "memory");
         return;
     }
-    frag xa[MT], wa[5], xb[MT], wb[5];
+    frag xa[MT], wa[NCB], xb[MT], wb[NCB];
     read_frags(xa, wa, 0u, 0u);
     asm volatile("s_waitcnt lgkmcnt(0)" ::: "memory");
     for (uint32_t it = 0; it < nt_mine; ++it) {
@@ -1295,22 +1298,30 @@
     }
 }
 
-template <typename T, int EPI, bool SPLIT, int MT, bool LNF = false>
+template <typename T, int EPI, bool SPLIT, int MT, bool LNF = false, int NCB = 5>
 int mm_launch_k(const MMArgs& a, uint32_t grid, hipStream_t st) {
     static bool attr_done = false;
     constexpr bool wide = MT == 8;
     constexpr size_t ldsb = wide ? 2u * 576u * 128u + 6144u + 256u
-                                 : 3u * (size_t)(64 * MT + 160) * 128u + (!SPLIT && (EPI == 2 || (EPI == 0 && !LNF)) ? 4096u : 0u);
+                                 : 3u * (size_t)(64 * MT + 32 * NCB) * 128u + (!SPLIT && (EPI == 2 || (EPI == 0 && !LNF)) ? 4096u : 0u);
     if (!attr_done) {
-        hipError_t e = hipFuncSetAttribute((const void*)gsw_mm_kernel<T, EPI, SPLIT, MT, LNF>, hipFuncAttributeMaxDynamicSharedMemorySize, 160 * 1024);
+        hipError_t e = hipFuncSetAttribute((const void*)gsw_mm_kernel<T, EPI, SPLIT, MT, LNF, NCB>, hipFuncAttributeMaxDynamicSharedMemorySize, 160 * 1024);
         if (e != hipSuccess) return (int)e;
         attr_done = true;
     }
-    hipLaunchKernelGGL((gsw_mm_kernel<T, EPI, SPLIT, MT, LNF>), dim3(grid), dim3(SPLIT ? 768 : 512), ldsb, st, a);
+    hipLaunchKernelGGL((gsw_mm_kernel<T, EPI, SPLIT, MT, LNF, NCB>), dim3(grid), dim3(SPLIT ? 768 : 512), ldsb, st, a);
     return (int)hipGetLastError();
 }
 template <typename T, int EPI>
-int mm_launch_t(const MMArgs& a, uint32_t grid, int mt, hipStream_t st) {
+int mm_launch_t(const MMArgs& a, uint32_t grid, int mt, int bn, hipStream_t st) {
+    if (bn == 128) {
+        if constexpr (EPI == 1) {
+            if (a.ln_stat || (mt != 4 && mt != 2)) return (int)hipErrorInvalidValue;
+            const bool split = (g_mm_split_mask.load(std::memory_order_relaxed) >> EPI) & 1;
+            if (mt == 4) return split ? mm_launch_k<T, 1, true, 4, false, 4>(a, grid, st) : mm_launch_k<T, 1, false, 4, false, 4>(a, grid, st);
+            return split ? mm_launch_k<T, 1, true, 2, false, 4>(a, grid, st) : mm_launch_k<T, 1, false, 2, false, 4>(a, grid, st);
+        } else return (int)hipErrorInvalidValue;
+    }
     if constexpr (EPI == 5) return mt == 4 ? mm_launch_k<T, 5, false, 4>(a, grid, st) : mm_launch_k<T, 5, false, 2>(a, grid, st);
     else {
     if (a.ln_stat) {
@@ -1336,13 +1347,13 @@
     return (int)hipGetLastError();
 }
 template <typename T>
-int mm_launch_e(const MMArgs& a, int epi, uint32_t grid, int mt, hipStream_t st) {
+int mm_launch_e(const MMArgs& a, int epi, uint32_t grid, int mt, int bn, hipStream_t st) {
     switch (epi) {
-        case 0: return mm_launch_t<T, 0>(a, grid, mt, st);
-        case 1: return mm_launch_t<T, 1>(a, grid, mt, st);
-        case 2: return mm_launch_t<T, 2>(a, grid, mt, st);
-        case 5: return mm_launch_t<T, 5>(a, grid, mt, st);
-        default: return mm_launch_t<T, 3>(a, grid, mt, st);
+        case 0: return mm_launch_t<T, 0>(a, grid, mt, bn, st);
+        case 1: return mm_launch_t<T, 1>(a, grid, mt, bn, st);
+        case 2: return mm_launch_t<T, 2>(a, grid, mt, bn, st);
+        case 5: return mm_launch_t<T, 5>(a, grid, mt, bn, st);
+        default: return mm_launch_t<T, 3>(a, grid, mt, bn, st);
     }
 }
 
@@ -1366,6 +1377,13 @@
     if (tile_rows != -1) g_mm_tile_rows.store(tile_rows, std::memory_order_relaxed);
     if (split_mask != -1) g_mm_split_mask.store(split_mask, std::memory_order_relaxed);
     return GSW_OK;
+}
+
+int gsw_mm_config_cols(int tile_cols) {
+    if (tile_cols != -1 && tile_cols != 0 && tile_cols != 128 && tile_cols != 160) return GSW_ERR_BAD_ARG;
+    const int now = g_mm_tile_cols.load(std::memory_order_relaxed);
+    if (tile_cols != -1) g_mm_tile_cols.store(tile_cols, std::memory_order_relaxed);
+    return now == 128 || now == 160 ? now : 0;
 }
 
 int gsw_mm_get_config(int* tile_rows, int* split_mask) {
@@ -1431,13 +1449,52 @@
     return pl;
 }
 
+static int mm_tile_cols(int epi_k, int64_t N) {
+    if (epi_k != 1) return 160;
+    const int force = g_mm_tile_cols.load(std::memory_order_relaxed);
+    if (force == 128 || force == 160) return force;
+    return (N + 127) / 128 * 128 < (N + 159) / 160 * 160 ? 128 : 160;
+}
+static int64_t mm_split_need(const MMPlan& pl, int64_t M, int64_t N) {
+    return (int64_t)pl.splits * (((M + pl.bm - 1) / pl.bm) * ((N + 159) / 160)) * 8 * 5 * (pl.bm / 64) * 64 * 16;
+}
+static bool mm_wide_shape(int epi_k, int64_t M, int64_t N) {
+    return N >= 320 && N % 320 == 0 && (epi_k == 1 || M % 256 == 0);
+}
+static bool mm_wide_fits(int epi_k, int64_t M, int64_t N, int32_t P, bool resid) {
+    static const int wide_mask = getenv("GSW_MM_WIDE") ? atoi(getenv("GSW_MM_WIDE")) : 7;
+    static const int pmin_dense = getenv("GSW_MM_WIDE_PMIN") ? atoi(getenv("GSW_MM_WIDE_PMIN")) : 5;
+    static const int pmin_pf = getenv("GSW_MM_WIDE_PMIN_PF") ? atoi(getenv("GSW_MM_WIDE_PMIN_PF")) : 64;
+    static const int pmin_res = getenv("GSW_MM_WIDE_PMIN_RES") ? atoi(getenv("GSW_MM_WIDE_PMIN_RES")) : 8;
+    const int p_min = epi_k == 1 ? pmin_pf : (resid ? std::max(pmin_dense, pmin_res) : pmin_dense);
+    const int64_t cus = mm_cus();
+    const int64_t t_w = ((M + 255) / 256) * ((N + 319) / 320), t_n = ((M + 255) / 256) * ((N + 159) / 160);
+    const double cost_w = 1.77 * (double)((t_w + cus - 1) / cus), cost_n = (double)((t_n + cus - 1) / cus);
+    return ((wide_mask >> epi_k) & 1) && t_w >= cus && cost_w <= 0.995 * cost_n && P >= p_min && M >= 2048;
+}
+
 double gsw_mm_predict_us(int64_t M, int N, int P, const GswMmExtras* ex) {
     const bool have_ws = ex && ex->workspace_bytes > 0 && ex->workspace_dev;
     const int max_splits = ex ? ex->max_splits : 0;
     const MMPlan pl = mm_plan(M, ((int64_t)N + 159) / 160, P, have_ws && max_splits != 1, max_splits);
-    const int64_t need = (int64_t)pl.splits * (((M + pl.bm - 1) / pl.bm) * (((int64_t)N + 159) / 160)) * 8 * 5 * (pl.bm / 64) * 64 * 16;
-    if (pl.splits >= 2 && need > (ex ? ex->workspace_bytes : 0)) return mm_plan(M, ((int64_t)N + 159) / 160, P, false, 1).t_us;
-    return pl.t_us;
+    if (pl.splits >= 2 && mm_split_need(pl, M, N) <= (ex ? ex->workspace_bytes : 0)) return pl.t_us;
+    const int bn = mm_tile_cols(1, N);
+    return mm_plan(M, ((int64_t)N + bn - 1) / bn, P, false, 1).t_us;
+}
+
+int gsw_mm_tile_policy(int mode, int64_t M, int N, int P, int* tile_cols, int* tile_rows, int* splits) {
+    if (mode < GSW_GEMM_PLAIN || mode > GSW_MM_POLICY_QKV || M <= 0 || M > 0x7FFFFF00 || N <= 0 || (N & 7) || P <= 0) return GSW_ERR_BAD_ARG;
+    const int epi_k = mode == GSW_GEMM_GEGLU ? 2 : mode == GSW_GEMM_PLAIN ? 0 : (mode == GSW_GEMM_TOK2PF || mode == GSW_MM_POLICY_CONV) ? 1 : 3;
+    int bn = 160, bm = 0, sp = 1;
+    const MMPlan pl = mm_plan(M, ((int64_t)N + 159) / 160, P, true, 0);
+    const int bm_cfg = g_mm_tile_rows.load(std::memory_order_relaxed);
+    if (pl.splits >= 2) { bm = pl.bm; sp = pl.splits; }
+    else if (epi_k <= 2 && mm_wide_shape(epi_k, M, N) && (bm_cfg == 512 || (bm_cfg == 0 && mm_wide_fits(epi_k, M, N, P, false)))) { bn = 320; bm = 256; }
+    else { bn = mm_tile_cols(epi_k, N); bm = mm_plan(M, ((int64_t)N + bn - 1) / bn, P, false, 1).bm; }
+    if (tile_cols) *tile_cols = bn;
+    if (tile_rows) *tile_rows = bm;
+    if (splits) *splits = sp;
+    return GSW_OK;
 }
 
 int gsw_mm_launch(MMArgs& a, int dtype, void* stream, GswMmExtras* ex) {
@@ -1453,16 +1510,18 @@
     const int max_splits = ex->max_splits;
     if (a.N % 8 || (a.mode == MM_MODE_GEGLU && a.N % 160) || a.M <= 0 || a.P <= 0) return GSW_ERR_UNSUPPORTED;
     if (a.mode == MM_MODE_QKV && (a.n_rows <= 0 || a.n_rows % 160 || a.n_rows >= a.N || !a.y2)) return GSW_ERR_UNSUPPORTED;
-    constexpr int BN = 160;
-    const int64_t tiles_n = (a.N + BN - 1) / BN;
-    {
+    const int epi = a.mode == MM_MODE_QKV ? 5 : a.mode == MM_MODE_TRANS ? 3 : a.mode == MM_MODE_GEGLU ? 2 : (a.mode == MM_MODE_DENSE && !a.rowbias) ? 0 : 1;
+    const int BN = mm_tile_cols(epi, a.N);
+    const int64_t tiles_n160 = (a.N + 159) / 160, tiles_n = (a.N + BN - 1) / BN;
+    auto set_panel = [&](int64_t tn, int bn) {
         static const int panel_env = getenv("GSW_MM_PANEL") ? atoi(getenv("GSW_MM_PANEL")) : 0;
         a.panel = 8;
-        if (tiles_n > 8 && tiles_n <= 32 && tiles_n * BN * (int64_t)a.P * 64 * 2 <= (2 << 20)) a.panel = (int32_t)tiles_n;
+        if (tn > 8 && tn <= 32 && tn * bn * (int64_t)a.P * 64 * 2 <= (2 << 20)) a.panel = (int32_t)tn;
         if (panel_env > 0) a.panel = panel_env;
-    }
-    const MMPlan plan = mm_plan(a.M, tiles_n, a.P, ws_dev && max_splits != 1 && !a.ln_stat, max_splits);
-    const int BM = plan.splits >= 2 ? mm_plan(a.M, tiles_n, a.P, false, 1).bm : plan.bm;
+    };
+    set_panel(tiles_n160, 160);
+    const MMPlan plan = mm_plan(a.M, tiles_n160, a.P, ws_dev && max_splits != 1 && !a.ln_stat, max_splits);
+    const int BM = mm_plan(a.M, tiles_n, a.P, false, 1).bm;
     hipStream_t st = (hipStream_t)stream;
     a.splits = 1; a.ws = nullptr;
     if ((a.mode == MM_MODE_DENSE || a.mode == MM_MODE_GEGLU) && ((uintptr_t)a.bias & 15u)) return GSW_ERR_BAD_ARG;
@@ -1476,10 +1535,10 @@
     if (a.ln_stat && a.rowbias) return GSW_ERR_UNSUPPORTED;
     if (plan.splits >= 2) {
         const int bm_s = plan.bm, splits = plan.splits;
-        const int64_t nt = (((int64_t)a.M + bm_s - 1) / bm_s) * tiles_n;
-        const int64_t need = (int64_t)splits * nt * 8 * 5 * (bm_s / 64) * 64 * 16;
+        const int64_t nt = (((int64_t)a.M + bm_s - 1) / bm_s) * tiles_n160;
+        const int64_t need = mm_split_need(plan, a.M, a.N);
         if (need <= ws_bytes) {
-            a.tiles_n = (int32_t)tiles_n;
+            a.tiles_n = (int32_t)tiles_n160;
             a.ntiles = (int32_t)nt;
             a.splits = splits; a.ws = (float*)ws_dev;
             ex->splits = splits;
@@ -1491,12 +1550,9 @@
     }
     bool wide = false;
     {
-        static const int wide_mask = getenv("GSW_MM_WIDE") ? atoi(getenv("GSW_MM_WIDE")) : 7;
-        const int epi_k = a.mode == MM_MODE_GEGLU ? 2 : (a.mode == MM_MODE_DENSE && !a.rowbias) ? 0 : 1;
-        const int wide_env = (wide_mask >> epi_k) & 1;
+        const int epi_k = epi;
         const int bm_cfg = g_mm_tile_rows.load(std::memory_order_relaxed);
         const bool mode_ok = a.mode == MM_MODE_DENSE || a.mode == MM_MODE_PF || a.mode == MM_MODE_TOK2PF || a.mode == MM_MODE_UP2X || a.mode == MM_MODE_GEGLU;
-        const int64_t tn_w = (a.N + 319) / 320, tm_w = ((int64_t)a.M + 255) / 256;
         int64_t rows_in = a.M;
         if (a.mode == MM_MODE_PF || a.mode == MM_MODE_UP2X) {
             const int64_t per_img = (a.flags & MM_FLAG_COMPACT) ? (int64_t)std::max(1, (a.Hp - 2) * (a.Wp - 2)) : (int64_t)a.Hp * a.Wp;
@@ -1509,20 +1565,14 @@
         if (a.mode == MM_MODE_UP2X) rows_out = rows_in * 4 + 8;
         const bool res_ok = !a.resid || rows_out * (int64_t)a.ldr * 2 < ((int64_t)1 << 32) - (1 << 20);
         const bool y_ok = !(a.mode == MM_MODE_DENSE && !a.rowbias) || (int64_t)a.M * a.ldy * 2 < ((int64_t)1 << 32) - (1 << 20);
-        const bool legal = mode_ok && res_ok && y_ok && a.N >= 320 && a.N % 320 == 0 && (!(a.mode == MM_MODE_GEGLU || (a.mode == MM_MODE_DENSE && !a.rowbias)) || a.M % 256 == 0) && rows_in * ld_max * 2 < ((int64_t)1 << 32) - (1 << 20) && (int64_t)a.N * a.ldw * 2 < ((int64_t)1 << 32) - (1 << 20);
-        static const int pmin_dense = getenv("GSW_MM_WIDE_PMIN") ? atoi(getenv("GSW_MM_WIDE_PMIN")) : 5;
-        static const int pmin_pf = getenv("GSW_MM_WIDE_PMIN_PF") ? atoi(getenv("GSW_MM_WIDE_PMIN_PF")) : 64;
-        static const int pmin_res = getenv("GSW_MM_WIDE_PMIN_RES") ? atoi(getenv("GSW_MM_WIDE_PMIN_RES")) : 8;
-        const int p_min = epi_k == 1 ? pmin_pf : (a.resid ? std::max(pmin_dense, pmin_res) : pmin_dense);
-        const int64_t cus = mm_cus();
-        const int64_t t_w = tm_w * tn_w, t_n = (((int64_t)a.M + 255) / 256) * tiles_n;
-        const double cost_w = 1.77 * (double)((t_w + cus - 1) / cus), cost_n = (double)((t_n + cus - 1) / cus);
-        const bool fits = t_w >= cus && cost_w <= 0.995 * cost_n && a.P >= p_min && a.M >= 2048;
+        const bool legal = mode_ok && res_ok && y_ok && mm_wide_shape(epi_k, a.M, a.N) && rows_in * ld_max * 2 < ((int64_t)1 << 32) - (1 << 20) && (int64_t)a.N * a.ldw * 2 < ((int64_t)1 << 32) - (1 << 20);
+        const bool fits = mm_wide_fits(epi_k, a.M, a.N, a.P, a.resid != nullptr);
         const bool aff_multi = epi_k != 1 && a.nseg > 1;
         if (aff_multi && legal && bm_cfg == 512) return GSW_ERR_UNSUPPORTED;
-        wide = legal && !aff_multi && (bm_cfg == 512 || (bm_cfg == 0 && wide_env != 0 && fits));
+        wide = legal && !aff_multi && (bm_cfg == 512 || (bm_cfg == 0 && fits));
     }
     const int BMt = wide ? 256 : BM, BNt = wide ? 320 : BN;
+    if (!wide) set_panel(tiles_n, BN);
     const int64_t tiles_nt = (a.N + BNt - 1) / BNt;
     const int64_t tiles_m = ((int64_t)a.M + BMt - 1) / BMt;
     if (tiles_m * tiles_nt > 0x7FFFFFFF) return GSW_ERR_UNSUPPORTED;
@@ -1543,8 +1593,7 @@
         a.colstats = cs_req;
         ex->colstats_rows_per_block = BMt / wmv; ex->colstats_blocks = (int)(tiles_m * wmv);
     }
-    const int epi = a.mode == MM_MODE_QKV ? 5 : a.mode == MM_MODE_TRANS ? 3 : a.mode == MM_MODE_GEGLU ? 2 : (a.mode == MM_MODE_DENSE && !a.rowbias) ? 0 : 1;
-    const int e = dtype == GSW_F16 ? mm_launch_e<_Float16>(a, epi, grid, wide ? 8 : BM / 64, st) : mm_launch_e<__bf16>(a, epi, grid, wide ? 8 : BM / 64, st);
+    const int e = dtype == GSW_F16 ? mm_launch_e<_Float16>(a, epi, grid, wide ? 8 : BM / 64, wide ? 160 : BN, st) : mm_launch_e<__bf16>(a, epi, grid, wide ? 8 : BM / 64, wide ? 160 : BN, st);
     if (e != 0) { g_last_hip_error = e; return GSW_ERR_HIP; }
     return GSW_OK;
 }
diff --git a/a-watermark-for-diffusion-models_amd/graph.py b/a-watermark-for-diffusion-models_amd/graph.py
--- a/a-watermark-for-diffusion-models_amd/graph.py
+++ b/a-watermark-for-diffusion-models_amd/graph.py
@@ -31,7 +31,7 @@
     return (U.FUSED_KERNELS, U.USE_PF, U.UPSAMPLE_SUBPIXEL, U.CACHE_CONTEXT_KV, U.FUSED_QK, U.FUSED_QKV, U.OWN_ATTENTION, U.OWN_GEMM, U.TEMB_TABLE,
             U.CONV_OUT_DIRECT_MAX_PIXELS, U.CFG_SHARED_PREFIX, pf.FUSE_GN_STATS, pf.GN_FUSED_MAX_WGS, pf.GN_FUSED_MAX_PIXELS, pf.FOLD_LN, pf.FOLD_LN_MIN_ROWS, pf.SPLITK_MAX,
             pf.SPLITK_BYTES, pf.SMALL_GEMM_MAX_ROWS, pf.ATTN_KEY_SPLIT, U.FOLD_FF_OUT, X.ENABLED, X.PRE_ENABLED, X.GNPROJ_ENABLED,
-            tr.value, sm.value)
+            tr.value, sm.value, N.lib().gsw_mm_config_cols(-1))
 
 
 class _Entry:
diff --git a/a-watermark-for-diffusion-models_amd/vae.py b/a-watermark-for-diffusion-models_amd/vae.py
--- a/a-watermark-for-diffusion-models_amd/vae.py
+++ b/a-watermark-for-diffusion-models_amd/vae.py
@@ -106,7 +106,7 @@
         return (x if self.conv_shortcut is None else self.conv_shortcut(x)) + h
 
     def forward_pf(self, x):
-        h = pf.conv_pf(pf.gn_pf(x, self.norm1), *_pw(self.conv1))
+        h = pf.conv_pf(pf.gn_pf(x, self.norm1), *_pw(self.conv1), gn_only=True)
         h = pf.gn_pf(h, self.norm2)
         sc = x if self.conv_shortcut is None else pf.conv_pf(x, *_pw(self.conv_shortcut), ksize=1)
         return pf.conv_pf(h, *_pw(self.conv2), resid=sc)
diff --git a/include/gswm.h b/include/gswm.h
--- a/include/gswm.h
+++ b/include/gswm.h
@@ -140,6 +140,12 @@
 int gsw_mm_config(int tile_rows, int split_mask);
 int gsw_mm_get_config(int* tile_rows, int* split_mask);
 
+int gsw_mm_config_cols(int tile_cols);
+
+#define GSW_MM_POLICY_CONV 4
+#define GSW_MM_POLICY_QKV 5
+int gsw_mm_tile_policy(int mode, int64_t M, int N, int P, int* tile_cols, int* tile_rows, int* splits);
+
 int gsw_softmax_rows(void* x_dev, int64_t rows, int cols, int64_t ld, float scale, int dtype, void* stream);
 
 int gsw_groupnorm_pf_fused(const void* x_dev, const void* x2_dev, int Ca, const void* gamma_dev, const void* beta_dev, void* out_dev, int B, int H, int W,
```

Result: no change. 7.992 images/s (median of 6 runs) (+0.4%).
